# ndmarco/BayesFMMM

Measured on AMD Instinct MI355X. Metric: Gibbs iterations/sec (whole node) at n_funct=4096, K=3, P=30, higher is better.
Workload: dtype f64; 1 GPU; BFMMM_warm_start sweep, n_funct=4096, n_i=100, K=3, P=30, M=6, fp64, one independent chain per GPU (1 chain(s): a chain does not shard, replicas only); chains=1, chains_per_gpu=1

## Files before the change

bayesfmmm_amd/_lib.py:

```python
import ctypes as C
import os

_HERE = os.path.dirname(os.path.abspath(__file__))
LIB_PATH = os.environ.get("BFMMM_LIB_PATH", os.path.join(_HERE, "libbfmmm_hip.so"))

c_double_p = C.POINTER(C.c_double)
c_int64_p = C.POINTER(C.c_int64)


class BfmmmConfig(C.Structure):
    _fields_ = [("model", C.c_int32), ("n_funct", C.c_int32), ("K", C.c_int32), ("n_eigen", C.c_int32),
                ("basis_degree", C.c_int32), ("n_internal_knots", C.c_int32), ("P", C.c_int32),
                ("tot_mcmc_iters", C.c_int32), ("c", C.c_double * 8), ("b", C.c_double), ("nu_1", C.c_double),
                ("alpha1l", C.c_double), ("alpha2l", C.c_double), ("beta1l", C.c_double), ("beta2l", C.c_double),
                ("a_Z_PM", C.c_double), ("a_pi_PM", C.c_double), ("var_alpha3", C.c_double),
                ("var_epsilon1", C.c_double), ("var_epsilon2", C.c_double), ("alpha_nu", C.c_double),
                ("beta_nu", C.c_double), ("alpha_eta", C.c_double), ("beta_eta", C.c_double),
                ("alpha_0", C.c_double), ("beta_0", C.c_double)]


SYMBOLS = {
    "bfmmm_config_defaults": (None, [C.POINTER(BfmmmConfig)]),
    "bfmmm_create": (C.c_int, [C.POINTER(BfmmmConfig), C.c_int, c_double_p, c_double_p, c_int64_p, c_double_p,
                               c_double_p, C.POINTER(C.c_void_p)]),
    "bfmmm_destroy": (None, [C.c_void_p]),
    "bfmmm_create_batch": (C.c_int, [C.POINTER(BfmmmConfig), C.c_int, c_double_p, c_double_p, c_int64_p, c_double_p,
                                     c_double_p, C.c_int, C.POINTER(C.c_void_p)]),
    "bfmmm_create_from_basis_batch": (C.c_int, [C.POINTER(BfmmmConfig), C.c_int, c_double_p, c_double_p, c_int64_p, C.c_int,
                                                C.c_int, c_double_p, C.c_int, C.c_int, C.POINTER(C.c_void_p)]),
    "bfmmm_select_chain": (C.c_int, [C.c_void_p, C.c_int]),
    "bfmmm_n_chains": (C.c_int, [C.c_void_p]),
    "bfmmm_selected_chain": (C.c_int, [C.c_void_p]),
    "bfmmm_set_chain_id_stride": (C.c_int, [C.c_void_p, C.c_uint32]),
    "bfmmm_gather_best": (C.c_int, [C.POINTER(C.c_void_p), C.c_int, c_double_p, C.POINTER(C.c_int32), C.POINTER(C.c_int)]),
    "bfmmm_set_covariates": (C.c_int, [C.c_void_p, c_double_p, C.c_int, C.c_int]),
    "bfmmm_get_basis": (C.c_int, [C.c_void_p, c_double_p, C.c_int64]),
    "bfmmm_set_state": (C.c_int, [C.c_void_p, C.c_char_p, c_double_p, C.c_int64]),
    "bfmmm_get_state": (C.c_int, [C.c_void_p, C.c_char_p, c_double_p, C.c_int64]),
    "bfmmm_init_state": (C.c_int, [C.c_void_p, C.c_int, C.c_uint64, C.c_uint32]),
    "bfmmm_run": (C.c_int, [C.c_void_p, C.c_uint32, C.c_int, C.c_int, C.c_uint64, C.c_uint32, C.c_int, C.c_double]),
    "bfmmm_prepare_run": (C.c_int, [C.c_void_p, C.c_uint32, C.c_int, C.c_int, C.c_uint64, C.c_uint32, C.c_int]),
    "bfmmm_set_slot_base": (C.c_int, [C.c_void_p, C.c_int]),
    "bfmmm_create_from_basis": (C.c_int, [C.POINTER(BfmmmConfig), C.c_int, c_double_p, c_double_p, c_int64_p, C.c_int, C.c_int,
                                          c_double_p, C.c_int, C.POINTER(C.c_void_p)]),
    "bfmmm_tempered_transition": (C.c_int, [C.c_void_p, C.c_uint32, C.c_int, C.c_int, C.c_double, C.c_uint64, C.c_uint32,
                                            c_double_p, C.POINTER(C.c_int)]),
    "bfmmm_get_chain": (C.c_int, [C.c_void_p, C.c_char_p, C.c_int, c_double_p, C.c_int64]),
    "bfmmm_chain_diagnostics": (C.c_int, [C.c_void_p, C.c_char_p, C.c_int, C.c_int, C.c_int64, c_double_p, c_double_p, c_double_p,
                                          c_double_p, c_double_p, c_double_p, c_double_p, C.c_int64]),
    "bfmmm_chain_curve_loglik": (C.c_int, [C.c_void_p, C.c_int, C.c_int, c_double_p, C.c_int64]),
    "bfmmm_chain_curve_diagnostics": (C.c_int, [C.c_void_p, C.c_int, C.c_int, C.c_int64, c_double_p, c_double_p, c_double_p,
                                                c_double_p, c_double_p, c_double_p, c_double_p, C.c_int64]),
    "bfmmm_chain_loo": (C.c_int, [C.c_void_p, C.c_int, C.c_int, C.c_int64, c_double_p, c_double_p, c_double_p, c_double_p,
                                  c_double_p, c_double_p, C.c_int64]),
    "bfmmm_chain_curve_fit": (C.c_int, [C.c_void_p, C.c_int, c_double_p, C.c_int, C.POINTER(C.c_int32), C.c_int, C.c_int, C.c_int,
                                        c_double_p, C.c_int64]),
    "bfmmm_chain_curve_bands": (C.c_int, [C.c_void_p, C.c_int, c_double_p, C.c_int, C.POINTER(C.c_int32), C.c_int, C.c_int, C.c_int,
                                          c_double_p, C.c_int, C.c_int64, c_double_p, c_double_p, c_double_p, C.c_int64]),
    "bfmmm_chain_curve_bands_sim": (C.c_int, [C.c_void_p, C.c_int, c_double_p, C.c_int, C.POINTER(C.c_int32), C.c_int, C.c_int, C.c_int,
                                              C.c_double, C.c_int64, c_double_p, c_double_p, c_double_p, c_double_p, c_double_p, C.c_int64]),
    "bfmmm_set_curve_fit_route": (None, [C.c_int]),
    "bfmmm_chain_similarity": (C.c_int, [C.c_void_p, C.POINTER(C.c_int32), C.c_int, C.c_int, C.c_int, C.c_int64, c_double_p, c_double_p,
                                         c_double_p, C.c_int64]),
    "bfmmm_set_similarity_block": (None, [C.c_int]),
    "bfmmm_chain_similarity_loss": (C.c_int, [C.c_void_p, C.c_int, C.c_int, C.c_int64, c_double_p, C.c_int64, C.POINTER(C.c_int32),
                                              C.POINTER(C.c_int32), c_double_p]),
    "bfmmm_get_slot": (C.c_int, [C.c_void_p, C.c_char_p, C.c_int, c_double_p, C.c_int64]),
    "bfmmm_set_chain": (C.c_int, [C.c_void_p, C.c_char_p, C.c_int, C.c_int, c_double_p, C.c_int64]),
    "bfmmm_chain_slot_loglik": (C.c_int, [C.c_void_p, C.c_int, C.c_int, C.c_int, C.c_int64, c_double_p, c_double_p, C.c_int64]),
    "bfmmm_chain_curve_cov": (C.c_int, [C.c_void_p, c_double_p, C.c_int, c_double_p, C.c_int, C.c_int, C.POINTER(C.c_int32), C.c_int, C.c_int,
                                        C.c_int, C.c_int64, c_double_p, c_double_p, c_double_p, C.c_int64]),
    "bfmmm_chain_align": (C.c_int, [C.c_void_p, c_double_p, C.c_int, C.c_int, C.POINTER(C.c_int32), c_double_p, C.c_int64]),
    "bfmmm_chain_aligned_summary": (C.c_int, [C.c_void_p, C.c_char_p, C.POINTER(C.c_int32), C.c_int, C.c_int, c_double_p, C.c_int,
                                              C.c_int64, c_double_p, c_double_p, c_double_p, c_double_p, c_double_p, c_double_p,
                                              c_double_p, c_double_p, C.c_int64]),
    "bfmmm_chain_cluster_mean_bands": (C.c_int, [C.c_void_p, C.POINTER(C.c_int32), c_double_p, C.c_int, C.c_int, C.c_int, c_double_p,
                                                 C.c_int, C.c_int64, c_double_p, c_double_p, c_double_p, C.c_int64]),
    "bfmmm_chain_cluster_cov_bands": (C.c_int, [C.c_void_p, C.POINTER(C.c_int32), c_double_p, C.c_int, c_double_p, C.c_int, C.c_int,
                                                C.POINTER(C.c_int32), C.c_int, c_double_p, C.c_int, C.c_int, c_double_p, C.c_int, C.c_double,
                                                C.c_int64, c_double_p, c_double_p, c_double_p, c_double_p, c_double_p, c_double_p,
                                                c_double_p, C.c_int64]),
    "bfmmm_chain_rescale": (C.c_int, [C.c_void_p, C.POINTER(C.c_int32), c_double_p, C.c_int, C.c_int, c_double_p, c_double_p,
                                      C.POINTER(C.c_int32), c_double_p, c_double_p, c_int64_p, C.c_int64]),
    "bfmmm_chain_rescaled_summary": (C.c_int, [C.c_void_p, C.c_char_p, c_double_p, c_double_p, C.c_int, C.c_int, c_double_p, C.c_int,
                                               C.c_int64] + [c_double_p] * 8 + [C.c_int64]),
    "bfmmm_chain_cluster_mean_bands_rescaled": (C.c_int, [C.c_void_p, c_double_p, c_double_p, C.c_int, c_double_p, C.c_int, C.c_int,
                                                          c_double_p, C.c_int, C.c_int64, c_double_p, c_double_p, c_double_p, C.c_int64]),
    "bfmmm_chain_cluster_cov_bands_rescaled": (C.c_int, [C.c_void_p, c_double_p, c_double_p, C.c_int, c_double_p, C.c_int, C.c_int,
                                                         C.POINTER(C.c_int32), C.c_int, c_double_p, C.c_int, C.c_int, c_double_p, C.c_int,
                                                         C.c_double, C.c_int64] + [c_double_p] * 7 + [C.c_int64]),
    "bfmmm_chain_cluster_contrast_bands": (C.c_int, [C.c_void_p, c_double_p, c_double_p, C.c_int, c_double_p, c_double_p, C.c_int,
                                                     c_double_p, C.c_int, C.c_int, c_double_p, C.c_int, C.c_double, C.c_int64,
                                                     c_double_p, c_double_p, c_double_p, C.POINTER(C.c_int32), c_double_p, c_double_p,
                                                     c_double_p, C.POINTER(C.c_int32), c_double_p, c_double_p, c_double_p, c_double_p,
                                                     C.c_int64]),
    "bfmmm_chain_cluster_eigen": (C.c_int, [C.c_void_p, C.POINTER(C.c_int32), c_double_p, C.c_int, c_double_p, c_double_p, C.c_int,
                                            c_double_p, C.c_int, C.c_int, c_double_p, C.c_int, C.c_int64] + [c_double_p] * 13 +
                                  [C.POINTER(C.c_int32), C.c_int64]),
    "bfmmm_set_cluster_eig_form": (None, [C.c_int]),
    "bfmmm_chain_predict": (C.c_int, [C.c_void_p, c_double_p, c_double_p, c_double_p, c_int64_p, C.c_int, c_double_p,
                                      C.POINTER(C.c_int32), C.c_int, C.c_int, C.c_int, C.c_int, C.c_uint64, c_double_p, C.c_int64] +
                            [c_double_p] * 10 + [C.c_int64]),
    "bfmmm_chain_predict_fit": (C.c_int, [C.c_void_p, c_double_p, c_double_p, c_double_p, c_int64_p, C.c_int, c_double_p,
                                          C.POINTER(C.c_int32), C.c_int, C.c_int, C.c_int, C.c_int, C.c_uint64, c_double_p,
                                          c_double_p, C.c_int, C.c_int, c_double_p, C.c_int, C.c_int64] +
                                [c_double_p] * 16 + [C.POINTER(C.c_int32), c_double_p, c_double_p, C.c_int64]),
    "bfmmm_chain_loo_marginal": (C.c_int, [C.c_void_p, C.c_int, C.c_int, C.c_int, C.c_int, C.c_uint64, C.c_int, C.c_double, C.c_int,
                                           C.c_int, C.c_int64] + [c_double_p] * 8 + [C.POINTER(C.c_int32)] * 2 + [c_double_p] * 3 +
                                 [C.POINTER(C.c_int32), c_double_p, c_double_p, c_int64_p, C.c_int64, C.c_int64]),
    "bfmmm_chain_predict_laplace": (C.c_int, [C.c_void_p, c_double_p, c_double_p, c_double_p, c_int64_p, C.c_int, c_double_p,
                                              C.POINTER(C.c_int32), C.c_int, C.c_int, C.c_int, C.c_uint64, C.c_int64] +
                                    [c_double_p] * 8 + [C.POINTER(C.c_int32), c_double_p, c_double_p, C.c_int64]),
    "bfmmm_chain_loo_marginal_laplace": (C.c_int, [C.c_void_p, C.c_int, C.c_int, C.c_int, C.c_uint64, C.c_double, C.c_int64] +
                                         [c_double_p] * 8 + [C.POINTER(C.c_int32), c_double_p, c_double_p, C.POINTER(C.c_int32),
                                                             c_double_p, c_double_p, C.c_int64]),
    "bfmmm_chain_loo_pointwise": (C.c_int, [C.c_void_p, C.POINTER(C.c_int32), C.c_int, C.c_int, C.c_int, C.c_int64] +
                                  [c_double_p] * 13 + [C.c_int64]),
    "bfmmm_chain_loo_blocks": (C.c_int, [C.c_void_p, C.POINTER(C.c_int32), c_int64_p, C.POINTER(C.c_int32), C.c_int64, C.c_int, C.c_int,
                                         C.c_int64] + [c_double_p] * 13 + [C.c_int64, C.c_int64]),
    "bfmmm_chain_loo_by_chain": (C.c_int, [C.c_void_p, C.c_int, C.POINTER(C.c_int32), C.c_int, C.c_int, C.c_int, C.c_int64] +
                                 [c_double_p] * 6 + [C.c_int64]),
    "bfmmm_debug_get": (C.c_int, [C.c_void_p, C.c_char_p, c_double_p, C.c_int64, c_int64_p]),
    "bfmmm_set_profile": (C.c_int, [C.c_void_p, C.c_int]),
    "bfmmm_get_timing": (C.c_int, [C.c_void_p, C.c_char_p, C.POINTER(C.c_double), c_int64_p]),
    "bfmmm_set_exact_instances": (None, [C.c_int]),
    "bfmmm_set_curve_record": (None, [C.c_int]),
    "bfmmm_set_solo_pair_gram": (None, [C.c_int]),
    "bfmmm_set_solo_pair_gram_tail": (None, [C.c_int]),
    "bfmmm_last_error": (C.c_char_p, []),
}

_LIB = None


def load():
    global _LIB
    if _LIB is None:
        if not os.path.exists(LIB_PATH):
            raise RuntimeError(
                f"{LIB_PATH} is missing: build it with `python -c 'import __graft_entry__ as g; g.build()'` "
                "(hipcc --offload-arch=gfx950). bayesfmmm_amd has no CPU fallback.")
        lib = C.CDLL(LIB_PATH)
        for name, (res, args) in SYMBOLS.items():
            fn = getattr(lib, name)
            fn.restype = res
            fn.argtypes = args
        _LIB = lib
    return _LIB


class BfmmmError(RuntimeError):
    pass


def check(rc):
    if rc != 0:
        raise BfmmmError(load().bfmmm_last_error().decode())
```

bayesfmmm_amd/csrc/bfmmm_capi.hip:

```cpp
#include "handle.hpp"
#include "rng.hpp"
#include "launchers.hpp"

#include <algorithm>
#include <cmath>
#include <cstring>
#include <map>
#include <chrono>
#include <mutex>

using namespace bfmmm;

static thread_local std::string g_err;
static constexpr int GRAPH_UNROLL = 10;
static std::mutex g_capture_mutex;
int bfmmm::fail(const std::string& msg) { g_err = msg; return 1; }

static const char* kFamNames[FAM_COUNT] = {"total", "curve_z", "pair_gram", "factor", "sweep", "curve_chi", "loglik", "pg_reduce"};

hipError_t bfmmm::copy_sync(bfmmm_handle* h, void* dst, const void* src, size_t bytes, hipMemcpyKind kind) {
  hipError_t e = hipMemcpyAsync(dst, src, bytes, kind, h->st);
  if (e != hipSuccess) return e;
  return hipStreamSynchronize(h->st);
}
// ... 45 lines not shown
extern "C" const char* bfmmm_last_error(void) { return g_err.c_str(); }

static void set_md(Dims& d, int MD) {
  d.MD = MD;
  d.A = d.K * MD;
  d.NZZ = d.K * (d.K + 1) / 2;
  d.NCC = MD * (MD + 1) / 2;
  d.R = d.NZZ * d.NCC;
  d.RT = (d.R + 15) / 16;
  d.AT = (d.A + 15) / 16;
  d.CTG = d.mv ? 1 : (d.LG + 15) / 16;
  d.CTS = (d.P + 15) / 16;
  d.NT = d.RT * d.CTG + d.AT * d.CTS;
}

struct BasisSpec {
  int P, band, pen_band;
  const double* B;
  const double* Pmat;
};

static int create_impl(const bfmmm_config* cfg, int device, const double* y, const double* t, const int64_t* offsets,
                       const double* internal_knots, const double* boundary_knots, const BasisSpec* bs, int n_chains,
                       bfmmm_handle** out);

extern "C" int bfmmm_create(const bfmmm_config* cfg, int device, const double* y, const double* t, const int64_t* offsets,
                            const double* internal_knots, const double* boundary_knots, bfmmm_handle** out) {
  return create_impl(cfg, device, y, t, offsets, internal_knots, boundary_knots, nullptr, 1, out);
}

extern "C" int bfmmm_create_batch(const bfmmm_config* cfg, int device, const double* y, const double* t, const int64_t* offsets,
                                  const double* internal_knots, const double* boundary_knots, int n_chains, bfmmm_handle** out) {
  return create_impl(cfg, device, y, t, offsets, internal_knots, boundary_knots, nullptr, n_chains, out);
}

extern "C" int bfmmm_create_from_basis(const bfmmm_config* cfg, int device, const double* y, const double* B, const int64_t* offsets,
                                       int P, int band, const double* Pmat, int pen_band, bfmmm_handle** out) {
  return bfmmm_create_from_basis_batch(cfg, device, y, B, offsets, P, band, Pmat, pen_band, 1, out);
}

extern "C" int bfmmm_create_from_basis_batch(const bfmmm_config* cfg, int device, const double* y, const double* B, const int64_t* offsets,
                                             int P, int band, const double* Pmat, int pen_band, int n_chains, bfmmm_handle** out) {
  if (!cfg || !y || !B || !offsets || !Pmat || !out) return fail("bfmmm_create_from_basis: null argument");
  if (cfg->model != BFMMM_MODEL_FUNCTIONAL) return fail("bfmmm_create_from_basis: functional model only");
  if (P < 1 || band < 0 || pen_band < 0) return fail("bfmmm_create_from_basis: bad dimensions");
  if (band > BWWIDE) return fail("bfmmm_create_from_basis: the band half-width of B'B must not exceed 31 in this build");
  BasisSpec bs = {P, band, pen_band, B, Pmat};
  return create_impl(cfg, device, y, nullptr, offsets, nullptr, nullptr, &bs, n_chains, out);
}

struct HandleGuard {
  bfmmm_handle* h;
  ~HandleGuard() { if (h) bfmmm_destroy(h); }
};

static int create_impl(const bfmmm_config* cfg, int device, const double* y, const double* t, const int64_t* offsets,
                       const double* internal_knots, const double* boundary_knots, const BasisSpec* bs, int n_chains,
                       bfmmm_handle** out) {
  if (!cfg || !out || !y) return fail("bfmmm_create: null argument");
  if (n_chains < 1 || n_chains > 4096) return fail("bfmmm_create_batch: n_chains must be between 1 and 4096");
  int ndev = 0;
  if (hipGetDeviceCount(&ndev) != hipSuccess || ndev <= 0)
    return fail("bfmmm_create: no HIP device available (the sampler has no CPU fallback)");
  if (device < 0 || device >= ndev) return fail("bfmmm_create: invalid device index");
  const bool mv = cfg->model == BFMMM_MODEL_MULTIVARIATE;
  const int n = cfg->n_funct, K = cfg->K, M = cfg->n_eigen;
  if (n < 1) return fail("'n_funct' must be an integer greater than or equal to 1");
  if (K < 2) return fail("'K' must be an integer greater than or equal to 2");
  if (K > KMAX) return fail("K larger than 8 is not supported by this build");
  if (M < 1) return fail("'n_eigen' must be an integer greater than or equal to 1");
  if (cfg->tot_mcmc_iters < 1) return fail("'tot_mcmc_iters' must be positive");
  int P, BW;
  if (mv) {
    P = cfg->P; BW = 0;
    if (P < 1) return fail("multivariate model: P must be positive");
  } else if (bs) {
    P = bs->P;
    BW = (bs->band <= BWMAX) ? std::min(bs->band, std::max(P - 1, 0)) : (bs->band <= BWMID) ? BWMID : BWWIDE;
  } else {
    if (!t || !offsets || !boundary_knots || (cfg->n_internal_knots > 0 && !internal_knots))
      return fail("bfmmm_create: null argument");
    if (cfg->basis_degree < 1) return fail("'basis_degree' must be an integer greater than or equal to 1");
    if (cfg->basis_degree > BWMAX) return fail("basis_degree larger than 5 is not supported by this build");
    for (int i = 0; i < cfg->n_internal_knots; ++i) {
      if (boundary_knots[0] >= internal_knots[i])
        return fail("at least one element in 'internal_knots' is less than or equal to first boundary knot");
      if (boundary_knots[1] <= internal_knots[i])
        return fail("at least one element in 'internal_knots' is more than or equal to second boundary knot");
    }
    P = cfg->n_internal_knots + cfg->basis_degree + 1;
    BW = std::min(cfg->basis_degree, P - 1);
  }
  if (P > PMAX) return fail("P larger than 64 is not supported by this build");
  if (M > 16) return fail("n_eigen larger than 16 is not supported by this build");

  HIPCHK(hipSetDevice(device));
  prepare_curve_kernels();
  prepare_pair_gram_kernels();
  prepare_factor_kernels();
  prepare_sweep_kernels();
  prepare_cov_kernels();
  { hipError_t e0 = hipGetLastError(); if (e0 != hipSuccess) fprintf(stderr, "[bfmmm] note: kernel attribute setup reported %s\n", hipGetErrorString(e0)); }
  bfmmm_handle* h = new bfmmm_handle();
  HandleGuard guard{h};
  h->cfg = *cfg;
  h->device = device;
  h->T = cfg->tot_mcmc_iters;
  h->nch = n_chains;
  HIPCHK(hipStreamCreateWithFlags(&h->st, hipStreamNonBlocking));
  HIPCHK(hipEventCreate(&h->evA));
  HIPCHK(hipEventCreate(&h->ev0));
  HIPCHK(hipEventCreate(&h->ev1));
  HIPCHK(hipHostMalloc((void**)&h->status_host, sizeof(uint32_t) * (size_t)n_chains, hipHostMallocMapped));
  if (hipHostGetDevicePointer((void**)&h->status_dev, h->status_host, 0) != hipSuccess) { (void)hipGetLastError(); h->status_dev = nullptr; }
  Ctx& c = h->c;
  memset(&c, 0, sizeof c);
  Dims& d = c.d;
  d.n = n; d.K = K; d.P = P; d.M = M; d.D = 0; d.BW = BW; d.LG = (BW + 1) * P;
  d.LREC = (d.LG + P + 1 + 1) / 2 * 2;
  d.mv = mv ? 1 : 0;
  d.BWP = mv ? 0 : std::max(BW, 1);
  if (bs) d.BWP = std::min(std::max(BW, bs->pen_band), (BW > BWMAX) ? BWWIDE : BWMAX);
  if (bs && BW == BWMID && bs->pen_band > BWMID) { BW = BWWIDE; d.BW = BW; d.LG = (BW + 1) * P; d.LREC = (d.LG + P + 1 + 1) / 2 * 2; d.BWP = std::min(std::max(BW, bs->pen_band), BWWIDE); }
  if (bs && BW <= BWMAX && bs->pen_band > BWMAX) return fail("bfmmm_create_from_basis: a penalty band wider than 5 needs a basis band wider than 5 in this build");
  set_md(d, M + 1);
  for (int k = 0; k < KMAX; ++k) c.h.c[k] = (k < 8) ? cfg->c[k] : 10.0;
  c.h.b = cfg->b; c.h.nu_1 = cfg->nu_1;
  c.h.alpha1l = cfg->alpha1l; c.h.alpha2l = cfg->alpha2l; c.h.beta1l = cfg->beta1l; c.h.beta2l = cfg->beta2l;
  c.h.a_Z_PM = cfg->a_Z_PM; c.h.a_pi_PM = cfg->a_pi_PM; c.h.var_alpha3 = cfg->var_alpha3;
  c.h.var_epsilon1 = cfg->var_epsilon1; c.h.var_epsilon2 = cfg->var_epsilon2;
  c.h.alpha_nu = cfg->alpha_nu; c.h.beta_nu = cfg->beta_nu; c.h.alpha_eta = cfg->alpha_eta; c.h.beta_eta = cfg->beta_eta;
  c.h.alpha_0 = cfg->alpha_0; c.h.beta_0 = cfg->beta_0;
  c.T = h->T;
  c.nblk_curve = curve_blocks(n, P);

  const int64_t n_obs = mv ? (int64_t)n * P : offsets[n];
  h->n_obs = n_obs;
  double* rec; int* ni;
  if (dalloc(h, &rec, (size_t)n * d.LREC) || dalloc(h, &ni, n)) return 1;
  c.rec = rec; c.ni = ni;
  int* stab;
  if (dalloc(h, &stab, sweep_tab_ints(K * (M + 1)))) return 1;
  c.sweep_tab = stab;
  std::vector<ArenaReq> ar;
  areq(ar, &c.dyn, 1);
  areq(ar, &c.Z, (size_t)n * K); areq(ar, &c.chi, (size_t)n * M); areq(ar, &c.theta, (size_t)K * (M + 1) * P);
  areq(ar, &c.delta, (size_t)K * M); areq(ar, &c.Aa, (size_t)K * 2); areq(ar, &c.gamma, (size_t)K * P * M);
  int NKS, KS;
  pg_geometry(d, NKS, KS);
  h->pg_part_doubles = (size_t)NKS * d.NT * 256;
  areq(ar, &c.logz_part, (size_t)c.nblk_curve * K); areq(ar, &c.rss_part, c.nblk_curve);
  areq(ar, &c.pg_part, h->pg_part_doubles); areq(ar, &c.H, (size_t)d.R * d.LG + 2); areq(ar, &c.H2, (size_t)d.R * P * (2 * d.BW + 2));
  areq(ar, &c.tvec, (size_t)d.A * P); areq(ar, &c.rvec, (size_t)d.A * P); areq(ar, &c.hq, (size_t)d.A * P);
  areq(ar, &c.gstd, gstd_doubles(K, P, M)); areq(ar, &c.zprep, (size_t)(3 * K + 5) * n);
  areq(ar, &c.chi_norm, (size_t)n * M); areq(ar, &c.zrec, zrec_stride(n, K)); areq(ar, &c.piprep, 9 * KMAX + 16); areq(ar, &c.Lz, (size_t)d.A * P);
  areq(ar, &c.Cmat, (size_t)d.A * P * P + 2);
  {
    const size_t T = (size_t)h->T;
    areq(ar, &c.c_nu, T * K * P); areq(ar, &c.c_chi, T * n * M); areq(ar, &c.c_Z, T * n * K); areq(ar, &c.c_pi, T * K);
    areq(ar, &c.c_alpha3, T); areq(ar, &c.c_delta, T * K * M); areq(ar, &c.c_A, T * K * 2); areq(ar, &c.c_sigma, T);
    areq(ar, &c.c_tau, T * K); areq(ar, &c.c_gamma, T * K * P * M); areq(ar, &c.c_Phi, T * K * P * M); areq(ar, &c.c_loglik, T);
  }
  if (arena_commit(h, ar, n_chains, &c.chain_bytes, &h->arena)) return 1;
  c.chain_bytes_cov = 0; c.chain_id_stride = 1; c.nch = n_chains;
  double* pm;
  if (dalloc(h, &pm, (size_t)P * P)) return 1;
  c.Pmat = pm;
  if (bs) {
    HIPCHK(copy_sync(h, pm, bs->Pmat, sizeof(double) * (size_t)P * P, hipMemcpyHostToDevice));
  } else {
    std::vector<double> Pm((size_t)P * P, 0.0);
    for (int j = 0; j < P; ++j) {
      Pm[0] = 1;
      if (j > 0) { Pm[j + (size_t)P * j] = 2; Pm[(j - 1) + (size_t)P * j] = -1; Pm[j + (size_t)P * (j - 1)] = -1; }
      Pm[(P - 1) + (size_t)P * (P - 1)] = 1;
    }
    HIPCHK(copy_sync(h, pm, Pm.data(), sizeof(double) * Pm.size(), hipMemcpyHostToDevice));
  }

  if (dalloc(h, &h->d_y, (size_t)n_obs)) return 1;
  HIPCHK(copy_sync(h, h->d_y, y, sizeof(double) * (size_t)n_obs, hipMemcpyHostToDevice));
  int* d_err;
  if (dalloc(h, &d_err, 1)) return 1;
  if (mv) {
    launch_stats_multivariate(n, P, d.LREC, h->d_y, rec, ni, h->st);
  } else if (bs) {
    std::vector<double> hrec((size_t)n * d.LREC, 0.0);
    std::vector<int> hni((size_t)n);
    for (int i = 0; i < n; ++i) {
      double* r = hrec.data() + (size_t)i * d.LREC;
      hni[i] = (int)(offsets[i + 1] - offsets[i]);
      for (int64_t l = offsets[i]; l < offsets[i + 1]; ++l) {
        const double* b = bs->B + (size_t)l * P;
        for (int lo = 0; lo < P; ++lo) {
          if (b[lo] == 0.0) continue;
          for (int dd = 0; dd <= BW && lo + dd < P; ++dd) r[dd * P + lo] += b[lo] * b[lo + dd];
          r[d.LG + lo] += b[lo] * y[l];
        }
        r[d.LG + P] += y[l] * y[l];
      }
    }
    HIPCHK(copy_sync(h, rec, hrec.data(), sizeof(double) * hrec.size(), hipMemcpyHostToDevice));
    HIPCHK(copy_sync(h, ni, hni.data(), sizeof(int) * hni.size(), hipMemcpyHostToDevice));
    h->B_host.assign(bs->B, bs->B + (size_t)n_obs * P);
  } else {
    const int deg = cfg->basis_degree, nint = cfg->n_internal_knots;
    h->n_knots = nint + 2 * (deg + 1);
    std::vector<double> knots(h->n_knots);
    for (int i = 0; i <= deg; ++i) knots[i] = boundary_knots[0];
    for (int i = 0; i < nint; ++i) knots[deg + 1 + i] = internal_knots[i];
    for (int i = 0; i <= deg; ++i) knots[deg + 1 + nint + i] = boundary_knots[1];
    if (dalloc(h, &h->d_t, (size_t)n_obs) || dalloc(h, &h->d_off, (size_t)n + 1) || dalloc(h, &h->d_knots, h->n_knots))
      return 1;
    HIPCHK(copy_sync(h, h->d_t, t, sizeof(double) * (size_t)n_obs, hipMemcpyHostToDevice));
    HIPCHK(copy_sync(h, h->d_off, offsets, sizeof(int64_t) * ((size_t)n + 1), hipMemcpyHostToDevice));
    HIPCHK(copy_sync(h, h->d_knots, knots.data(), sizeof(double) * knots.size(), hipMemcpyHostToDevice));
    if (launch_stats_functional(deg, n, P, d.LREC, h->d_off, h->d_t, h->d_y, h->d_knots, h->n_knots, rec, ni, nullptr,
                                d_err, h->st))
      return fail("unsupported basis_degree");
  }
  double* d_yy; long long* d_cnt;
  if (dalloc(h, &d_yy, 1) || dalloc(h, &d_cnt, 2)) return 1;
  launch_stats_totals(n, d.LREC, d.LG + P, rec, ni, d_yy, d_cnt, h->st);
  HIPCHK(hipStreamSynchronize(h->st));
  HIPCHK(hipGetLastError());
  int herr = 0; long long cnt[2];
  HIPCHK(copy_sync(h, &herr, d_err, sizeof(int), hipMemcpyDeviceToHost));
  HIPCHK(copy_sync(h, &c.YY, d_yy, sizeof(double), hipMemcpyDeviceToHost));
  HIPCHK(copy_sync(h, cnt, d_cnt, sizeof cnt, hipMemcpyDeviceToHost));
  if (herr) return fail("at least one time point lies outside 'boundary_knots'");
  d.n_obs_total = cnt[0];
  d.half_sum = cnt[1];
  Dyn dyn0;
  memset(&dyn0, 0, sizeof dyn0);
  dyn0.beta = 1; dyn0.sigma2 = 1; dyn0.alpha3 = 1;
  for (int k = 0; k < KMAX; ++k) { dyn0.pi[k] = 1.0 / K; dyn0.tau[k] = 1; }
  for (int q = 0; q < n_chains; ++q)
    HIPCHK(copy_sync(h, chain_ctx(c, (unsigned)q).dyn, &dyn0, sizeof dyn0, hipMemcpyHostToDevice));
  guard.h = nullptr;
  *out = h;
  return 0;
}

extern "C" int bfmmm_set_covariates(bfmmm_handle* h, const double* X, int D, int covariance_adj) {
  if (!h || !X) return fail("bfmmm_set_covariates: null argument");
  if (D < 1 || D > 8) return fail("bfmmm_set_covariates: the number of covariates must be between 1 and 8 in this build");
  if (h->c.d.D != 0) return fail("bfmmm_set_covariates: covariates are already set");
  HIPCHK(hipSetDevice(h->device));
  Ctx& c = h->c;
  Dims& d = c.d;
  const size_t n = d.n, K = d.K, P = d.P, M = d.M, T = (size_t)h->T;
  d.D = D;
  c.covariance_adj = covariance_adj ? 1 : 0;
  c.A2 = (int)(K * D + (covariance_adj ? K * M * D : 0));
  c.NB2 = cov_w2_chunks((int)n);
  c.NBS = cov_step_blocks(c.nblk_curve);
  c.NPG = D * (D + 1) / 2;
  c.NPAIR = (c.A2 / D) * c.NPG;
  if (!cov_block_fits(c)) {
    d.D = 0;
    return fail("bfmmm_set_covariates: this many covariates with this basis exceed the covariate kernels' on-chip staging (fewer covariates or a narrower band)");
  }
  double* Xd;
  if (dalloc(h, &Xd, n * D)) return 1;
  HIPCHK(copy_sync(h, Xd, X, sizeof(double) * n * D, hipMemcpyHostToDevice));
  c.X = Xd;
  std::vector<ArenaReq> ar;
  areq(ar, &c.thetaX, K * (M + 1) * D * P); areq(ar, &c.tau_eta, K * D); areq(ar, &c.gamma_xi, K * P * D * M);
  areq(ar, &c.delta_xi, K * M * D); areq(ar, &c.A_xi, K * 2 * D); areq(ar, &c.stil, n * P);
  areq(ar, &c.yyp_part, (size_t)c.nblk_curve); areq(ar, &c.cfull, n * P); areq(ar, &c.gfull, n * P);
  areq(ar, &c.w2_part, (size_t)c.NPAIR * c.NB2 * d.LG); areq(ar, &c.H2aa, (size_t)c.NPAIR * d.LG);
  areq(ar, &c.Wdir, n * (size_t)c.A2); areq(ar, &c.gstd2, K * D + K * M * D + K * D * P * M);
  areq(ar, &c.C2, (size_t)c.A2 * P * P + 2); areq(ar, &c.Lz2, (size_t)c.A2 * P);
  areq(ar, &c.step_part, 2 * (size_t)c.NBS * (D * P + 1)); areq(ar, &c.thetaN, K * (M + 1) * D * P); areq(ar, &c.delta_cur, P + 2);
  areq(ar, &c.c_eta, T * P * D * K); areq(ar, &c.c_xi, T * K * P * D * M); areq(ar, &c.c_tau_eta, T * K * D);
  areq(ar, &c.c_gamma_xi, T * K * P * D * M); areq(ar, &c.c_delta_xi, T * K * M * D); areq(ar, &c.c_A_xi, T * K * 2 * D);
  if (arena_commit(h, ar, h->nch, &c.chain_bytes_cov, &h->arena_cov)) { d.D = 0; return 1; }
  std::vector<double> ones(std::max({K * D, K * P * D * M, K * M * D, K * 2 * D}), 1.0);
  for (int q = 0; q < h->nch; ++q) {
    const Ctx cq = chain_ctx(c, (unsigned)q);
    HIPCHK(copy_sync(h, cq.tau_eta, ones.data(), sizeof(double) * K * D, hipMemcpyHostToDevice));
    HIPCHK(copy_sync(h, cq.gamma_xi, ones.data(), sizeof(double) * K * P * D * M, hipMemcpyHostToDevice));
    HIPCHK(copy_sync(h, cq.delta_xi, ones.data(), sizeof(double) * K * M * D, hipMemcpyHostToDevice));
    HIPCHK(copy_sync(h, cq.A_xi, ones.data(), sizeof(double) * K * 2 * D, hipMemcpyHostToDevice));
  }
  drop_graphs(h);
  return 0;
}

extern "C" void bfmmm_destroy(bfmmm_handle* h) {
  if (!h) return;
  (void)hipSetDevice(h->device);
  if (h->st) (void)hipStreamSynchronize(h->st);
  drop_graphs(h);
  for (int q = 1; q < bfmmm_handle::MAX_SUB; ++q) { if (h->sub_st[q]) (void)hipStreamDestroy(h->sub_st[q]); if (h->sub_ev[q]) (void)hipEventDestroy(h->sub_ev[q]); }
  for (void* p : h->allocs) (void)hipFree(p);
  if (h->status_host) (void)hipHostFree(h->status_host);
  if (h->ev0) (void)hipEventDestroy(h->ev0);
  if (h->ev1) (void)hipEventDestroy(h->ev1);
  if (h->evA) (void)hipEventDestroy(h->evA);
  if (h->st) (void)hipStreamDestroy(h->st);
  delete h;
}

extern "C" int bfmmm_get_basis(bfmmm_handle* h, double* out, int64_t capacity) {
  if (!h || !out) return fail("bfmmm_get_basis: null argument");
  const Dims& d = h->c.d;
// ... 270 lines not shown
    launch_loglik_flush(c, sb.st, h->status_dev);
    return;
  }
  for (int r = 0; r < reps; ++r)
    launch_iteration(h, sb.c, plan, sb.r, sb.st, nullptr, kind != GK_FULL, kind == GK_FUSED, kind == GK_DEFERRED);
}

template <typename F>
static int cached_graph(bfmmm_handle* h, int sub, int kind, int reps, hipStream_t st, std::vector<FreshGraph>& fresh, F body,
                        hipGraphExec_t* out) {
  int n_whole = 0;
  for (const auto& e : h->graphs) {
    if (e.sub == sub && e.kind == kind && e.reps == reps) { *out = e.g; return 0; }
    n_whole += e.kind == GK_WHOLE;
  }
  if (kind == GK_WHOLE && n_whole >= WHOLE_KEEP) {
    auto it = std::find_if(h->graphs.begin(), h->graphs.end(), [](const bfmmm_handle::CachedGraph& e) { return e.kind == GK_WHOLE; });
    (void)hipGraphExecDestroy(it->g);
    h->graphs.erase(it);
  }
  std::lock_guard<std::mutex> lock(g_capture_mutex);
  hipGraph_t graph = nullptr;
  HIPCHK(hipStreamBeginCapture(st, hipStreamCaptureModeRelaxed));
  body();
  const hipError_t ec = hipStreamEndCapture(st, &graph);
  if (ec != hipSuccess) { if (graph) (void)hipGraphDestroy(graph); HIPCHK(ec); }
  hipGraphExec_t g = nullptr;
  const hipError_t ei = hipGraphInstantiate(&g, graph, nullptr, nullptr, 0);
  (void)hipGraphDestroy(graph);
  HIPCHK(ei);
  (void)hipGraphUpload(g, st);
  h->graphs.push_back({sub, kind, reps, g});
  fresh.push_back({g, st});
  *out = g;
  return 0;
}

static int dry_launch(bfmmm_handle* h, const Ctx& c, uint32_t mask, const Sub* subs, int nsub, const std::vector<FreshGraph>& fresh,
                      int first_iter, uint32_t tt_step, double beta) {
  if (fresh.empty()) return 0;
  const size_t wb1 = (size_t)((char*)h->c.c_nu - (char*)h->c.dyn);
  const size_t wb2 = (c.d.D > 0 && h->arena_cov) ? (size_t)((char*)h->c.c_eta - (char*)h->c.thetaX) : 0;
  const size_t need = (size_t)h->nch * (wb1 + wb2);
  if (h->dry_snap_bytes < need) {
    char* nb = nullptr;
    if (hipMalloc((void**)&nb, need) != hipSuccess) { (void)hipGetLastError(); return 0; }
    h->allocs.push_back(nb);
    h->dry_snap = nb; h->dry_snap_bytes = need;
  }
  const size_t cb1 = h->nch > 1 ? h->c.chain_bytes : wb1, cb2 = h->nch > 1 ? h->c.chain_bytes_cov : wb2;
  char* snap2 = h->dry_snap + (size_t)h->nch * wb1;
  for (int q = 0; q < nsub; ++q) HIPCHK(hipStreamSynchronize(subs[q].st));
  HIPCHK(hipMemcpy2DAsync(h->dry_snap, wb1, h->c.dyn, cb1, wb1, (size_t)h->nch, hipMemcpyDeviceToDevice, h->st));
  if (wb2) HIPCHK(hipMemcpy2DAsync(snap2, wb2, h->c.thetaX, cb2, wb2, (size_t)h->nch, hipMemcpyDeviceToDevice, h->st));
  ensure_sweep_tables(h, c, mask);
  const auto t_dry = std::chrono::steady_clock::now();
  for (int round = 0; round < 64; ++round) {
    for (const FreshGraph& fg : fresh) {
      hipLaunchKernelGGL(k_run_begin, dim3(h->nch), dim3(64), 0, h->st, h->c, (uint32_t)first_iter, (uint32_t)h->slot_base, tt_step, beta, 0);
      HIPCHK(hipStreamSynchronize(h->st));
      HIPCHK(hipGraphLaunch(fg.g, fg.st));
      HIPCHK(hipStreamSynchronize(fg.st));
    }
    if (std::chrono::duration<double, std::milli>(std::chrono::steady_clock::now() - t_dry).count() >= 10.0) break;
  }
  HIPCHK(hipMemcpy2DAsync(h->c.dyn, cb1, h->dry_snap, wb1, wb1, (size_t)h->nch, hipMemcpyDeviceToDevice, h->st));
  if (wb2) HIPCHK(hipMemcpy2DAsync(h->c.thetaX, cb2, snap2, wb2, wb2, (size_t)h->nch, hipMemcpyDeviceToDevice, h->st));
  HIPCHK(hipStreamSynchronize(h->st));
  HIPCHK(hipGetLastError());
  return 0;
}

static int run_profiled(bfmmm_handle* h, const Ctx& c, const Plan& plan, const PgRoute& r, int n_iters, uint32_t tt_step) {
  const bool fuse = plan.z && plan.z_update && plan.chi && c.d.D == 0 && n_iters >= 2 && tt_step == 0;
  for (int it = 0; it < n_iters; ++it) {
    std::vector<hipEvent_t> evs;
    const bool skip_z = fuse && it > 0, fuse_z = fuse && it + 1 < n_iters;
    launch_iteration(h, c, plan, r, h->st, &evs, skip_z, fuse_z, false);
    HIPCHK(hipStreamSynchronize(h->st));
    const int fams[7] = {FAM_Z, FAM_PG, FAM_REDUCE, FAM_FACTOR, FAM_SWEEP, FAM_CHI, FAM_LOGLIK};
    const bool ran[7] = {plan.z && !skip_z, true, plan.pg, plan.factor, true, true, c.defer_loglik == 0};
    for (int q = 0; q < 7; ++q) {
      float ms = 0;
      (void)hipEventElapsedTime(&ms, evs[q], evs[q + 1]);
      if (ran[q]) { h->fam_ms[fams[q]] += ms; h->fam_launches[fams[q]] += 1; }
    }
    for (hipEvent_t e : evs) (void)hipEventDestroy(e);
  }
  return 0;
}

static int finish_run(bfmmm_handle* h, const Ctx& c, const Plan& plan, uint32_t mask, int first_iter, int n_iters, bool whole) {
  const bool status_by_kernel = c.defer_loglik && n_iters > 0 && h->status_dev != nullptr;
  if (c.defer_loglik && n_iters > 0 && !whole) launch_loglik_flush(c, h->st, status_by_kernel ? h->status_dev : nullptr);
  const int s0 = first_iter - h->slot_base, s1 = s0 + n_iters;
  if (!(mask & U_Z)) launch_fill_slots(c, c.c_Z, c.Z, (size_t)c.d.n * c.d.K, s0, s1, h->st);
  if (!plan.chi_update) launch_fill_slots(c, c.c_chi, c.chi, (size_t)c.d.n * c.d.M, s0, s1, h->st);
  HIPCHK(hipEventRecord(h->ev1, h->st));
  if (!status_by_kernel)
    HIPCHK(hipMemcpy2DAsync(h->status_host, sizeof(uint32_t), &h->c.dyn->status, h->nch > 1 ? h->c.chain_bytes : sizeof(uint32_t), sizeof(uint32_t),
                            (size_t)h->nch, hipMemcpyDeviceToHost, h->st));
  HIPCHK(hipStreamSynchronize(h->st));
  if (h->launch_error == 2) { h->launch_error = 0; drop_graphs(h); return fail("bfmmm_run: internal error (no per-curve kernel instance is built for the route the launcher chose)"); }
  if (h->launch_error) { h->launch_error = 0; return fail("bfmmm_run: problem size exceeds the sweep kernel's LDS (5 A P doubles + A^2 ints must fit 160 KB)"); }
  HIPCHK(hipGetLastError());
  float ms = 0;
  HIPCHK(hipEventElapsedTime(&ms, h->ev0, h->ev1));
  h->fam_ms[FAM_TOTAL] = ms;
  h->fam_launches[FAM_TOTAL] = n_iters;
  for (int q = 0; q < h->nch; ++q) {
    const uint32_t status = h->status_host[q];
    if (status & 8u) return fail("bfmmm_run: internal error (the pi / alpha_3 job of k_factor did not signal)");
    if (status & 4u) return fail("bfmmm_run: internal error (a hand-off inside the sweep kernel timed out)");
    if (status & 2u) return fail("bfmmm_run: internal error (fused Z update without prepared proposals)");
    if (status & 1u)
      return fail("bfmmm_run: a conditional precision matrix was not positive definite");
  }
  return 0;
}

static void record_curve_route(bfmmm_handle* h, const Ctx& c, const Plan& plan, bool fuse, bool defer) {
  double v[14] = {0, -1, 0, 0, 0, 0, -1, 0, 0, 0, 0, 0, 0, 0};
  const int mode = chi_launch_arg(plan, false);
  const CurveRoute rc = curve_route_decide(c.d, 1, mode);
  const double w[8] = {(double)rc.BW, (double)rc.LPC, rc.COV ? 1.0 : 0.0, rc.SMALL ? 1.0 : 0.0, (double)rc.KX, (double)rc.MX, (double)mode,
                       fuse ? 1.0 : 0.0};
  memcpy(v + 6, w, sizeof w);
  if (fuse) {
    const CurveRoute rf = curve_route_decide(c.d, 1, chi_launch_arg(plan, true));
    const double z[6] = {3, (double)rf.BW, (double)rf.LPC, 0, (double)(rf.KX ? rf.KX : (rf.SMALL ? 4 : KMAX)), rf.KX ? 1.0 : 0.0};
    memcpy(v, z, sizeof z);
  } else if (plan.z) {
    const CurveRoute rz = curve_route_decide(c.d, 0, z_launch_arg(plan, defer));
    const double z[6] = {rz.LEAN ? 2.0 : 1.0, (double)rz.BW, (double)rz.LPC, rz.COV ? 1.0 : 0.0, (double)rz.KT, rz.KEX ? 1.0 : 0.0};
    memcpy(v, z, sizeof z);
  }
  memcpy(h->last_curve, v, sizeof v);
}

static int run_impl(bfmmm_handle* h, uint32_t mask, int first_iter, int n_iters, uint64_t seed, uint32_t chain,
                    int phi_chi_zero, double beta, uint32_t tt_step, bool prepare_only = false) {
  if (!h) return fail("bfmmm_run: null handle");
  if (n_iters < 0 || first_iter < h->slot_base || first_iter - h->slot_base + n_iters > h->T)
    return fail("bfmmm_run: iterations exceed the allocated chain");
  HIPCHK(hipSetDevice(h->device));
  Ctx c = h->c;
  const int MD = phi_chi_zero ? 1 : (c.d.M + 1);
  set_md(c.d, MD);
  c.seed = seed; c.chain = chain; c.mask = mask;
  Plan plan = make_plan(mask, MD);
  if (c.d.D > 0) { plan.z = true; plan.chi = true; plan.use_rss_part = 1; }
  c.defer_loglik = (c.d.D == 0) ? 1 : 0;
  c.ll_use_part = plan.use_rss_part;
  h->last_md = MD;
  int nsub = 1;
  if (!h->profile && h->nch >= 4) nsub = 2;
  if (const char* env_split = h->profile ? nullptr : getenv("BFMMM_BATCH_SPLIT"))
    nsub = std::max(1, std::min({atoi(env_split), (int)bfmmm_handle::MAX_SUB, h->nch / 2}));
  Sub subs[bfmmm_handle::MAX_SUB];
  h->sub_st[0] = h->st;
  for (int q = 0, q0 = 0; q < nsub; ++q) {
    const int cnt = h->nch / nsub + (q < h->nch % nsub ? 1 : 0);
    if (pg_route(h, c, plan.pg, cnt, h->profile ? bfmmm_handle::MAX_SUB : q, subs[q].r)) return 1;
    if (!h->sub_st[q]) HIPCHK(hipStreamCreateWithFlags(&h->sub_st[q], hipStreamNonBlocking));
    if (!h->sub_ev[q]) HIPCHK(hipEventCreateWithFlags(&h->sub_ev[q], hipEventDisableTiming));
    subs[q].c = chain_ctx(c, (unsigned)q0);
    subs[q].c.nch = cnt;
    subs[q].st = h->sub_st[q];
    q0 += cnt;
  }
  {
    const PgRoute& r0 = subs[0].r;
    const double v[6] = {r0.packed ? 1.0 : 0.0, (double)r0.KS, (double)r0.NKS, (double)r0.body, (double)r0.G, (double)r0.tail};
    memcpy(h->last_route, v, sizeof v);
    const SweepRoute sr = sweep_route_decide(c.d);
    const double w[5] = {(double)sr.kernel, (double)sr.targ, c.d.mv ? 1.0 : 0.0, (double)sr.direct, (double)sr.threads};
    memcpy(h->last_sweep, w, sizeof w);
    if (c.d.D > 0) {
      const CovRoute cr = cov_route_decide(c);
      const double x[11] = {(double)cr.BW, (double)cr.LPC, (double)cr.DX, (double)cr.W2D, (double)cr.PP, (double)cr.NB2, (double)cr.NBS,
                            (double)cr.NPG, (double)cr.launches, cr.do_eta ? 1.0 : 0.0, cr.do_xi ? 1.0 : 0.0};
      memcpy(h->last_cov, x, sizeof x);
    }
  }
  const int rec_on = bfmmm::g_curve_record;
  if (!rec_on) {
    c.zrec = nullptr;
    for (int q = 0; q < nsub; ++q) subs[q].c.zrec = nullptr;
  }
  c.defer_hyper = (c.defer_loglik && plan.pg && plan.chi && h->nch == 1 && !subs[0].r.packed && subs[0].r.NKS >= 2) ? 1 : 0;
  subs[0].c.defer_hyper = c.defer_hyper;
  if (!prepare_only) {
    ensure_sweep_tables(h, c, mask);
    hipLaunchKernelGGL(k_run_begin, dim3(h->nch), dim3(64), 0, h->st, h->c, (uint32_t)first_iter, (uint32_t)h->slot_base, tt_step, beta,
                       h->state_dirty ? 1 : 0);
    h->state_dirty = false;
    for (int f = 0; f < FAM_COUNT; ++f) { h->fam_ms[f] = 0; h->fam_launches[f] = 0; }
  }
  const bool fuse = plan.z && plan.z_update && plan.chi && c.d.D == 0 && n_iters >= 2 && tt_step == 0;
  const bool defer = !h->profile && !fuse && plan.z && plan.z_update && plan.factor && (mask & U_Z) && c.d.D == 0 && c.d.K <= 4 &&
                     c.d.BW <= 5 && n_iters >= 2 && tt_step == 0;
  if (n_iters > 0) record_curve_route(h, c, plan, fuse, defer);
  {
    const bool lean_host = defer && !plan.chi;
    const double v[3] = {c.defer_hyper ? 2.0 : (lean_host ? 1.0 : 0.0), subs[0].r.packed ? 2.0 : (pg_route_solo_ll(subs[0].r) ? 1.0 : 0.0),
                         (plan.factor && (mask & (U_PI | U_ALPHA3))) ? 1.0 : 0.0};
    memcpy(h->last_hyper, v, sizeof v);
  }
  if (!prepare_only && n_iters > 0) h->zrec_form = (rec_on && plan.z && plan.z_update) ? (fuse ? 2 : 1) : 0;
  if (!prepare_only && n_iters > 0) h->pi_flag_stored = rec_on && (mask & (U_PI | U_ALPHA3)) != 0;
  if (h->profile) {
    if (prepare_only) return 0;
    HIPCHK(hipEventRecord(h->ev0, h->st));
    if (run_profiled(h, c, plan, subs[0].r, n_iters, tt_step)) return 1;
    return finish_run(h, c, plan, mask, first_iter, n_iters, false);
  }
  const bool bodies = fuse || defer;
  const int body_kind = fuse ? GK_FUSED : GK_DEFERRED;
  const int nrep = bodies ? n_iters - 1 : n_iters;
  const bool whole = bodies && nsub == 1 && n_iters <= WHOLE_MAX && c.defer_loglik && h->status_dev != nullptr;
  std::vector<std::pair<int, int>> segs;
  const int kind = bodies ? body_kind : GK_FULL;
  if (whole) {
    segs.push_back({GK_WHOLE, n_iters});
  } else {
    for (int q = 0; q < nrep / GRAPH_UNROLL; ++q) segs.push_back({kind, GRAPH_UNROLL});
    if (nrep % GRAPH_UNROLL) segs.push_back({kind, nrep % GRAPH_UNROLL});
    if (bodies) segs.push_back({GK_CLOSING, 1});
  }
  const bfmmm_handle::GraphKey key{mask, MD, seed, chain, nsub, (bfmmm::g_exact_instances ? 1 : 0) | (bfmmm::g_solo_pair_gram ? 2 : 0) |
                                                                        (bfmmm::g_solo_pair_gram_tail ? 4 : 0) | (rec_on ? 8 : 0)};
  if (n_iters > 0 && !(h->g_valid && h->g_key == key)) { drop_graphs(h); h->g_key = key; h->g_valid = true; }
  std::vector<FreshGraph> fresh;
  std::vector<hipGraphExec_t> seq[bfmmm_handle::MAX_SUB];
  for (int s = 0; s < nsub; ++s)
    for (const auto& sg : segs) {
      hipGraphExec_t g = nullptr;
      if (cached_graph(h, s, sg.first, sg.second, subs[s].st, fresh, [&]() { queue_graph(h, c, subs[s], plan, sg.first, sg.second, body_kind); }, &g))
        return 1;
      seq[s].push_back(g);
    }
  if (prepare_only) return dry_launch(h, c, mask, subs, nsub, fresh, first_iter, tt_step, beta);
  HIPCHK(hipEventRecord(h->ev0, h->st));
  if (nsub > 1) HIPCHK(hipEventRecord(h->evA, h->st));
  for (int q = 1; q < nsub; ++q) HIPCHK(hipStreamWaitEvent(subs[q].st, h->evA, 0));
  for (int s = 0; s < nsub && n_iters > 0; ++s) {
    if (bodies && !whole) launch_curve_checked(h, subs[s].c, 0, z_launch_arg(plan, false), subs[s].st);
    for (hipGraphExec_t g : seq[s]) HIPCHK(hipGraphLaunch(g, subs[s].st));
  }
  for (int q = 1; q < nsub; ++q) { HIPCHK(hipEventRecord(h->sub_ev[q], subs[q].st)); HIPCHK(hipStreamWaitEvent(h->st, h->sub_ev[q], 0)); }
  return finish_run(h, c, plan, mask, first_iter, n_iters, whole);
}

extern "C" int bfmmm_set_slot_base(bfmmm_handle* h, int base) {
  if (!h || base < 0) return fail("bfmmm_set_slot_base: bad arguments");
  h->slot_base = base;
  return 0;
}

extern "C" int bfmmm_run(bfmmm_handle* h, uint32_t mask, int first_iter, int n_iters, uint64_t seed, uint32_t chain,
                         int phi_chi_zero, double beta) {
  return run_impl(h, mask, first_iter, n_iters, seed, chain, phi_chi_zero, beta, 0);
}

extern "C" int bfmmm_prepare_run(bfmmm_handle* h, uint32_t mask, int first_iter, int n_iters, uint64_t seed, uint32_t chain,
                                 int phi_chi_zero) {
  return run_impl(h, mask, first_iter, n_iters, seed, chain, phi_chi_zero, 1.0, 0, true);
}

extern "C" int bfmmm_tempered_transition(bfmmm_handle* h, uint32_t mask, int iter, int N_t, double beta_N_t,
                                         uint64_t seed, uint32_t chain, double* logA_out, int* accepted_out) {
  if (!h) return fail("bfmmm_tempered_transition: null handle");
  if (N_t < 1 || iter < h->slot_base || iter - h->slot_base >= h->T) return fail("bfmmm_tempered_transition: bad arguments");
  if (h->nch != 1) return fail("bfmmm_tempered_transition: a tempered transition accepts or rejects one chain: not available on a chain batch");
  HIPCHK(hipSetDevice(h->device));
  const Ctx& c = h->c;
  const Dims& d = c.d;
  const size_t n_th = (size_t)d.K * (d.M + 1) * d.P, n_chi = (size_t)d.n * d.M, n_Z = (size_t)d.n * d.K,
               n_dl = (size_t)d.K * d.M, n_A = (size_t)d.K * 2, n_g = (size_t)d.K * d.P * d.M;
  const size_t Dc = (size_t)d.D;
  const size_t n_tx = (size_t)d.K * (d.M + 1) * Dc * d.P, n_te = (size_t)d.K * Dc, n_gx = (size_t)d.K * d.P * Dc * d.M,
               n_dx = (size_t)d.K * d.M * Dc, n_ax = (size_t)d.K * 2 * Dc;
  if (!h->tt_save) { if (dalloc(h, &h->tt_save, n_th + n_chi + n_Z + n_dl + n_A + n_g + n_tx + n_te + n_gx + n_dx + n_ax + 8)) return 1; }
  double* sv = h->tt_save;
  double* sv_th = sv; double* sv_chi = sv_th + n_th; double* sv_Z = sv_chi + n_chi; double* sv_dl = sv_Z + n_Z;
  double* sv_A = sv_dl + n_dl; double* sv_g = sv_A + n_A;
  double* sv_tx = sv_g + n_g; double* sv_te = sv_tx + n_tx; double* sv_gx = sv_te + n_te; double* sv_dx = sv_gx + n_gx;
  double* sv_ax = sv_dx + n_dx;
  auto d2d = [&](double* dst, const double* src, size_t cnt) {
    return cnt ? hipMemcpyAsync(dst, src, sizeof(double) * cnt, hipMemcpyDeviceToDevice, h->st) : hipSuccess;
  };
  HIPCHK(d2d(sv_th, c.theta, n_th)); HIPCHK(d2d(sv_chi, c.chi, n_chi)); HIPCHK(d2d(sv_Z, c.Z, n_Z));
  HIPCHK(d2d(sv_dl, c.delta, n_dl)); HIPCHK(d2d(sv_A, c.Aa, n_A)); HIPCHK(d2d(sv_g, c.gamma, n_g));
  if (Dc > 0) {
    HIPCHK(d2d(sv_tx, c.thetaX, n_tx)); HIPCHK(d2d(sv_te, c.tau_eta, n_te)); HIPCHK(d2d(sv_gx, c.gamma_xi, n_gx));
    HIPCHK(d2d(sv_dx, c.delta_xi, n_dx)); HIPCHK(d2d(sv_ax, c.A_xi, n_ax));
  }
  Dyn dyn0;
  if (dyn_get(h, dyn0)) return 1;
  std::vector<double> ladder((size_t)N_t, 1.0);
  ladder[N_t - 1] = beta_N_t;
  const double geom_mult = std::pow(beta_N_t, 1.0 / N_t);
  for (int i = 1; i < N_t; ++i) ladder[i] = ladder[i - 1] * geom_mult;
  const int L = 2 * N_t + 1;
  std::vector<double> sig((size_t)L), rss((size_t)L);
  sig[0] = dyn0.sigma2; rss[0] = dyn0.rss;
  int temp_ind = 0;
  for (int l = 1; l < L; ++l) {
    if (run_impl(h, mask | U_LOGLIK, iter, 1, seed, chain, 0, ladder[temp_ind], (uint32_t)l)) return 1;
    Dyn dl;
    if (dyn_get(h, dl)) return 1;
    sig[l] = dl.sigma2; rss[l] = dl.rss;
    if (l < N_t) temp_ind = temp_ind + 1;
    if (l > N_t) temp_ind = temp_ind - 1;
  }
  const double N = (double)d.n_obs_total;
  auto PZ = [&](double b, int l) { return (-(b / 2) * std::log(sig[l])) * N - (b / (2 * sig[l])) * rss[l]; };
  double logA = 0;
  const int m = L - 1;
  for (int i = 0; i < N_t - 1; ++i) {
    logA = logA + PZ(ladder[i + 1], i);
    logA = logA - PZ(ladder[i], i);
    logA = logA - PZ(ladder[i + 1], m - i);
    logA = logA + PZ(ladder[i], m - i);
  }
  const double logu = std::log(runif(make_key(seed, chain, (uint32_t)iter, 0), UPD_TT_ACC, 0));
  const int accepted = (logu < logA) ? 1 : 0;
  if (accepted) {
    HIPCHK(d2d(c.gamma, sv_g, n_g));
    HIPCHK(hipStreamSynchronize(h->st));
  } else {
    HIPCHK(d2d(c.theta, sv_th, n_th)); HIPCHK(d2d(c.chi, sv_chi, n_chi)); HIPCHK(d2d(c.Z, sv_Z, n_Z));
    HIPCHK(d2d(c.delta, sv_dl, n_dl)); HIPCHK(d2d(c.Aa, sv_A, n_A)); HIPCHK(d2d(c.gamma, sv_g, n_g));
    if (Dc > 0) {
      HIPCHK(d2d(c.thetaX, sv_tx, n_tx)); HIPCHK(d2d(c.tau_eta, sv_te, n_te)); HIPCHK(d2d(c.gamma_xi, sv_gx, n_gx));
      HIPCHK(d2d(c.delta_xi, sv_dx, n_dx)); HIPCHK(d2d(c.A_xi, sv_ax, n_ax));
    }
    dyn0.zprep_valid = 0;
    dyn0.piprep_valid = 0;
    if (dyn_put(h, dyn0)) return 1;
    if (run_impl(h, U_LOGLIK, iter, 1, seed, chain, 0, 1.0, 0)) return 1;
  }
  Dyn dn;
  if (dyn_get(h, dn)) return 1;
  dn.iter = (uint32_t)(iter + 1); dn.slot = (uint32_t)(iter + 1 - h->slot_base); dn.tt_step = 0; dn.beta = 1.0;
  if (dyn_put(h, dn)) return 1;
  if (logA_out) *logA_out = logA;
  if (accepted_out) *accepted_out = accepted;
  return 0;
}

extern "C" int bfmmm_debug_get(bfmmm_handle* h, const char* name, double* out, int64_t capacity, int64_t* count) {
  if (!h || !name || !out || !count) return fail("bfmmm_debug_get: null argument");
  HIPCHK(hipSetDevice(h->device));
  const Ctx c = selc(h);
  Dims d = c.d;
  if (h->last_md > 0) set_md(d, h->last_md);
  const std::string s(name);
  HIPCHK(hipStreamSynchronize(h->st));
  if (s == "dims") {
    const double v[] = {(double)d.n, (double)d.K, (double)d.P, (double)d.M, (double)d.BW, (double)d.LG, (double)d.LREC,
                        (double)d.MD, (double)d.A, (double)d.R, (double)d.NT, (double)d.n_obs_total, (double)d.half_sum, c.YY,
                        (double)d.BWP};
    const int64_t cnt = sizeof v / sizeof v[0];
    if (capacity < cnt) return fail("bfmmm_debug_get: buffer too small");
    memcpy(out, v, sizeof v);
    *count = cnt;
    return 0;
  }
  if (s == "pg_route") {
    const int64_t cnt = sizeof h->last_route / sizeof h->last_route[0];
    if (capacity < cnt) return fail("bfmmm_debug_get: buffer too small");
    memcpy(out, h->last_route, sizeof h->last_route);
    *count = cnt;
    return 0;
  }
  if (s == "sweep_route") {
    const int64_t cnt = sizeof h->last_sweep / sizeof h->last_sweep[0];
    if (capacity < cnt) return fail("bfmmm_debug_get: buffer too small");
    memcpy(out, h->last_sweep, sizeof h->last_sweep);
    *count = cnt;
    return 0;
  }
  if (s == "curve_route") {
    const int64_t cnt = sizeof h->last_curve / sizeof h->last_curve[0];
    if (capacity < cnt) return fail("bfmmm_debug_get: buffer too small");
    memcpy(out, h->last_curve, sizeof h->last_curve);
    *count = cnt;
    return 0;
  }
  if (s == "cov_route") {
    if (d.D == 0) return fail("bfmmm_debug_get(" + s + "): the record exists once covariates are set");
    const int64_t cnt = sizeof h->last_cov / sizeof h->last_cov[0];
    if (capacity < cnt) return fail("bfmmm_debug_get: buffer too small");
    memcpy(out, h->last_cov, sizeof h->last_cov);
    *count = cnt;
    return 0;
  }
  if (s == "hyper_route") {
    const int64_t cnt = sizeof h->last_hyper / sizeof h->last_hyper[0];
    if (capacity < cnt) return fail("bfmmm_debug_get: buffer too small");
    memcpy(out, h->last_hyper, sizeof h->last_hyper);
    *count = cnt;
    return 0;
  }
  if (s == "pi_prepared") {
    if (!bfmmm::g_curve_record) return fail("bfmmm_debug_get(" + s + "): recording is off (bfmmm_set_curve_record)");
    if (!h->pi_flag_stored) return fail("bfmmm_debug_get(" + s + "): the last run stored no flag (neither U_PI nor U_ALPHA3 in its mask, or recording was off)");
    if (capacity < 1) return fail("bfmmm_debug_get(" + s + "): buffer too small");
    HIPCHK(copy_sync(h, out, c.zrec + zrec_stride(d.n, d.K) - 1, sizeof(double), hipMemcpyDeviceToHost));
    *count = 1;
    return 0;
  }
  if (s == "z_record" || s == "z_prepared") {
    if (!bfmmm::g_curve_record) return fail("bfmmm_debug_get(" + s + "): recording is off (bfmmm_set_curve_record)");
    if (!h->zrec_form) return fail("bfmmm_debug_get(" + s + "): the last run stored no record (no Z update in its mask, or recording was off)");
    const int64_t len = (int64_t)(ZREC_SCALARS + d.K) * d.n, cnt = s == "z_record" ? len : 1;
    if (capacity < cnt) return fail("bfmmm_debug_get(" + s + "): buffer too small");
    if (s == "z_prepared" && h->zrec_form == 2) out[0] = 1.0;
    else HIPCHK(copy_sync(h, out, c.zrec + (s == "z_record" ? 0 : len), sizeof(double) * (size_t)cnt, hipMemcpyDeviceToHost));
    *count = cnt;
    return 0;
  }
  if (s == "rss") {
    if (capacity < 1) return fail("bfmmm_debug_get: buffer too small");
    Dyn dn;
    if (dyn_get(h, dn)) return 1;
    out[0] = dn.rss;
    *count = 1;
    return 0;
  }
  if (s == kPostNames[PT_CURVE_LL]) {
    if (capacity < 1) return fail("bfmmm_debug_get: buffer too small");
    out[0] = h->post_ms[PT_CURVE_LL];
    *count = 1;
    return 0;
  }
  struct Arr { const char* nm; const double* p; int64_t len; };
  const Arr arrs[] = {{"rec", c.rec, (int64_t)d.n * d.LREC}, {"H", c.H, (int64_t)d.R * d.LG}, {"tvec", c.tvec, (int64_t)d.A * d.P},
                      {"H2", c.H2, (int64_t)d.R * d.P * (2 * d.BW + 2)},
                      {"Cmat", c.Cmat, (int64_t)d.A * d.P * d.P}, {"Lz", c.Lz, (int64_t)d.A * d.P},
                      {"rvec", c.rvec, (int64_t)d.A * d.P}, {"hq", c.hq, (int64_t)d.A * d.P},
                      {"theta", c.theta, (int64_t)d.K * (d.M + 1) * d.P},
                      {"chi_norm", c.chi_norm, (int64_t)d.n * d.M}, {"zprep", c.zprep, (int64_t)(3 * d.K + 5) * d.n},
                      {"gstd", c.gstd, (int64_t)gstd_doubles(d.K, d.P, d.M)}, {"piprep", c.piprep, (int64_t)9 * KMAX + 16},
                      {"rss_part", c.rss_part, (int64_t)c.nblk_curve}, {"logz_part", c.logz_part, (int64_t)c.nblk_curve * d.K},
                      {"stil", c.stil, (int64_t)d.n * d.P}, {"yyp_part", c.yyp_part, (int64_t)c.nblk_curve},
                      {"cfull", c.cfull, (int64_t)d.n * d.P}, {"gfull", c.gfull, (int64_t)d.n * d.P},
                      {"Wdir", c.Wdir, (int64_t)d.n * c.A2}, {"H2aa", c.H2aa, (int64_t)c.NPAIR * d.LG},
                      {"C2", c.C2, (int64_t)c.A2 * d.P * d.P}, {"Lz2", c.Lz2, (int64_t)c.A2 * d.P},
                      {"gstd2", c.gstd2, (int64_t)d.K * d.D + (int64_t)d.K * d.M * d.D + (int64_t)d.K * d.D * d.P * d.M},
                      {"thetaX", c.thetaX, (int64_t)d.K * (d.M + 1) * d.D * d.P}};
  for (const Arr& a : arrs)
    if (s == a.nm) {
      if (!a.p) return fail("bfmmm_debug_get(" + s + "): the array exists once covariates are set");
      if (capacity < a.len) return fail("bfmmm_debug_get(" + s + "): buffer too small");
      HIPCHK(copy_sync(h, out, a.p, sizeof(double) * (size_t)a.len, hipMemcpyDeviceToHost));
      *count = a.len;
      return 0;
    }
  return fail("bfmmm_debug_get: unknown name '" + s + "'");
}

namespace bfmmm { int g_exact_instances = 1; int g_solo_pair_gram = 1; int g_solo_pair_gram_tail = 1; int g_curve_record = 0; }
extern "C" void bfmmm_set_curve_record(int enable) { bfmmm::g_curve_record = enable ? 1 : 0; }
extern "C" void bfmmm_set_exact_instances(int enable) { bfmmm::g_exact_instances = enable ? 1 : 0; }
extern "C" void bfmmm_set_solo_pair_gram(int enable) { bfmmm::g_solo_pair_gram = enable ? 1 : 0; }
extern "C" void bfmmm_set_solo_pair_gram_tail(int enable) { bfmmm::g_solo_pair_gram_tail = enable ? 1 : 0; }

extern "C" int bfmmm_set_profile(bfmmm_handle* h, int enable) {
  if (!h) return fail("bfmmm_set_profile: null handle");
  h->profile = enable ? 1 : 0;
  return 0;
}

extern "C" int bfmmm_get_timing(bfmmm_handle* h, const char* name, double* ms, int64_t* launches) {
  if (!h || !name || !ms || !launches) return fail("bfmmm_get_timing: null argument");
  for (int f = 0; f < FAM_COUNT; ++f)
    if (!strcmp(name, kFamNames[f])) { *ms = h->fam_ms[f]; *launches = h->fam_launches[f]; return 0; }
  for (int f = PT_CURVE_LL + 1; f < PT_COUNT; ++f)
    if (!strcmp(name, kPostNames[f])) { *ms = h->post_ms[f]; *launches = h->post_launches[f]; return 0; }
  if (!strcmp(name, "curve_fit")) {
    *ms = 0; *launches = 0;
    for (int f = PT_FIT_PROJECT; f <= PT_FIT_REDUCE; ++f) { *ms += h->post_ms[f]; *launches += h->post_launches[f]; }
    return 0;
  }
  return fail("bfmmm_get_timing: unknown name");
}

#include <rccl/rccl.h>

#define NCCLCHK(x)                                                                                   \
  do {                                                                                              \
    ncclResult_t r_ = (x);                                                                          \
    if (r_ != ncclSuccess) {                                                                        \
      char buf_[512];                                                                               \
      snprintf(buf_, sizeof buf_, "RCCL error %s at %s:%d (%s)", ncclGetErrorString(r_), __FILE__, __LINE__, #x); \
      return fail(buf_);                                                                            \
    }                                                                                               \
  } while (0)

struct GatherGuard {
  std::vector<ncclComm_t> comms;
  std::vector<int> devs;
  std::vector<double*> bufs;
  ~GatherGuard() {
    for (ncclComm_t cm : comms) if (cm) (void)ncclCommDestroy(cm);
    for (size_t i = 0; i < bufs.size(); ++i)
      if (bufs[i]) { (void)hipSetDevice(devs[i / 2]); (void)hipFree(bufs[i]); }
  }
};

extern "C" int bfmmm_gather_best(bfmmm_handle* const* handles, int n_handles, const double* scores, const int32_t* chain_ids,
                                 int* winner_out) {
  if (!handles || !scores || !chain_ids || n_handles < 1) return fail("bfmmm_gather_best: bad arguments");
  const int G = n_handles;
  std::vector<int> devs(G);
  for (int g = 0; g < G; ++g) {
    if (!handles[g]) return fail("bfmmm_gather_best: null handle");
    devs[g] = handles[g]->device;
    if (handles[g]->c.chain_bytes != handles[0]->c.chain_bytes || handles[g]->c.chain_bytes_cov != handles[0]->c.chain_bytes_cov)
      return fail("bfmmm_gather_best: the handles were not created with the same configuration");
    for (int g2 = 0; g2 < g; ++g2)
      if (devs[g2] == devs[g]) return fail("bfmmm_gather_best: one handle per device");
  }
  GatherGuard gg;
  gg.devs = devs;
  gg.comms.assign(G, nullptr);
  gg.bufs.assign(2 * (size_t)G, nullptr);
  std::vector<ncclComm_t>& comms = gg.comms;
  NCCLCHK(ncclCommInitAll(comms.data(), G, devs.data()));
  std::vector<double*> sbuf(G, nullptr), rbuf(G, nullptr);
  for (int g = 0; g < G; ++g) {
    HIPCHK(hipSetDevice(devs[g]));
    HIPCHK(hipMalloc((void**)&gg.bufs[2 * g], sizeof(double) * 2));
    HIPCHK(hipMalloc((void**)&gg.bufs[2 * g + 1], sizeof(double) * 2 * (size_t)G));
    sbuf[g] = gg.bufs[2 * g];
    rbuf[g] = gg.bufs[2 * g + 1];
    const double pair[2] = {scores[g], (double)chain_ids[g]};
    HIPCHK(copy_sync(handles[g], sbuf[g], pair, sizeof pair, hipMemcpyHostToDevice));
  }
  NCCLCHK(ncclGroupStart());
  for (int g = 0; g < G; ++g) NCCLCHK(ncclAllGather(sbuf[g], rbuf[g], 2, ncclDouble, comms[g], handles[g]->st));
  NCCLCHK(ncclGroupEnd());
  std::vector<double> all(2 * (size_t)G);
  int winner = -1;
  for (int g = 0; g < G; ++g) {
    HIPCHK(hipSetDevice(devs[g]));
    HIPCHK(hipStreamSynchronize(handles[g]->st));
    HIPCHK(copy_sync(handles[g], all.data(), rbuf[g], sizeof(double) * all.size(), hipMemcpyDeviceToHost));
    int w = -1;
    for (int r = 0; r < G; ++r) {
      if (!(all[2 * r] == all[2 * r])) continue;
      if (w < 0 || all[2 * r] > all[2 * w] || (all[2 * r] == all[2 * w] && all[2 * r + 1] < all[2 * w + 1])) w = r;
    }
    if (g == 0) winner = w;
    else if (w != winner) return fail("bfmmm_gather_best: ranks disagree on the winner");
  }
  if (winner < 0) return fail("bfmmm_gather_best: no rank holds a valid chain");
  if (winner != 0) {
    bfmmm_handle* hs = handles[winner], *hd = handles[0];
    const size_t cb = hd->c.chain_bytes, cbc = hd->c.chain_bytes_cov;
    if (!hs->arena || !hd->arena || (cbc && (!hs->arena_cov || !hd->arena_cov))) return fail("bfmmm_gather_best: a handle has no chain arena");
    NCCLCHK(ncclGroupStart());
    NCCLCHK(ncclSend(hs->arena + (size_t)hs->sel * cb, cb, ncclChar, 0, comms[winner], hs->st));
    NCCLCHK(ncclRecv(hd->arena + (size_t)hd->sel * cb, cb, ncclChar, winner, comms[0], hd->st));
    if (cbc) {
      NCCLCHK(ncclSend(hs->arena_cov + (size_t)hs->sel * cbc, cbc, ncclChar, 0, comms[winner], hs->st));
      NCCLCHK(ncclRecv(hd->arena_cov + (size_t)hd->sel * cbc, cbc, ncclChar, winner, comms[0], hd->st));
    }
    NCCLCHK(ncclGroupEnd());
    HIPCHK(hipSetDevice(devs[winner]));
    HIPCHK(hipStreamSynchronize(handles[winner]->st));
    HIPCHK(hipSetDevice(devs[0]));
    HIPCHK(hipStreamSynchronize(handles[0]->st));
    handles[0]->state_dirty = true;
  }
  if (winner_out) *winner_out = winner;
  return 0;
}
```

bayesfmmm_amd/csrc/handle.hpp:

```cpp
#pragma once
#include "../../include/bfmmm.h"
#include "model.hpp"

#include <cstdio>
#include <string>
#include <tuple>
#include <vector>

#define HIPCHK(x)                                                                                   \
  do {                                                                                              \
    hipError_t e_ = (x);                                                                            \
    if (e_ != hipSuccess) {                                                                         \
      (void)hipGetLastError();  \
      char buf_[512];                                                                               \
      snprintf(buf_, sizeof buf_, "HIP error %s at %s:%d (%s)", hipGetErrorString(e_), __FILE__, __LINE__, #x); \
      return bfmmm::fail(buf_);                                                                     \
    }                                                                                               \
  } while (0)

enum { FAM_TOTAL = 0, FAM_Z, FAM_PG, FAM_FACTOR, FAM_SWEEP, FAM_CHI, FAM_LOGLIK, FAM_REDUCE, FAM_COUNT };

enum { PT_CURVE_LL = 0, PT_FIT_PROJECT, PT_FIT_ROWS, PT_FIT_VALUES, PT_FIT_REDUCE, PT_SIM, PT_SIM_REDUCE, PT_SIMILARITY,
       PT_COV_PROJECT, PT_COV, PT_SIM_LOSS, PT_SIM_LOSS_REDUCE, PT_ALIGN_GRAM, PT_ALIGN_GATHER, PT_ALIGN_PROJECT,
       PT_CCOV_PROJECT, PT_CCOV, PT_CCOV_MAXDEV, PT_CEIG_GRAM, PT_CEIG, PT_CEIG_VALUES, PT_PREDICT_STATS, PT_PREDICT, PT_PREDICT_FIT,
       PT_LOO_MARGINAL, PT_LOO_MARGINAL_PSIS, PT_PREDICT_LAPLACE, PT_LOO_MARGINAL_LAPLACE, PT_LOO_POINTWISE, PT_LOO_POINTWISE_PSIS,
       PT_RESCALE_TRANSFORM, PT_RESCALE_GATHER, PT_RESCALE_PROJECT, PT_LOO_BLOCKS, PT_LOO_BLOCKS_PSIS, PT_CONTRAST_COEF,
       PT_CONTRAST_VALUES, PT_CONTRAST_NORM, PT_SLOT_LL, PT_SLOT_LL_REDUCE, PT_COUNT };
inline constexpr const char* kPostNames[PT_COUNT] = {"curve_ll_ms", "curve_fit_project", "curve_fit_rows", "curve_fit_values",
                                                     "curve_fit_reduce", "curve_sim", "curve_sim_reduce", "similarity",
                                                     "curve_cov_project", "curve_cov", "similarity_loss", "similarity_loss_reduce",
                                                     "align_gram", "align_gather", "align_project",
                                                     "cluster_cov_project", "cluster_cov", "cluster_cov_maxdev",
                                                     "cluster_eig_gram", "cluster_eig", "cluster_eig_values",
                                                     "predict_stats", "predict", "predict_fit",
                                                     "loo_marginal", "loo_marginal_psis", "predict_laplace",
                                                     "loo_marginal_laplace", "loo_pointwise", "loo_pointwise_psis",
                                                     "rescale_transform", "rescale_gather", "rescale_project",
                                                     "loo_blocks", "loo_blocks_psis",
                                                     "contrast_coef", "contrast_values", "contrast_norm",
                                                     "slot_loglik", "slot_loglik_reduce"};

struct bfmmm_handle {
  bfmmm_config cfg;
  int device = 0;
  hipStream_t st = nullptr;
  hipEvent_t evA = nullptr;
  bfmmm::Ctx c;
  int nch = 1;
  int sel = 0;
  int T = 0;
  int64_t n_obs = 0;
  double* d_t = nullptr; double* d_y = nullptr; int64_t* d_off = nullptr; double* d_knots = nullptr; int n_knots = 0;
  std::vector<void*> allocs;
  char* arena = nullptr;
  char* arena_cov = nullptr;
  uint32_t* status_host = nullptr;
  uint32_t* status_dev = nullptr;
  size_t pg_part_doubles = 0;
  static constexpr int MAX_SUB = 4;
  char* dry_snap = nullptr;
  size_t dry_snap_bytes = 0;
  double* pg_pack[MAX_SUB + 1] = {};
  size_t pg_pack_doubles[MAX_SUB + 1] = {};
  hipStream_t sub_st[MAX_SUB] = {nullptr, nullptr, nullptr, nullptr};
  hipEvent_t sub_ev[MAX_SUB] = {nullptr, nullptr, nullptr, nullptr};
  struct CachedGraph { int sub, kind, reps; hipGraphExec_t g; };
  std::vector<CachedGraph> graphs;
  using GraphKey = std::tuple<uint32_t, int, uint64_t, uint32_t, int, int>;
  GraphKey g_key;
  bool g_valid = false;
  int last_md = -1;
  double last_route[6] = {0, 0, 0, -1, 0, 0};
  double last_sweep[5] = {-1, 0, 0, 0, 0};
  double last_curve[14] = {0, -1, 0, 0, 0, 0, -1, 0, 0, 0, 0, 0, 0, 0};
  double last_cov[11] = {-1, 0, 0, 0, 0, 0, 0, 0, 0, 0, 0};
  double last_hyper[3] = {-1, -1, 0};
  bool pi_flag_stored = false;
  int64_t tab_key = -1;
  int launch_error = 0;
  int zrec_form = 0;
  int slot_base = 0;
  double* tt_save = nullptr;
  std::vector<double> B_host;
  bool state_dirty = true;
  int profile = 0;
  double fam_ms[FAM_COUNT] = {0};
  int64_t fam_launches[FAM_COUNT] = {0};
  hipEvent_t ev0 = nullptr, ev1 = nullptr;
  double post_ms[PT_COUNT] = {0};
  int64_t post_launches[PT_COUNT] = {0};
};

namespace bfmmm {
int fail(const std::string& msg);
hipError_t copy_sync(bfmmm_handle* h, void* dst, const void* src, size_t bytes, hipMemcpyKind kind);
Ctx selc(const bfmmm_handle* h);
}
```

bayesfmmm_amd/csrc/kernels_factor.hip:

```cpp
#include "model.hpp"
#include "rng.hpp"
#include "scalar_jobs.hpp"
#include "factor_core.hpp"
#include "z_proposal.hpp"
#include "sweep_helpers.hpp"
#include "launchers.hpp"

namespace bfmmm {

#ifdef BFMMM_TIMELINE
void fetch_fct(unsigned long long* out) { (void)hipMemcpyFromSymbol(out, HIP_SYMBOL(g_fct), sizeof(unsigned long long) * 8); }
#endif

template <int PP, int BW>
__global__ __launch_bounds__(256, (BW <= 5) ? 3 : 1) void k_factor(Ctx c0) {
  const int nch_ = c0.nch;
  const Ctx c = chain_ctx(c0, blockIdx.x % nch_);
  const int bx = blockIdx.x / nch_;
  TIMELINE(c, 3);
  extern __shared__ __attribute__((aligned(16))) double smem[];
  const Dims& d = c.d;
  const int P = d.P, MD = d.MD, K = d.K, A = d.A, M = d.M;
  constexpr int W = 2 * BW + 2;
  const int tid = threadIdx.x;
  const bool split = !((BW == 0) && d.BWP == 0);
  const int nF0 = split ? 2 * A : A;
  if (c.pi_in_factor && bx == nF0) {
    job_pi_alpha(c, true, c0.zrec != nullptr);
    __syncthreads();
    if (tid == 0) {
      __threadfence();
      __hip_atomic_store(&c.dyn->pi_done, c.dyn->iter + 1u, __ATOMIC_RELEASE, __HIP_MEMORY_SCOPE_AGENT);
    }
    return;
  }
  const int nF = nF0 + (c.pi_in_factor ? 1 : 0);
  auto wait_pi = [&]() {
    if (!c.pi_in_factor) return;
    if (tid == 0) {
      const uint32_t want = c.dyn->iter + 1u;
      int spins = 0;
      while (__hip_atomic_load(&c.dyn->pi_done, __ATOMIC_RELAXED, __HIP_MEMORY_SCOPE_AGENT) != want) {
        __builtin_amdgcn_s_sleep(64);
        if (++spins > (1 << 20)) { atomicOr(&c.dyn->status, 8u); break; }
      }
      __builtin_amdgcn_fence(__ATOMIC_ACQUIRE, "agent");
    }
    __syncthreads();
  };
  if (bx >= nF) {
    const int ndraw = (hyper_gstd_count(d) + 1 + 8 * d.K + 255) / 256;
    const int zcw = zprep_curves_per_wg(d.K);
    const int nzp = (c.mask & U_Z) ? (d.n + zcw - 1) / zcw : 0;
    const int npi = (c.mask & (U_PI | U_ALPHA3)) ? 1 : 0;
    const int sb = bx - nF;
#ifdef BFMMM_TIMELINE
    const int kind_ = sb < ndraw ? 0 : sb < ndraw + npi ? 2 : sb < ndraw + npi + nzp ? 1 : 3;
    const bool first_ = (sb == 0) || kind_ == 2 || (sb == ndraw + npi && nzp > 0) || (kind_ == 3 && sb == ndraw + npi + nzp);
    if (first_ && threadIdx.x == 0) c.dyn->stamps[56 + 2 * kind_] = wall_clock64();
#endif
    if (sb < ndraw) job_hyper_draws(c, sb * 256);
    else if (sb < ndraw + npi) { wait_pi(); job_pi_prepare(c); }
    else if (sb < ndraw + npi + nzp) job_z_prepare(c, sb - ndraw - npi);
    else job_chi_normals(c, sb - ndraw - npi - nzp);
#ifdef BFMMM_TIMELINE
    if (first_ && threadIdx.x == 0) c.dyn->stamps[57 + 2 * kind_] = wall_clock64();
#endif
    return;
  }
  const bool role_r = split && bx >= A;
  const bool role_f = !role_r;
  const bool do_r = role_r || !split;
  const int a = role_r ? bx - A : bx;
  const int j = a / MD, mt = a - j * MD;
#ifdef BFMMM_TIMELINE
#define FST(i) do { if (bx == 1 && threadIdx.x == 0) c.dyn->stamps[48 + (i)] = wall_clock64(); } while (0)
#else
#define FST(i) do { } while (0)
#endif
  FST(0);
  const int AP = A * P, PS = P + 2 * BW + 1;
  const bool diag = (BW == 0) && d.BWP == 0;
  double* S = smem;
  double* X = S + PP * PP;
  double* thp = diag ? smem : X + PP * PP;
  double* part = thp + A * PS;
  double* zv = part + AP;
  double* hb2 = zv + PP;
  double* dsc = hb2 + P * W;
  const bool upd_nu = (mt == 0) && (c.mask & U_NU);
  const bool upd_phi = (mt > 0) && (c.mask & U_PHI);
  const bool upd = upd_nu || upd_phi;
  const Dyn* dyn = c.dyn;
  constexpr int MAXI = (BW > 5) ? 1 : 4;
  v2d hreg[MAXI][BW + 1];
  double tval[MAXI];
  const bool upd_nu0 = (mt == 0) && (c.mask & U_NU), upd_phi0 = (mt > 0) && (c.mask & U_PHI);
  if (split && role_f && !(upd_nu0 || upd_phi0)) return;
  if (do_r) {
#pragma unroll
    for (int it = 0; it < MAXI; ++it) {
      const int e = min(tid + 256 * it, AP - 1);
      const int b = e / P, p = e - b * P;
      tval[it] = c.theta[(size_t)full_dir(d, b) * P + p];
      const v2d* blk = (const v2d*)(c.H2 + (size_t)hrow(d, a, b) * P * W);
#pragma unroll
      for (int k = 0; k <= BW; ++k) hreg[it][k] = blk[k * P + p];
    }
  } else {
    const v2d* blk = (const v2d*)(c.H2 + (size_t)hrow(d, a, a) * P * W);
    const int p = min(tid, P - 1);
#pragma unroll
    for (int k = 0; k <= BW; ++k) hreg[0][k] = blk[k * P + p];
  }
  const double tv0 = do_r ? c.tvec[a * P + min(tid >> 3, P - 1)] : 0.0;
  constexpr int NPRI = (BW > 5) ? ((BWWIDE + 1) * PP + 255) / 256 : 2;
  double pri[NPRI];
#pragma unroll
  for (int u = 0; u < NPRI; ++u) {
    const int e = tid + 256 * u, t = e / PP, p = e - t * PP, q = p + t;
    const bool in = t <= d.BWP && q < P;
    const int pc = min(p, P - 1), qc = min(q, P - 1);
    double v = 0.0;
    if (mt == 0) v = d.mv ? 0.0 : c.Pmat[pc + (size_t)P * qc];
    else v = c.gamma[j + (size_t)K * (pc + (size_t)P * (mt - 1))];
    pri[u] = (in && (mt == 0 || t == 0)) ? v : 0.0;
  }
  const double dlt = (mt > 0 && tid < M) ? c.delta[j + (size_t)K * tid] : 1.0;
  const double f = dyn->beta / dyn->sigma2;
  const double tau_j = dyn->tau[j];
  if (do_r) for (int x = tid; x < A * PS; x += 256) thp[x] = 0.0;
  if (role_f && upd && tid >= 64 && tid < 64 + P) {
    const RngKey key = make_key(c.seed, c.chain, dyn->iter, dyn->tt_step);
    const uint32_t idx0 = (mt == 0) ? (uint32_t)(j * P) : (uint32_t)((j * M + (mt - 1)) * P);
    zv[tid - 64] = rnorm(key, (mt == 0) ? UPD_NU : UPD_PHI, idx0 + (uint32_t)(tid - 64));
  }
  FST(1);
  __syncthreads();
  FST(2);
  if (!do_r) {
    if (tid < P) {
#pragma unroll
      for (int k = 0; k <= BW; ++k) { hb2[tid * W + 2 * k] = hreg[0][k].x; hb2[tid * W + 2 * k + 1] = hreg[0][k].y; }
    }
    if (tid < 16) dsc[tid] = dlt;
    __syncthreads();
  }
  if (do_r) {
#pragma unroll
  for (int it = 0; it < MAXI; ++it) {
    const int e = tid + 256 * it;
    if (e < AP) { const int b = e / P, p = e - b * P; thp[b * PS + BW + p] = tval[it]; }
  }
  for (int e = tid + 256 * MAXI; e < AP; e += 256) {
    const int b = e / P, p = e - b * P;
    thp[b * PS + BW + p] = c.theta[(size_t)full_dir(d, b) * P + p];
  }
  if (tid < 16) dsc[tid] = dlt;
  __syncthreads();
  for (int base = 0; base < AP; base += 256 * MAXI) {
    if (base > 0) {
#pragma unroll
      for (int it = 0; it < MAXI; ++it) {
        const int e = min(base + tid + 256 * it, AP - 1);
        const int b = e / P, p = e - b * P;
        const v2d* blk = (const v2d*)(c.H2 + (size_t)hrow(d, a, b) * P * W);
#pragma unroll
        for (int k = 0; k <= BW; ++k) hreg[it][k] = blk[k * P + p];
      }
    }
#pragma unroll
    for (int it = 0; it < MAXI; ++it) {
      const int e = base + tid + 256 * it;
      if (e < AP) {
        const int b = e / P, p = e - b * P;
        const double* tb = thp + b * PS + p;
        double v = 0.0;
#pragma unroll
        for (int k = 0; k <= BW; ++k) v += hreg[it][k].x * tb[2 * k] + hreg[it][k].y * tb[2 * k + 1];
        part[e] = v;
        if (b == a) {
#pragma unroll
          for (int k = 0; k <= BW; ++k) { hb2[p * W + 2 * k] = hreg[it][k].x; hb2[p * W + 2 * k + 1] = hreg[it][k].y; }
        }
      }
    }
  }
  __syncthreads();
  FST(3);
  for (int p0 = 0; p0 < P; p0 += 32) {
    const int p = p0 + (tid >> 3), g = tid & 7;
    double acc = 0.0;
    if (p < P)
      for (int b = g; b < A; b += 8) acc += part[b * P + p];
    acc = dpp_add<0xB1>(acc);
    acc = dpp_add<0x4E>(acc);
    acc = dpp_add<0x141>(acc);
    const double tvp = (p0 == 0) ? tv0 : c.tvec[a * P + min(p, P - 1)];
    if (p < P && g == 0) {
      c.rvec[a * P + p] = tvp - acc;
      c.hq[a * P + p] = part[a * P + p];
    }
  }
  FST(4);
  }
  if (role_r || !upd) return;
  double tt = 1.0;
  for (int m2 = 0; m2 < mt; ++m2) tt *= dsc[m2];
  if (diag) {
    double* Cg = c.Cmat + (size_t)a * P * P;
    for (int e = tid; e < P * P; e += 256) {
      const int p = e % P, q = e / P;
      double cv = 0.0;
      if (p == q) {
        double dk = f * hb2[p * W + BW];
        if (mt == 0) dk += d.mv ? 1.0 / tau_j : tau_j * c.Pmat[p + (size_t)P * p];
        else dk += tt * c.gamma[j + (size_t)K * (p + (size_t)P * (mt - 1))];
        double rk = __builtin_amdgcn_rsq(dk);
        rk = rk * (1.5 - (0.5 * dk) * (rk * rk));
        rk = rk * (1.5 - (0.5 * dk) * (rk * rk));
        if (!(dk > 0.0)) atomicOr(&c.dyn->status, 1u);
        cv = rk * rk;
        c.Lz[(size_t)a * P + p] = rk * zv[p];
      }
      Cg[q + (size_t)P * p] = cv;
    }
    FST(6);
    return;
  }
  auto build_prec = [&](bool full) {
    for (int e = tid; e < PP * PP; e += 256) X[e] = 0.0;
    if (BW > 5 || full) {
      for (int e = tid; e < PP * PP; e += 256) S[e] = (!full && e % PP == e / PP) ? 1.0 : 0.0;
      __syncthreads();
    }
#pragma unroll
    for (int u = 0; u < NPRI; ++u) {
      const int e = tid + 256 * u, t = e / PP, p = e - t * PP, q = p + t;
      if (t <= d.BWP && q < P) {
        double v = (t <= BW) ? f * hb2[p * W + BW + t] : 0.0;
        if (mt == 0) v += d.mv ? ((t == 0) ? 1.0 / tau_j : 0.0) : tau_j * pri[u];
        else v += tt * pri[u];
        S[p + PP * q] = v;
        if (BW > 5 || full) S[q + PP * p] = v;
      }
    }
    __syncthreads();
  };
  build_prec(false);
  FST(5);
  double* wkp = dsc + 16;
  if (factor_core<PP>(S, X, zv, P, d.BWP, c.Cmat + (size_t)a * P * P, nullptr, c.Lz + (size_t)a * P, tid, nullptr)) {
    build_prec(true);
    factor_pinv<PP>(S, X, zv, P, c.Cmat + (size_t)a * P * P, nullptr, c.Lz + (size_t)a * P, tid, wkp);
  }
  FST(6);
}

template <int PP>
static void launch_factor_pp(const Ctx& c, int grid, size_t lds, hipStream_t st) {
  switch (c.d.BW) {
    case 0: hipLaunchKernelGGL((k_factor<PP, 0>), dim3(c.nch * grid), dim3(256), lds, st, c); break;
    case 1: hipLaunchKernelGGL((k_factor<PP, 1>), dim3(c.nch * grid), dim3(256), lds, st, c); break;
    case 2: hipLaunchKernelGGL((k_factor<PP, 2>), dim3(c.nch * grid), dim3(256), lds, st, c); break;
    case 3: hipLaunchKernelGGL((k_factor<PP, 3>), dim3(c.nch * grid), dim3(256), lds, st, c); break;
    case 4: hipLaunchKernelGGL((k_factor<PP, 4>), dim3(c.nch * grid), dim3(256), lds, st, c); break;
    case 5: hipLaunchKernelGGL((k_factor<PP, 5>), dim3(c.nch * grid), dim3(256), lds, st, c); break;
    case BWMID: hipLaunchKernelGGL((k_factor<PP, BWMID>), dim3(c.nch * grid), dim3(256), lds, st, c); break;
    default: hipLaunchKernelGGL((k_factor<PP, BWWIDE>), dim3(c.nch * grid), dim3(256), lds, st, c); break;
  }
}

void launch_factor(const Ctx& c, hipStream_t st) {
  const int PP = (c.d.P <= 32) ? 32 : 64;
  const int W = 2 * c.d.BW + 2, PS = c.d.P + 2 * c.d.BW + 1;
  const bool diag = c.d.BW == 0 && c.d.BWP == 0;
  const size_t lds = ((diag ? 0 : 2 * (size_t)PP * PP) + (size_t)c.d.A * PS + (size_t)c.d.A * c.d.P + PP + (size_t)c.d.P * W + 16 + 4 * PP + 2) * sizeof(double);
  const int n_draw = c.d.K * c.d.P * c.d.M + c.d.K * c.d.M + c.d.K + 4 * c.d.K + 1 + 8 * c.d.K;
  const int zcw = zprep_curves_per_wg(c.d.K);
  const int n_zprep = (c.mask & U_Z) ? (c.d.n + zcw - 1) / zcw : 0;
  const int n_znorm = ((c.mask & U_CHI) && c.d.MD > 1) ? (c.d.n * c.d.M + 255) / 256 : 0;
  const int n_pi = (c.mask & (U_PI | U_ALPHA3)) ? 1 : 0;
  const int grid = (diag ? 1 : 2) * c.d.A + (c.pi_in_factor ? 1 : 0) + (n_draw + 255) / 256 + n_zprep + n_znorm + n_pi;
  if (PP == 32) launch_factor_pp<32>(c, grid, lds, st);
  else launch_factor_pp<64>(c, grid, lds, st);
}

void prepare_factor_kernels() {
  set_max_lds((const void*)k_factor<32, 0>); set_max_lds((const void*)k_factor<64, 0>);
  set_max_lds((const void*)k_factor<32, 1>); set_max_lds((const void*)k_factor<64, 1>);
  set_max_lds((const void*)k_factor<32, 2>); set_max_lds((const void*)k_factor<64, 2>);
  set_max_lds((const void*)k_factor<32, 3>); set_max_lds((const void*)k_factor<64, 3>);
  set_max_lds((const void*)k_factor<32, 4>); set_max_lds((const void*)k_factor<64, 4>);
  set_max_lds((const void*)k_factor<32, 5>); set_max_lds((const void*)k_factor<64, 5>);
  set_max_lds((const void*)k_factor<32, BWMID>); set_max_lds((const void*)k_factor<64, BWMID>);
  set_max_lds((const void*)k_factor<32, BWWIDE>); set_max_lds((const void*)k_factor<64, BWWIDE>);
}

}
```

bayesfmmm_amd/csrc/kernels_pair_gram.hip:

```cpp
#include "model.hpp"
#include "scalar_jobs.hpp"
#include "sweep_helpers.hpp"
#include "launchers.hpp"

#include <algorithm>

namespace bfmmm {

#ifdef BFMMM_TIMELINE
__device__ unsigned long long g_wgtrace[3 * 1024];
void fetch_wgtrace(unsigned long long* out) { (void)hipMemcpyFromSymbol(out, HIP_SYMBOL(g_wgtrace), sizeof(unsigned long long) * 3 * 1024); }
#endif

constexpr int PG_THREADS = 512;

constexpr int PG_SOLO = 2;
constexpr int PGS_TMAX = 4;
constexpr int PGS_KS = 256;

inline bool pg_solo_fits(const Dims& d, int KS) {
  return !d.mv && d.D == 0 && d.K <= 4 && d.MD - 1 <= 8 && d.P <= 32 && d.LG <= 128 && KS <= PGS_KS &&
         d.RT <= PGS_TMAX * (PG_THREADS / 64);
}

// ... 58 lines not shown
  const int nlive = min(KS, n - i0);
  const int nchunk = (nlive + 15) >> 4;
  const int nst = nchunk * 16;
  const int KSP = KS + 2, KQ = KS >> 2;
  const int NZZ = d.NZZ, NP = NZZ + d.NCC;
  double* sB = smem;
  double* sP = sB + 16 * KSP;
  const bool wl = tid < nlive;
  const int iw = i0 + tid;
  double z[4], x[8];
  pg_solo_load_zx(c0, wl, iw, z, x);
  const int ccg = tid & 15, ilg = tid >> 4;
  const bool colok = ct * 16 + ccg < d.LG;
  const double* srcg = c0.rec + (size_t)i0 * d.LREC + min(ct * 16 + ccg, d.LREC - 1);
  double vb[PGS_KS / 32];
#pragma unroll
  for (int u = 0; u < PGS_KS / 32; ++u) {
    const int il = ilg + 32 * u;
    vb[u] = (il < nlive && colok) ? srcg[(size_t)il * d.LREC] : 0.0;
  }
  TSTAMP0(c, 47);
  if (tid < nst) {
    double* dst = sP + (tid & 3) * KQ + (tid >> 2);
    int e = 0;
#pragma unroll
    for (int a = 0; a < 4; ++a)
#pragma unroll
      for (int b = a; b < 4; ++b)
        if (b < K) { dst[e * KSP] = z[a] * z[b]; ++e; }
    const double xt[9] = {1.0, x[0], x[1], x[2], x[3], x[4], x[5], x[6], x[7]};
#pragma unroll
    for (int a = 0; a < 9; ++a)
#pragma unroll
      for (int b = a; b < 9; ++b)
        if (b < MD) { dst[e * KSP] = xt[a] * xt[b]; ++e; }
    dst[NP * KSP] = 0.0;
  }
#pragma unroll
  for (int u = 0; u < PGS_KS / 32; ++u) {
    const int il = ilg + 32 * u;
    if (il < nst) sB[ccg * KSP + (il & 3) * KQ + (il >> 2)] = vb[u];
  }
  TSTAMP0(c, 41);
  lds_barrier();
  TSTAMP0(c, 42);
  constexpr int NW = PG_THREADS / 64;
  const int wave = tid >> 6, lane = tid & 63, lr = lane & 15, kq = lane >> 4;
  const int ntl = __builtin_amdgcn_readfirstlane(max(0, min(PGS_TMAX, (d.RT - wave + NW - 1) / NW)));
  int o1[PGS_TMAX], o2[PGS_TMAX];
#pragma unroll
  for (int q = 0; q < PGS_TMAX; ++q) {
    const int row = (wave + NW * q) * 16 + lr;
    o1[q] = o2[q] = NP;
    if (q < ntl && row < d.R) { const int zz = row / d.NCC; o1[q] = zz; o2[q] = NZZ + (row - zz * d.NCC); }
  }
  double4_t acc[PGS_TMAX];
#pragma unroll
  for (int q = 0; q < PGS_TMAX; ++q) acc[q] = double4_t{0.0, 0.0, 0.0, 0.0};
  switch (ntl) {
    case 1: pg_solo_tiles<1>(sP, sB, KSP, KQ, nchunk, o1, o2, lr, kq, acc); break;
    case 2: pg_solo_tiles<2>(sP, sB, KSP, KQ, nchunk, o1, o2, lr, kq, acc); break;
    case 3: pg_solo_tiles<3>(sP, sB, KSP, KQ, nchunk, o1, o2, lr, kq, acc); break;
    case 4: pg_solo_tiles<4>(sP, sB, KSP, KQ, nchunk, o1, o2, lr, kq, acc); break;
    default: break;
  }
#pragma unroll
  for (int q = 0; q < PGS_TMAX; ++q)
    if (q < ntl) {
      double* out = c0.pg_part + ((size_t)ks * d.NT + (size_t)(wave + NW * q) * d.CTG + ct) * 256 + lane;
      __builtin_nontemporal_store(acc[q][0], out); __builtin_nontemporal_store(acc[q][1], out + 64);
      __builtin_nontemporal_store(acc[q][2], out + 128); __builtin_nontemporal_store(acc[q][3], out + 192);
    }
  TSTAMP0(c, 44);
}

constexpr int PG_SOLO_S = 4;
constexpr int PG_SOLO_LL = 8;
constexpr int PGS_SU = PGS_KS / (PG_THREADS / 32);

__device__ inline void pg_solo_s(const Ctx& c0, int KS, int ks, double* smem) {
  const Dims& d = c0.d;
  const int n = d.n, K = d.K, MD = d.MD, tid = threadIdx.x;
  const int i0 = ks * KS;
  const int nlive = min(KS, n - i0);
  const int nchunk = (nlive + 15) >> 4;
  const int nst = nchunk * 16;
  const int KSP = KS + 2, KQ = KS >> 2;
  const int ncol = d.CTS * 16;
  double* sB = smem;
  double* sS = sB + ncol * KSP;
  const bool wl = tid < nlive;
  const int iw = i0 + tid;
  double z[4], x[8];
  pg_solo_load_zx(c0, wl, iw, z, x);
  const int sh = (d.CTS == 1) ? 4 : 5;
  const int cc = tid & (ncol - 1), ilg = tid >> sh, ilstep = PG_THREADS >> sh;
  const bool colok = cc < d.P;
  const double* src = c0.rec + (size_t)i0 * d.LREC + min(d.LG + cc, d.LREC - 1);
  double vb[PGS_SU];
#pragma unroll
  for (int u = 0; u < PGS_SU; ++u) {
    const int il = ilg + ilstep * u;
    vb[u] = (il < nlive && colok) ? src[(size_t)il * d.LREC] : 0.0;
  }
  if (tid < nst) {
    double* dst = sS + (tid & 3) * KQ + (tid >> 2);
    const double xt[9] = {1.0, x[0], x[1], x[2], x[3], x[4], x[5], x[6], x[7]};
#pragma unroll
    for (int a = 0; a < 4; ++a)
#pragma unroll
      for (int m = 0; m < 9; ++m)
        if (a < K && m < MD) dst[(a * MD + m) * KSP] = z[a] * xt[m];
    dst[d.A * KSP] = 0.0;
  }
#pragma unroll
  for (int u = 0; u < PGS_SU; ++u) {
    const int il = ilg + ilstep * u;
    if (il < nst) sB[cc * KSP + (il & 3) * KQ + (il >> 2)] = vb[u];
  }
  lds_barrier();
  const int wave = __builtin_amdgcn_readfirstlane(tid >> 6), lane = tid & 63, lr = lane & 15, kq = lane >> 4;
  if (wave >= d.AT * d.CTS) return;
  const int at = wave / d.CTS, cs = wave - at * d.CTS;
  const int row = at * 16 + lr;
  const v2d* pa = (const v2d*)(sS + (row < d.A ? row : d.A) * KSP + kq * KQ);
  const v2d* pc = (const v2d*)(sB + (cs * 16 + lr) * KSP + kq * KQ);
  struct Ops { v2d a[2], c[2]; };
  auto load = [&](Ops& o, int t) { o.a[0] = pa[2 * t]; o.c[0] = pc[2 * t]; o.a[1] = pa[2 * t + 1]; o.c[1] = pc[2 * t + 1]; };
  double4_t acc = double4_t{0.0, 0.0, 0.0, 0.0};
  auto mfma = [&](const Ops& o) {
#pragma unroll
    for (int u = 0; u < 2; ++u) {
      acc = __builtin_amdgcn_mfma_f64_16x16x4f64(o.a[u].x, o.c[u].x, acc, 0, 0, 0);
      acc = __builtin_amdgcn_mfma_f64_16x16x4f64(o.a[u].y, o.c[u].y, acc, 0, 0, 0);
    }
  };
  Ops s0, s1;
  load(s0, 0);
  for (int t = 0; t < nchunk; t += 2) {
    if (t + 1 < nchunk) load(s1, t + 1);
    __builtin_amdgcn_sched_barrier(0);
    mfma(s0);
    __builtin_amdgcn_sched_barrier(0);
    if (t + 2 < nchunk) load(s0, t + 2);
    __builtin_amdgcn_sched_barrier(0);
    if (t + 1 < nchunk) mfma(s1);
    __builtin_amdgcn_sched_barrier(0);
  }
  double* out = c0.pg_part + ((size_t)ks * d.NT + (size_t)d.RT * d.CTG + wave) * 256 + lane;
  __builtin_nontemporal_store(acc[0], out); __builtin_nontemporal_store(acc[1], out + 64);
  __builtin_nontemporal_store(acc[2], out + 128); __builtin_nontemporal_store(acc[3], out + 192);
}

template <bool BATCH, bool GROUPS>
__global__ __launch_bounds__(PG_THREADS) void k_pair_gram(Ctx c0, int KS, int nks, int do_pg, int G) {
  const int nch = BATCH ? c0.nch : 1;
  TIMELINE(c0, 1);
#ifdef BFMMM_TIMELINE
  const int wgid = blockIdx.x + gridDim.x * blockIdx.y;
  if (threadIdx.x == 0 && wgid < 1024) {
    unsigned id, hw;
    asm volatile("s_getreg_b32 %0, hwreg(HW_REG_XCC_ID)" : "=s"(id));
    asm volatile("s_getreg_b32 %0, hwreg(HW_REG_HW_ID)" : "=s"(hw));
    g_wgtrace[3 * wgid] = wall_clock64();
    g_wgtrace[3 * wgid + 1] = ((unsigned long long)(id & 0xf) << 32) | hw;
  }
  struct EndTrace { int w; __device__ ~EndTrace() { if (threadIdx.x == 0 && w < 1024) g_wgtrace[3 * w + 2] = wall_clock64(); } } et_{wgid};
#endif
  extern __shared__ __attribute__((aligned(16))) double smem[];
  const Dims& d = c0.d;
  const int n = d.n, K = d.K, MD = d.MD;
  const int ks = blockIdx.y, ct = blockIdx.x;
  if (ct == d.CTG + 1) {
    if (ks < nch && threadIdx.x < 256) {
      const Ctx c = chain_ctx(c0, (unsigned)ks);
      job_pi_alpha(c, BATCH || !(do_pg & PG_SOLO_LL), c0.zrec != nullptr);
      TSTAMP(c, 46);
    } else if (ks >= nch && ks < 2 * nch && threadIdx.x < 256) {
      const Ctx c = chain_ctx(c0, (unsigned)(ks - nch));
      if (c.dyn->hyper_pending) {
        job_hyper(c, false);
        __syncthreads();
        if (threadIdx.x == 0) c.dyn->hyper_pending = 0u;
      }
    } else if (!BATCH && (do_pg & PG_SOLO_LL) && ks == 2 * nch && threadIdx.x < 256) {
      if (c0.dyn->ll_pending) deferred_loglik(c0, smem);
    }
    return;
  }
  if (ks >= nks) return;
  if (!do_pg) return;
  const bool single = ct == d.CTG;
  if constexpr (!BATCH) {
    if ((do_pg & PG_SOLO) && !single) { pg_solo_g(c0, KS, ks, ct, smem); return; }
    if ((do_pg & PG_SOLO_S) && single) { pg_solo_s(c0, KS, ks, smem); return; }
  }
  const int ncol = single ? d.CTS * 16 : 16;
  const int col0 = single ? d.LG : ct * 16;
  const int colend = single ? d.LG + d.P : d.LG;
  const int i0 = ks * KS;
  const int RS = K + MD + 1, ONE = K;
  const int NP = d.NZZ + d.NCC, RP = NP + 1;
  const int KSP = KS + 2;
  const int KQ4 = KS >> 2;
  auto pos = [&](int il) { return (il & 3) * KQ4 + (il >> 2); };
  const int GG = GROUPS ? G : 1;
  const int TB = RS + (single ? 0 : RP);
  double* sB = smem;
  double* sW = sB + (size_t)ncol * KSP;
  double* sP = sW + (size_t)RS * KSP;
  const int tid = threadIdx.x;
  constexpr int UW = 12, UB = 6;
  const int ncw = K + MD - 1;
  const int nB = KS * ncol;
  auto loadW = [&](const double* Zq, const double* chiq, int il0, int cb, double (&v)[UW]) {
    const int i = min(i0 + il0 + tid, n - 1);
#pragma unroll
    for (int u = 0; u < UW; ++u) {
      const int col = min(cb + u, ncw - 1);
      v[u] = (col < K) ? Zq[i + (size_t)n * col] : chiq[i + (size_t)n * (col - K)];
    }
  };
  auto storeW = [&](int il0, int cb, const double (&v)[UW]) {
    const int il = il0 + tid;
    if (il >= KS) return;
    const bool live = i0 + il < n;
#pragma unroll
    for (int u = 0; u < UW; ++u) {
      const int col = cb + u;
      if (col < ncw) sW[((col < K) ? col : col + 1) * KSP + pos(il)] = live ? v[u] : 0.0;
    }
    if (cb == 0) { sW[ONE * KSP + il] = 1.0; sW[(K + MD) * KSP + il] = 0.0; }
  };
  auto loadB = [&](const double* stilq, int base, double (&v)[UB]) {
#pragma unroll
    for (int u = 0; u < UB; ++u) {
      const int q = min(base + tid + PG_THREADS * u, nB - 1);
      const int il = q / ncol, cc = q - il * ncol;
      const int i = min(i0 + il, n - 1), col = min(col0 + cc, d.LREC - 1);
      v[u] = (d.D > 0) ? stilq[(size_t)i * d.P + min(cc, d.P - 1)] : c0.rec[(size_t)i * d.LREC + col];
    }
  };
  auto storeB = [&](int base, const double (&v)[UB]) {
#pragma unroll
    for (int u = 0; u < UB; ++u) {
      const int q = base + tid + PG_THREADS * u;
      if (q < nB) {
        const int il = q / ncol, cc = q - il * ncol;
        sB[cc * KSP + pos(il)] = (i0 + il < n && col0 + cc < colend) ? v[u] : 0.0;
      }
    }
  };
  const int ccg = tid & 15, ilg = tid >> 4;
  const double* srcg = c0.rec + min(col0 + ccg, d.LREC - 1);
  const bool colok = col0 + ccg < colend;
  auto loadG = [&](int ub0, double (&v)[UB]) {
#pragma unroll
    for (int u = 0; u < UB; ++u) v[u] = srcg[(size_t)min(i0 + ilg + (PG_THREADS / 16) * (ub0 + u), n - 1) * d.LREC];
  };
  auto storeG = [&](int ub0, const double (&v)[UB]) {
#pragma unroll
    for (int u = 0; u < UB; ++u) {
      const int il = ilg + (PG_THREADS / 16) * (ub0 + u);
      if (il < KS) sB[ccg * KSP + pos(il)] = (i0 + il < n && colok) ? v[u] : 0.0;
    }
  };
  int* ptab = (int*)(sW + (size_t)GG * TB * KSP);
  if (!single && tid < NP) {
    int e = tid, off = 0, dim = K;
    if (e >= d.NZZ) { e -= d.NZZ; off = K; dim = MD; }
    int a = 0;
    while (e >= dim - a) { e -= dim - a; ++a; }
    ptab[tid] = (off + a) | ((off + a + e) << 16);
  }
  const bool shared_cols = !(single && d.D > 0);
  for (int q = 0; q < nch; q += GG) {
    const int gc = GROUPS ? min(GG, nch - q) : 1;
    const size_t off1 = (size_t)q * c0.chain_bytes;
    const double* Zq = ptr_shift(c0.Z, off1);
    const double* chiq = ptr_shift(c0.chi, off1);
    const double* stilq = ptr_shift(c0.stil, (size_t)q * c0.chain_bytes_cov);
#ifdef BFMMM_TIMELINE
    struct { Dyn* dyn; } c = {ptr_shift(c0.dyn, off1)};
#endif
    {
      TSTAMP0(c, 40);
      double vw[UW], vb[UB];
      const bool stage_cols = (q == 0) || !shared_cols;
      const int nitem = gc * ncw * KS;
      constexpr bool grp = GROUPS;
      if (grp) {
#pragma unroll
        for (int u = 0; u < UW; ++u) {
          const int e = min(tid + PG_THREADS * u, nitem - 1);
          const int ci = e / KS, il = e - ci * KS;
          const int g = ci / ncw, col = ci - g * ncw;
          const int i = min(i0 + il, n - 1);
          const size_t offg = (size_t)g * c0.chain_bytes;
          vw[u] = (col < K) ? ptr_shift(Zq, offg)[i + (size_t)n * col] : ptr_shift(chiq, offg)[i + (size_t)n * (col - K)];
        }
      } else {
        loadW(Zq, chiq, 0, 0, vw);
      }
      if (stage_cols) { if (single) loadB(stilq, 0, vb); else loadG(0, vb); }
      TSTAMP0(c, 47);
      if (grp) {
#pragma unroll
        for (int u = 0; u < UW; ++u) {
          const int e = tid + PG_THREADS * u;
          if (e < nitem) {
            const int ci = e / KS, il = e - ci * KS;
            const int g = ci / ncw, col = ci - g * ncw;
            sW[((size_t)g * TB + ((col < K) ? col : col + 1)) * KSP + pos(il)] = (i0 + il < n) ? vw[u] : 0.0;
          }
        }
        for (int x = tid; x < gc * KS; x += PG_THREADS) {
          const int g = x / KS, il = x - g * KS;
          sW[((size_t)g * TB + ONE) * KSP + il] = 1.0; sW[((size_t)g * TB + K + MD) * KSP + il] = 0.0;
        }
      } else {
        storeW(0, 0, vw);
      }
      TSTAMP0(c, 48);
      if (stage_cols) { if (single) storeB(0, vb); else storeG(0, vb); }
      if (!grp)
// ... 306 lines not shown
        b[u][1] = *(const v2d*)(sB + il * PGP_RB + 32);
      }
#pragma unroll
      for (int u = 0; u < 2; ++u) {
        acc[0] = __builtin_amdgcn_mfma_f64_16x16x4f64(a[u], b[u][0].x, acc[0], 0, 0, 0);
        acc[1] = __builtin_amdgcn_mfma_f64_16x16x4f64(a[u], b[u][0].y, acc[1], 0, 0, 0);
        acc[2] = __builtin_amdgcn_mfma_f64_16x16x4f64(a[u], b[u][1].x, acc[2], 0, 0, 0);
        acc[3] = __builtin_amdgcn_mfma_f64_16x16x4f64(a[u], b[u][1].y, acc[3], 0, 0, 0);
      }
    }
  };
  load_chunk(0);
  store_chunk(0, 0);
  __syncthreads();
  for (int t = 0; t < nchunk; ++t) {
    if (t + 1 < nchunk) load_chunk(t + 1);
    mfma_chunk(t & 1);
    if (t + 1 < nchunk) store_chunk(t + 1, (t + 1) & 1);
    __syncthreads();
  }
  if (!has_tile) return;
  double* out0 = pack + (size_t)ks * g.NTP * 256 + lane;
#pragma unroll
  for (int x = 0; x < 4; ++x) {
    const int tp = 2 * cg + (x >> 1);
    const bool keep = single ? (x < 2) : (tp < g.NP2);
    if (keep) {
      const int idx = single ? g.TG * 2 * g.NP2 + tile * 2 + x : (tile * g.NP2 + tp) * 2 + (x & 1);
      double* out = out0 + (size_t)idx * 256;
      out[0] = acc[x][0]; out[64] = acc[x][1]; out[128] = acc[x][2]; out[192] = acc[x][3];
    }
  }
}

__global__ __launch_bounds__(256) void k_pg_reduce_pack(Ctx c0, PgPack g, const double* __restrict__ pack) {
  const Dims& d = c0.d;
  const int bx = blockIdx.x;
  const int gid4 = bx * 256 + threadIdx.x;
  const int gid = gid4 >> 2, gl = gid4 & 3;
  const bool live = gid < g.NTP * 256;
  const int gc = live ? gid : 0;
  const int t = gc >> 8, q = gc & 255;
  const int r = q >> 6, lane = q & 63;
  const int rit = (lane >> 4) + 4 * r, cit = lane & 15;
  const double* src = pack + (size_t)t * 256 + q;
  const size_t stride = (size_t)g.NTP * 256;
  const int NKS = g.NKS;
  double sg = 0.0;
  const int nfull = NKS & ~3;
  for (int k0 = gl; k0 < nfull; k0 += 32) {
    double v8[8];
#pragma unroll
    for (int u = 0; u < 8; ++u) v8[u] = src[(size_t)min(k0 + 4 * u, NKS - 1) * stride];
#pragma unroll
    for (int u = 0; u < 8; ++u) if (k0 + 4 * u < nfull) sg += v8[u];
  }
  {
    double vt[3];
#pragma unroll
    for (int u = 0; u < 3; ++u) vt[u] = src[(size_t)min(nfull + u, NKS - 1) * stride];
#pragma unroll
    for (int u = 0; u < 3; ++u) if (gl == 0 && nfull + u < NKS) sg += vt[u];
  }
  const double s01 = sg + __shfl_xor(sg, 1, 4);
  const double s = s01 + __shfl_xor(s01, 2, 4);
  if (!live || gl != 0) return;
  const int NACC = 2 * g.NP2;
  if (t < g.TG * NACC) {
    const int tile = t / NACC, x = t - tile * NACC;
    const int grow = tile * 16 + rit;
    const int qc = grow / d.R, row = grow - qc * d.R;
    const int col = 32 * (x >> 1) + 2 * cit + (x & 1);
    if (qc < c0.nch && col < d.LG) {
      const size_t off = (size_t)qc * c0.chain_bytes;
      ptr_shift(c0.H, off)[(size_t)row * d.LG + col] = s;
      const int dd = col / d.P, p0 = col - dd * d.P, W = 2 * d.BW + 2;
      double* h2 = ptr_shift(c0.H2, off) + (size_t)row * d.P * W;
      h2[h2_index(d.P, p0, d.BW + dd)] = s;
      if (dd > 0 && p0 + dd < d.P) h2[h2_index(d.P, p0 + dd, d.BW - dd)] = s;
    }
  } else {
    const int t2 = t - g.TG * NACC;
    const int tile = t2 >> 1, par = t2 & 1;
    const int grow = tile * 16 + rit;
    const int qc = grow / d.A, a = grow - qc * d.A;
    const int p = 2 * cit + par;
    if (qc < c0.nch && p < d.P) ptr_shift(c0.tvec, (size_t)qc * c0.chain_bytes)[(size_t)a * d.P + p] = s;
  }
}

void pg_geometry(const Dims& d, int& NKS, int& KS) {
  const int row_g = (d.K + d.MD + 1) + 16 + (d.NZZ + d.NCC + 1);
  const int row_s = (d.K + d.MD + 1) + d.CTS * 16;
  const int ks_cap = std::max(16, (int)((96 * 1024) / (sizeof(double) * (size_t)std::max(row_g, row_s)) - 2) / 16 * 16);
  NKS = std::max(1, std::min(256 / (d.CTG + 2), d.n / 16));
  KS = (d.n + NKS - 1) / NKS;
  KS = (KS + 15) / 16 * 16;
  KS = std::min(KS, ks_cap);
  NKS = (d.n + KS - 1) / KS;
}

static size_t pair_gram_lds_bytes(const Dims& d, int KS, int G) {
  const int RS = d.K + d.MD + 1, RP = d.NZZ + d.NCC + 1;
  const size_t tables = (size_t)(KS + 2) * std::max(16 + G * (RS + RP), d.CTS * 16 + G * RS) + 128;
  return std::max(tables, (size_t)std::max(PI_ALPHA_LDS_DOUBLES, HYPER_LDS_DOUBLES)) * sizeof(double);
}

static size_t pgp_lds_bytes(const PgPack& g) {
  const size_t lg = 2 * (16 * (size_t)PGP_RB + (size_t)g.NQG * 16 * g.SLS), ls = 2 * (16 * (size_t)PGP_RB + (size_t)g.NQS * 16 * g.SLS);
  return std::max(lg, ls) * sizeof(double);
}
static bool pgp_geometry(const Dims& d, int nch, int KS, int NKS, PgPack& g) {
  if (d.mv || d.D > 0 || d.K > 4 || d.MD - 1 > 8 || d.P > 32 || (d.LREC & 1) || (KS & 15)) return false;
  g.KS = KS; g.NKS = NKS;
  g.NP2 = (d.LG + 31) / 32;
  g.TG = (nch * d.R + 15) / 16; g.TS = (nch * d.A + 15) / 16;
  g.WPG = PGP_WPG;
  g.NRG = (g.TG + PGP_WPG - 1) / PGP_WPG; g.NCG = (g.NP2 + 1) / 2; g.NWG_S = (g.TS + PGP_WPG - 1) / PGP_WPG;
  g.SLG = (d.NZZ + d.NCC + 1 + 1) & ~1; g.SLS = (d.K + d.MD + 1 + 1) & ~1;
  g.NQG = std::min(nch, (PGP_WPG * 16 + d.R - 2) / d.R + 1); g.NQS = std::min(nch, (PGP_WPG * 16 + d.A - 2) / d.A + 1);
  g.NTP = g.TG * 2 * g.NP2 + g.TS * 2;
  const int NV = d.K + d.MD - 1;
  if (std::max(g.NQG, g.NQS) * NV * 16 > PGP_NWV * 64 * PGP_WPG) return false;
  return pgp_lds_bytes(g) <= 64 * 1024;
}
size_t pgp_pack_doubles(const PgPack& g) { return (size_t)g.NKS * g.NTP * 256; }

PgRoute pg_route_decide(const Dims& d, int nch_handle, int nch, bool pg, bool defer_loglik, size_t pg_part_doubles, bool may_pack) {
  PgRoute r;
  pg_geometry(d, r.NKS, r.KS);
  const int KSl = ((d.n + 127) / 128 + 15) / 16 * 16, NKSl = (d.n + KSl - 1) / KSl;
  const bool long_set = d.n > 16384 && pgp_geometry(d, 1, KSl, NKSl, r.pk);
  if (long_set) { r.KS = KSl; r.NKS = NKSl; }
  if (may_pack && pg && (long_set || nch_handle >= 4) && pgp_geometry(d, nch, r.KS, r.NKS, r.pk)) {
    r.packed = true;
    r.lds = pgp_lds_bytes(r.pk);
    return r;
  }
  if (long_set && (pair_gram_lds_bytes(d, r.KS, 1) > 160 * 1024 || (size_t)r.NKS * d.NT * 256 > pg_part_doubles))
    pg_geometry(d, r.NKS, r.KS);
  const int ncw = d.K + d.MD - 1;
  r.G = 1;
  if (nch > 1 && d.D == 0 && d.RT < 8)
    while (r.G < nch && pair_gram_lds_bytes(d, r.KS, r.G + 1) <= 144 * 1024 && (size_t)(r.G + 1) * ncw * r.KS <= 12 * 512) ++r.G;
  r.body = nch > 1 ? (r.G > 1 ? 3 : 2) : (g_solo_pair_gram && pg_solo_fits(d, r.KS)) ? 1 : 0;
  r.lds = pair_gram_lds_bytes(d, r.KS, r.G);
  if (pg && r.body == 1) {
    if (g_solo_pair_gram_tail) {
      if (d.AT * d.CTS <= PG_THREADS / 64 && d.CTS <= 2) r.tail |= PG_SOLO_S;
      if (defer_loglik && r.NKS >= 3) r.tail |= PG_SOLO_LL;
    }
    r.do_pg = PG_SOLO | r.tail;
    if (r.tail & PG_SOLO_S) r.lds = std::max(r.lds, (size_t)(r.KS + 2) * (d.CTS * 16 + d.A + 1) * sizeof(double));
  } else {
    r.do_pg = pg ? 1 : 0;
  }
  return r;
}

bool pg_route_solo_ll(const PgRoute& r) { return !r.packed && r.body <= 1 && (r.do_pg & PG_SOLO_LL) != 0; }

void launch_pair_gram(const Ctx& c, const PgRoute& r, hipStream_t st) {
  const Dims& d = c.d;
  if (r.body == 3) hipLaunchKernelGGL((k_pair_gram<true, true>), dim3(d.CTG + 2, r.do_pg ? std::max(r.NKS, c.nch) : c.nch, 1), dim3(PG_THREADS), r.lds, st, c, r.KS, r.NKS, r.do_pg, r.G);
  else if (r.body == 2) hipLaunchKernelGGL((k_pair_gram<true, false>), dim3(d.CTG + 2, r.do_pg ? std::max(r.NKS, c.nch) : c.nch, 1), dim3(PG_THREADS), r.lds, st, c, r.KS, r.NKS, r.do_pg, 1);
  else hipLaunchKernelGGL((k_pair_gram<false, false>), dim3(d.CTG + 2, r.do_pg ? r.NKS : 1, 1), dim3(PG_THREADS), r.lds, st, c, r.KS, r.NKS, r.do_pg, 1);
}

void launch_pair_gram_pack(const Ctx& c, const PgRoute& r, hipStream_t st) {
  const PgPack& g = r.pk;
  const dim3 grid(g.NRG * g.NCG + g.NWG_S, g.NKS, 1);
  hipLaunchKernelGGL(k_pair_gram_pack<PGP_WPG>, grid, dim3(64 * PGP_WPG), r.lds, st, c, g, r.pack);
  const int nblk_red = (g.NTP * 256 * 4 + 255) / 256;
  hipLaunchKernelGGL(k_pg_reduce_pack, dim3(nblk_red), dim3(256), 0, st, c, g, r.pack);
}

void launch_pg_reduce(const Ctx& c, int NKS, hipStream_t st) {
  const int nthreads = c.d.NT * 256 * 4;
  hipLaunchKernelGGL(k_pg_reduce, dim3((nthreads + 255) / 256, 1, c.nch), dim3(256), 0, st, c, NKS);
}

void prepare_pair_gram_kernels() {
  set_max_lds((const void*)k_pair_gram<false, false>); set_max_lds((const void*)k_pair_gram<true, false>); set_max_lds((const void*)k_pair_gram<true, true>);
}

}
```

bayesfmmm_amd/csrc/launchers.hpp:

```cpp
#pragma once
#include "model.hpp"
#include <string>

long long diag_row_max();
size_t diag_row_ws_doubles(int C, int S);
std::string diag_launch(const double* d_x, long long rows, int C, int S, double* d_out, long long ld_out, double* ws, long long ws_rows,
                        hipStream_t st);
std::string diag_gather(const double* base, size_t chain_bytes, long long ss, long long ps, int first, int S, int C, int p0, int P,
                        double* ws, hipStream_t st);

int post_psis_device(const double* d_ll, long long ld, int n, int S, double* const out[6]);
int post_psis_expect_device(const double* d_ll, long long ld, int n, int S, const double* d_aux, int n_aux, long long aux_stride,
                            double* const out[6], double* expect_host);

int post_stacking_device(double* d_L, long long n, int Q, const double* init, int max_iter, int check_every, double tol, double* weights,
                         double* pointwise, double* objective, double* gap, int* n_iter, int* converged);
void post_stacking_geometry(int* threads, int* max_workgroups);

namespace bfmmm {

int launch_stats_functional(int degree, int n, int P, int LREC, const int64_t* off, const double* t, const double* y,
                            const double* knots, int n_knots, double* rec, int* ni, double* B_dense, int* err,
                            hipStream_t st);
void launch_stats_multivariate(int n, int P, int LREC, const double* Y, double* rec, int* ni, hipStream_t st);
void launch_stats_totals(int n, int LREC, int yy_off, const double* rec, const int* ni, double* out_yy,
                         long long* out_counts, hipStream_t st);

struct CurveRoute {
  int which = 0;
  int BW = -1;
  int LPC = 0;
  bool COV = false;
  int KT = 0;
  bool LEAN = false, KEX = false;
  bool SMALL = false;
  int KX = 0, MX = 0;
  int nblk = 0;
  size_t lds = 0;
};
CurveRoute curve_route_decide(const Dims& d, int which, int arg);
int launch_curve(const Ctx& c, int which, int do_update, hipStream_t st);
int curve_blocks(int n, int P);
void prepare_curve_kernels();

struct PgRoute {
  bool packed = false;
  int KS = 0, NKS = 0;
  int body = -1;
  int G = 0;
  int tail = 0;
  int do_pg = 0;
  size_t lds = 0;
  PgPack pk;
  double* pack = nullptr;
};
void pg_geometry(const Dims& d, int& NKS, int& KS);
PgRoute pg_route_decide(const Dims& d, int nch_handle, int nch, bool pg, bool defer_loglik, size_t pg_part_doubles, bool may_pack);
bool pg_route_solo_ll(const PgRoute& r);
size_t pgp_pack_doubles(const PgPack& g);
void launch_pair_gram(const Ctx& c, const PgRoute& r, hipStream_t st);
void launch_pg_reduce(const Ctx& c, int NKS, hipStream_t st);
void launch_pair_gram_pack(const Ctx& c, const PgRoute& r, hipStream_t st);
void prepare_pair_gram_kernels();

void launch_factor(const Ctx& c, hipStream_t st);
void prepare_factor_kernels();

struct SweepRoute {
  int kernel = -1;
  int targ = 0;
  int direct = 0;
  int threads = 0;
  size_t lds = 0;
};
SweepRoute sweep_route_decide(const Dims& d);
int launch_sweep(const Ctx& c, hipStream_t st);
void launch_sweep_tables(const Ctx& c, hipStream_t st);
size_t sweep_tab_ints(int A);
void launch_loglik(const Ctx& c, int use_rss_part, int r_stored, hipStream_t st);
void launch_loglik_flush(const Ctx& c, hipStream_t st, uint32_t* status_out);
void launch_fill_slots(const Ctx& c, double* chain, const double* cur, size_t len, int s0, int s1, hipStream_t st);
void prepare_sweep_kernels();

struct CovRoute {
  int BW = 0;
  int LPC = 0;
  int DX = 0;
  int W2D = 0;
  int PP = 0;
  int NB2 = 0, NBS = 0, NPG = 0;
  int launches = 0;
  bool do_eta = false, do_xi = false;
  size_t lds_group = 0;
};
CovRoute cov_route_decide(const Ctx& c);
void launch_cov_block(const Ctx& c, hipStream_t st);
int cov_step_blocks(int nblk_curve);
int cov_w2_chunks(int n);
void prepare_cov_kernels();
bool cov_block_fits(const Ctx& c);

std::string launch_chain_curve_ll(const Ctx& c, int first_slot, int n_slots, int i0, int rows, double* out, hipStream_t st);

std::string launch_slot_rss(const Ctx& c, int first_slot, int n_slots, int i0, int rows, double* part, hipStream_t st);
std::string launch_slot_ll_reduce(const Ctx& c, int first_slot, int n_slots, int i0, int rows, int per_curve, int store, double* part,
                                  double* acc, hipStream_t st);

constexpr int LP_ROWS = 64;
struct LpTile { int32_t curve, rows; int64_t y0, b0, out_row; };
std::string loo_pointwise_check(const Ctx& c);
std::string launch_loo_pointwise(const Ctx& c, const LpTile* tiles, long long n_tiles, const double* B, const double* y, int first_slot,
                                 int n_slots, double* out, size_t out_stride, hipStream_t st);
std::string launch_loo_pointwise_var(const double* mean, double* second, size_t count, hipStream_t st);

struct LbRow { int64_t b; int32_t obs; int16_t bpos, blen; };
struct LbTile { int32_t curve, rows; int64_t y0, row0; };
std::string loo_blocks_check(const Ctx& c);
std::string launch_loo_blocks(const Ctx& c, const LbTile* tiles, long long n_tiles, const LbRow* rows, const double* B, const double* y,
                              int first_slot, int n_slots, double* out, size_t out_stride, hipStream_t st);

struct FitCall {
  int which = 0, G = 0, first_slot = 0, n_slots = 0;
  const double* E = nullptr;
  const int* curves = nullptr;
  double* tab = nullptr;
};
long long fit_directions(const Dims& d, int which);
int fit_lds_rows();
std::string fit_check(const Ctx& c, const FitCall& f);
std::string launch_fit_project(const Ctx& c, const FitCall& f, hipStream_t st);
std::string launch_fit_rows(const Ctx& c, const FitCall& f, int r0, int rows, const double* probs, int nq, double* mean, double* sd,
                            double* quant, hipStream_t st);
std::string launch_fit_values(const Ctx& c, const FitCall& f, int r0, int rows, double* out, hipStream_t st);
std::string launch_fit_quantiles(const double* W, int NP, int T, long long ncol, const double* probs, int nq, double* quant, hipStream_t st);
int fit_sim_gmax();
std::string launch_fit_sim(const Ctx& c, const FitCall& f, int r0, int rows, double p, double* mean, double* sd, double* crit, double* lower,
                           double* upper, double* cw, hipStream_t st);
std::string launch_fit_sim_band(const double* mean, const double* sd, const double* crit, int G, int rows, double* lower, double* upper,
                                hipStream_t st);

std::string launch_similarity(const Ctx& c, int first_slot, int n_slots, const int* curves, int r0, int rows, double* mean, double* sd,
                              double* chain_mean, hipStream_t st);
extern int g_similarity_block;
long long similarity_loss_blocks(int n);
std::string launch_similarity_loss(const Ctx& c, int first_slot, int n_slots, long long b0, long long nb, double* partial, hipStream_t st);
std::string launch_similarity_loss_reduce(const Ctx& c, int first_slot, int n_slots, long long b0, long long nb, const double* partial,
                                          double* loss, hipStream_t st);

std::string launch_align_gram(const Ctx& c, const double* Zref, int first_slot, int n_slots, int32_t* perm, double* score, hipStream_t st);
std::string launch_align_gather(const double* base, size_t chain_bytes, long long ss, long long ps, int first, int S, int C, int p0, int P,
                                const int32_t* perm, int K, long long inner, double* ws, hipStream_t st);
std::string launch_align_project(const Ctx& c, const double* E, int G, const int32_t* perm, int first_slot, int n_slots, int r0, int rows,
                                 double* V, hipStream_t st);

std::string launch_rescale_transform(const Ctx& c, const int32_t* perm, const double* given, int first_slot, int n_slots, double* mix,
                                     double* mix_inv, int32_t* curve, double* rcond, double* z_min, int32_t* singular_flag, hipStream_t st);
std::string launch_rescale_gather(const double* base, size_t chain_bytes, long long ss, long long ps, int first, int S, int C, int p0, int P,
                                  const double* W, int sk, int sc, int K, long long inner, double* ws, hipStream_t st);
std::string launch_rescale_project(const Ctx& c, const double* E, int G, const double* mix, const double* x, int first_slot, int n_slots,
                                   int r0, int rows, double* V, hipStream_t st);

struct CovCall {
  int G1 = 0, G2 = 0, diagonal = 0, first_slot = 0, n_slots = 0;
  const double *E1 = nullptr, *E2 = nullptr;
  const int* curves = nullptr;
  double *tab1 = nullptr, *tab2 = nullptr;
};
std::string cov_check(const Ctx& c, const CovCall& f);
size_t cov_table_doubles(const Ctx& c, const CovCall& f, int which);
std::string launch_cov_project(const Ctx& c, const CovCall& f, hipStream_t st);
std::string launch_curve_cov(const Ctx& c, const CovCall& f, int r0, int rows, double* mean, double* sd, double* chain_mean, hipStream_t st);

struct CcovCall {
  int G1 = 0, G2 = 0, diagonal = 0, first_slot = 0, n_slots = 0;
  long long n_pairs = 0;
  const double *E1 = nullptr, *E2 = nullptr, *x = nullptr;
  const int32_t *perm = nullptr, *pairs = nullptr;
  const double* mix = nullptr;
  double *tab1 = nullptr, *tab2 = nullptr;
};
std::string ccov_check(const Ctx& c, const CcovCall& f);
size_t ccov_table_doubles(const Ctx& c, const CcovCall& f, int which);
std::string launch_ccov_project(const Ctx& c, const CcovCall& f, hipStream_t st);
std::string launch_ccov_values(const Ctx& c, const CcovCall& f, long long r0, long long rows, double* V, hipStream_t st);
std::string launch_ccov_maxdev(const CcovCall& f, long long N, long long r0, long long rows, const double* V, const double* mean,
                               const double* sd, double* dev, hipStream_t st);
int ccov_sort_rows();
std::string launch_ccov_crit(const double* dev, long long N, long long m, double p, double* crit, hipStream_t st);

struct ContrastCall {
  int G = 0, R = 0, first_slot = 0, n_slots = 0;
  const double *E = nullptr, *mix = nullptr, *w_nu = nullptr, *w_eta = nullptr, *w = nullptr;
  double* tab = nullptr;
};
std::string contrast_check(const Ctx& c, const ContrastCall& f);
std::string launch_contrast_coef(const Ctx& c, const ContrastCall& f, hipStream_t st);
std::string launch_contrast_values(const Ctx& c, const ContrastCall& f, long long r0, long long rows, double* V, hipStream_t st);
std::string launch_contrast_norm(const Ctx& c, const ContrastCall& f, long long r0, long long rows, const double* V, double* acc, hipStream_t st);
std::string launch_rows_count(const double* V, long long N, long long rows, const double* thr, int ge, int32_t* count, hipStream_t st);

struct CeigCall {
  int G = 0, J = 0, first_slot = 0, n_slots = 0;
  const double *E = nullptr, *w = nullptr, *x = nullptr, *ref = nullptr;
  const int32_t* perm = nullptr;
// ... 60 lines not shown
```

bayesfmmm_amd/csrc/model.hpp:

```cpp
#pragma once
#include <hip/hip_runtime.h>
#include <stdint.h>

namespace bfmmm {

constexpr int KMAX = 8;
constexpr int PMAX = 64;
constexpr int BWMAX = 5;
constexpr int BWWIDE = 31;
constexpr int BWMID = 15;

enum : uint32_t {
  U_Z = 1u << 0, U_PI = 1u << 1, U_ALPHA3 = 1u << 2, U_PHI = 1u << 3, U_DELTA = 1u << 4, U_A = 1u << 5,
  U_GAMMA = 1u << 6, U_NU = 1u << 7, U_TAU = 1u << 8, U_SIGMA = 1u << 9, U_CHI = 1u << 10,
  U_ETA = 1u << 11, U_TAU_ETA = 1u << 12, U_XI = 1u << 13, U_DELTA_XI = 1u << 14, U_A_XI = 1u << 15,
  U_GAMMA_XI = 1u << 16, U_LOGLIK = 1u << 17
};

struct Hyper {
  double c[KMAX];
  double b, nu_1;
  double alpha1l, alpha2l, beta1l, beta2l;
  double a_Z_PM, a_pi_PM, var_alpha3, var_epsilon1, var_epsilon2;
  double alpha_nu, beta_nu, alpha_eta, beta_eta, alpha_0, beta_0;
};

struct Dyn {
  uint32_t iter;
  uint32_t slot;
  uint32_t tt_step;
  uint32_t status;
  uint32_t iter_hyper;
  uint32_t slot_hyper;
  int32_t pend_dir;
  uint32_t ll_pending;
  uint32_t ll_slot;
  uint32_t ll_use_part;
  uint32_t zprep_valid, zprep_iter, zprep_tt, zprep_chain;
  uint32_t znorm_valid, znorm_iter, znorm_tt;
  uint32_t piprep_valid, piprep_iter;
  uint32_t slot_base;
  unsigned long long zprep_seed;
  double beta;
  double sigma2;
  double alpha3;
  double rss;
  double loglik;
  double pi[KMAX];
  double tau[KMAX];
  uint32_t pi_done;
  uint32_t hyper_pending;
  unsigned long long stamps[64];
};

struct DynHead {
  uint32_t iter, slot, tt_step, status, iter_hyper, slot_hyper;
  int32_t pend_dir;
  uint32_t ll_pending, ll_slot, ll_use_part;
  uint32_t zprep_valid, zprep_iter, zprep_tt, zprep_chain;
  uint32_t znorm_valid, znorm_iter, znorm_tt;
  uint32_t piprep_valid, piprep_iter;
  uint32_t slot_base;
  unsigned long long zprep_seed;
  double beta, sigma2, alpha3;
};
static_assert(sizeof(DynHead) == 112, "DynHead is seven 16-byte loads");
static_assert(offsetof(Dyn, zprep_seed) == offsetof(DynHead, zprep_seed) && offsetof(Dyn, alpha3) == offsetof(DynHead, alpha3) &&
              offsetof(Dyn, slot_base) == offsetof(DynHead, slot_base), "DynHead mirrors the head of Dyn");

#if defined(__HIPCC__)
__device__ __forceinline__ DynHead dyn_head(const Dyn* dyn) {
  union U { DynHead h; int4 q[7]; __device__ U() {} } u;
  const int4* p = reinterpret_cast<const int4*>(dyn);
#pragma unroll
  for (int j = 0; j < 7; ++j) u.q[j] = p[j];
  return u.h;
}
#endif

constexpr int DYN_LDS_DOUBLES = 24;
static_assert(offsetof(Dyn, pi) == 128 && sizeof(double) * KMAX == 64, "dwords 0 .. 47 of Dyn: head, rss, loglik, pi");
#if defined(__HIPCC__)
__device__ __forceinline__ uint32_t dyn_head_fetch(const Dyn* dyn) {
  return reinterpret_cast<const uint32_t*>(dyn)[min((int)(threadIdx.x & 63), 47)];
}
__device__ __forceinline__ void dyn_head_stage(double* sDyn, uint32_t w) {
  reinterpret_cast<uint32_t*>(sDyn)[min((int)(threadIdx.x & 63), 47)] = w;
}
__device__ __forceinline__ DynHead dyn_head_lds(const double* sDyn) {
  union U { DynHead h; int4 q[7]; __device__ U() {} } u;
  const int4* p = reinterpret_cast<const int4*>(sDyn);
#pragma unroll
  for (int j = 0; j < 7; ++j) u.q[j] = p[j];
  return u.h;
}
__device__ __forceinline__ const double* dyn_pi_lds(const double* sDyn) { return sDyn + 16; }
#endif

struct Dims {
  int n, K, P, M, D;
  int BW;
  int BWP;
  int LG;
  int LREC;
  int MD;
  int A;
  int NZZ, NCC, R;
  int RT, AT;
  int CTG, CTS;
  int NT;
  int NWG;
  int mv;
  int64_t n_obs_total;
  int64_t half_sum;
};

constexpr int ZREC_SCALARS = 6;
__host__ __device__ inline size_t zrec_stride(int n, int K) { return (size_t)(ZREC_SCALARS + K) * n + 2; }
constexpr int GSTD_SPARE = 7, GSTD_REC = 2;
static_assert(GSTD_REC <= GSTD_SPARE, "the recorded acceptance values live in the spare doubles of gstd");
__host__ __device__ inline size_t gstd_used(int K, int P, int M) { return (size_t)K * P * M + (size_t)K * M + 13 * (size_t)K + 1; }
__host__ __device__ inline size_t gstd_doubles(int K, int P, int M) { return gstd_used(K, P, M) + GSTD_SPARE; }

struct Ctx {
  Dims d;
  Hyper h;
  uint64_t seed;
  uint32_t chain;
  uint32_t mask;
  int T;
  Dyn* dyn;
  const double* rec;
  const int* ni;
  double* Z;
  double* chi;
  double* theta;
  double* delta;
  double* Aa;
  double* gamma;
  double* logz_part;
  double* rss_part;
  double* pg_part;
  double* H;
  double* H2;
  double* tvec;
  double* rvec;
  double* hq;
  double* Lz;
  double* gstd;
  double* zprep;
  double* chi_norm;
  double* piprep;
  double* Cmat;
  const double* Pmat;
  const int* sweep_tab;
  const double* X;
  double* thetaX;
  double* tau_eta;
  double* gamma_xi;
  double* delta_xi;
  double* A_xi;
  double* stil;
  double* yyp_part;
  double* cfull;
  double* gfull;
  double* w2_part;
  double* H2aa;
  double* gstd2;
  double* Wdir;
  double* C2;
  double* Lz2;
  double* step_part;
  double* thetaN;
  double* delta_cur;
  int pi_in_factor;
  int defer_loglik;
  int defer_hyper;
  int ll_use_part;
  int covariance_adj;
  int A2;
  int NB2, NBS;
  int NPG, NPAIR;
  double *c_eta, *c_xi, *c_tau_eta, *c_gamma_xi, *c_delta_xi, *c_A_xi;
  double YY;
  size_t chain_bytes, chain_bytes_cov;
  uint32_t chain_id_stride;
  int nch;
  double *c_nu, *c_chi, *c_Z, *c_pi, *c_alpha3, *c_delta, *c_A, *c_sigma, *c_tau, *c_gamma, *c_Phi, *c_loglik;
  int nblk_curve;
  double* zrec;
};

struct PgPack {
  int KS, NKS;
  int TG, TS;
  int NRG, NCG, NWG_S;
  int SLG, SLS;
  int NQG, NQS;
  int WPG;
  int NTP;
  int NP2;
};

#define BFMMM_CHAIN_PTRS(X_)                                                                                         \
  X_(dyn) X_(Z) X_(chi) X_(theta) X_(delta) X_(Aa) X_(gamma) X_(logz_part) X_(rss_part) X_(pg_part) X_(H) X_(H2)       \
  X_(tvec) X_(rvec) X_(hq) X_(Lz) X_(gstd) X_(zprep) X_(chi_norm) X_(zrec) X_(piprep) X_(Cmat)                        \
  X_(c_nu) X_(c_chi) X_(c_Z) X_(c_pi) X_(c_alpha3) X_(c_delta) X_(c_A) X_(c_sigma) X_(c_tau) X_(c_gamma) X_(c_Phi) X_(c_loglik)
#define BFMMM_CHAIN_PTRS_COV(X_)                                                                                     \
  X_(thetaX) X_(tau_eta) X_(gamma_xi) X_(delta_xi) X_(A_xi) X_(stil) X_(yyp_part) X_(cfull) X_(gfull) X_(w2_part)      \
  X_(H2aa) X_(gstd2) X_(Wdir) X_(C2) X_(Lz2) X_(step_part) X_(thetaN) X_(delta_cur)                                   \
  X_(c_eta) X_(c_xi) X_(c_tau_eta) X_(c_gamma_xi) X_(c_delta_xi) X_(c_A_xi)

template <typename T>
__host__ __device__ inline T* ptr_shift(T* p, size_t bytes) { return (T*)((char*)p + bytes); }

__host__ __device__ inline Ctx chain_ctx(const Ctx& c0, unsigned q) {
  Ctx c = c0;
  const size_t o1 = (size_t)q * c0.chain_bytes, o2 = (size_t)q * c0.chain_bytes_cov;
#define X_(f) c.f = ptr_shift(c0.f, o1);
  BFMMM_CHAIN_PTRS(X_)
#undef X_
#define X_(f) c.f = ptr_shift(c0.f, o2);
  BFMMM_CHAIN_PTRS_COV(X_)
#undef X_
  c.chain = c0.chain + q * c0.chain_id_stride;
  return c;
}
#ifdef __HIPCC__
__device__ inline Ctx chain_view(const Ctx& c0) { return chain_ctx(c0, blockIdx.z); }
#endif

extern int g_exact_instances;
extern int g_curve_record;
extern int g_solo_pair_gram;
extern int g_solo_pair_gram_tail;

__host__ __device__ inline int tri_index(int n, int a, int b) {
  return a * n - (a * (a - 1)) / 2 + (b - a);
}

#ifdef BFMMM_TIMELINE
struct Timeline {
  unsigned long long* s; int k;
  __device__ Timeline(const Ctx& c, int k_) : s(c.dyn->stamps), k(k_) {
    if (blockIdx.x == 0 && blockIdx.y == 0 && threadIdx.x == 0) s[2 * k] = wall_clock64();
    if (threadIdx.x == 0) atomicMax(&s[16 + k], (unsigned long long)wall_clock64());
  }
  __device__ ~Timeline() { if (threadIdx.x == 0) atomicMax(&s[2 * k + 1], (unsigned long long)wall_clock64()); }
};
#define TIMELINE(c, k) Timeline tl_((c), (k))
#define TSTAMP(c, i) do { if (threadIdx.x == 0) atomicMax(&(c).dyn->stamps[i], (unsigned long long)wall_clock64()); } while (0)
#define TSTAMP0(c, i) do { if (threadIdx.x == 0 && blockIdx.x == 0 && blockIdx.y == 0) (c).dyn->stamps[i] = wall_clock64(); } while (0)
#else
#define TIMELINE(c, k) do { } while (0)
#define TSTAMP(c, i) do { } while (0)
#define TSTAMP0(c, i) do { } while (0)
#endif

typedef double double4_t __attribute__((ext_vector_type(4)));
typedef double v2d __attribute__((ext_vector_type(2)));

template <int CTRL>
__device__ inline double dpp_add(double v) {
  const int lo = __builtin_amdgcn_update_dpp(0, __double2loint(v), CTRL, 0xf, 0xf, true);
  const int hi = __builtin_amdgcn_update_dpp(0, __double2hiint(v), CTRL, 0xf, 0xf, true);
  return v + __hiloint2double(hi, lo);
}
__device__ inline double row16_sum(double v) {
  v = dpp_add<0xB1>(v);
  v = dpp_add<0x4E>(v);
  v = dpp_add<0x141>(v);
  v = dpp_add<0x140>(v);
  return v;
}

template <int LPC>
__device__ inline double group_sum(double v) {
  v = row16_sum(v);
  v += __shfl_xor(v, 16, 64);
  if (LPC == 64) v += __shfl_xor(v, 32, 64);
  return v;
}

template <int UN>
__device__ inline void copy_to_lds(double* dst, const double* __restrict__ src, int count, int tid, int nthreads) {
  for (int base = 0; base < count; base += nthreads * UN) {
    double v[UN];
#pragma unroll
    for (int u = 0; u < UN; ++u) v[u] = src[min(base + tid + nthreads * u, count - 1)];
#pragma unroll
    for (int u = 0; u < UN; ++u) {
      const int idx = base + tid + nthreads * u;
      if (idx < count) dst[idx] = v[u];
    }
  }
}

inline void set_max_lds(const void* fn) {
  hipFuncAttributes at;
  if (hipFuncGetAttributes(&at, fn) != hipSuccess) { (void)hipGetLastError(); return; }
  const int room = 160 * 1024 - (int)at.sharedSizeBytes;
  if (hipFuncSetAttribute(fn, hipFuncAttributeMaxDynamicSharedMemorySize, room) != hipSuccess) (void)hipGetLastError();
}

}
```

bayesfmmm_amd/csrc/scalar_jobs.hpp:

```cpp
#pragma once
#include "model.hpp"
#include "rng.hpp"

namespace bfmmm {

__device__ inline double block_sum256(double v, double* scratch) {
  __syncthreads();
  scratch[threadIdx.x] = v;
  __syncthreads();
  for (int o = 128; o > 0; o >>= 1) {
    if ((int)threadIdx.x < o) scratch[threadIdx.x] += scratch[threadIdx.x + o];
    __syncthreads();
  }
  const double r = scratch[0];
  __syncthreads();
  return r;
}

__device__ inline double logGamma_ref(double x) { return log(tgamma(x)); }

__device__ inline void deferred_loglik(const Ctx& c, double* red) {
  Dyn* dyn = c.dyn;
  const int tid = threadIdx.x;
  double rss = dyn->rss;
// ... 47 lines not shown
#pragma unroll
  for (int k = 0; k < KMAX; ++k) if (k < K) gsum += t.g[k];
#pragma unroll
  for (int k = 0; k < KMAX; ++k) { pi_old[k] = (k < K) ? dyn->pi[k] : 0.0; pi_new[k] = (k < K) ? t.g[k] / gsum : 0.0; }
  const double a3_ph = t.ph_s[0];
  if (tid < 6 * K + 6) {
    const bool is_sum = tid >= 6 * K;
    const int row = is_sum ? tid - 6 * K : tid / K, k = is_sum ? 0 : tid - row * K;
    const double sc = (row < 2) ? c.h.a_pi_PM : ((row < 4) ? alpha3 : a3_ph);
    double arg = 0.0;
#pragma unroll
    for (int k2 = 0; k2 < KMAX; ++k2)
      if (k2 < K) {
        const double term = sc * ((row & 1) ? pi_new[k2] : pi_old[k2]);
        if (is_sum) arg += term;
        else if (k2 == k) arg = term;
      }
    t.lg[tid] = lgamma_pos(arg);
  } else if (tid >= 64 && tid < 64 + 2 * K) {
    const int e = tid - 64;
    double arg = 1.0;
#pragma unroll
    for (int k = 0; k < KMAX; ++k) { if (k < K && e == k) arg = pi_old[k]; if (k < K && e == K + k) arg = pi_new[k]; }
    t.lp[e] = log(arg);
  } else if (tid == 128 || tid == 129) {
    t.dt[tid - 128] = (tid == 128) ? dtruncnorm_lo_log(a3_ph, a3_ph, sd, 0.0) : dtruncnorm_lo_log(alpha3, alpha3, sd, 0.0);
  }
  __syncthreads();
}

__device__ inline void job_pi_prepare(const Ctx& c) {
  extern __shared__ __attribute__((aligned(16))) double smem[];
  Dyn* dyn = c.dyn;
  const PiAlphaTabs t = pi_alpha_layout(smem);
  pi_alpha_tables(c, make_key(c.seed, c.chain, dyn->iter + 1u, 0u), t);
  for (int e = threadIdx.x; e < PI_TAB_DOUBLES; e += 256) c.piprep[e] = smem[e];
  if (threadIdx.x == 0) { dyn->piprep_iter = dyn->iter + 1u; dyn->zprep_chain = c.chain; dyn->zprep_seed = c.seed; dyn->piprep_valid = 1u; }
}

__device__ inline void job_pi_alpha(const Ctx& c, bool loglik = true, bool rec = false) {
  extern __shared__ __attribute__((aligned(16))) double smem[];
  double (*red)[256] = (double (*)[256])smem;
  double* S = smem + KMAX * 256;
  const PiAlphaTabs t = pi_alpha_layout(S + KMAX);
  double *g = t.g, *lg = t.lg, *ph_s = t.ph_s, *lu = t.lu, *lp = t.lp, *dt = t.dt;
  const Dims& d = c.d;
  const int K = d.K, n = d.n, tid = threadIdx.x;
  Dyn* dyn = c.dyn;
  const uint32_t mask = c.mask;
  if (loglik && dyn->ll_pending) deferred_loglik(c, smem);
  if (!(mask & (U_PI | U_ALPHA3))) {
    if (tid == 0) {
      c.c_alpha3[dyn->slot] = dyn->alpha3;
      for (int k = 0; k < K; ++k) c.c_pi[(size_t)dyn->slot * K + k] = dyn->pi[k];
    }
    return;
  }
  const bool pre = dyn->piprep_valid && dyn->piprep_iter == dyn->iter && dyn->tt_step == 0 &&
                   dyn->zprep_chain == c.chain && dyn->zprep_seed == c.seed;
  if (rec && tid == 0) c.zrec[zrec_stride(n, K) - 1] = pre ? 1.0 : 0.0;
  if (pre) {
    for (int e = tid; e < PI_TAB_DOUBLES; e += 256) t.g[e] = c.piprep[e];
  } else {
    pi_alpha_tables(c, make_key(c.seed, c.chain, dyn->iter, dyn->tt_step), t);
  }
  {
    double acc[KMAX];
#pragma unroll
    for (int k = 0; k < KMAX; ++k) acc[k] = 0.0;
    const int per = (c.nblk_curve + 255) / 256;
    for (int b = tid * per; b < min(c.nblk_curve, (tid + 1) * per); ++b)
#pragma unroll
      for (int k = 0; k < KMAX; ++k)
        if (k < K) acc[k] += c.logz_part[(size_t)b * K + k];
#pragma unroll
    for (int k = 0; k < KMAX; ++k) red[k][tid] = acc[k];
    __syncthreads();
    for (int o = 128; o > 0; o >>= 1) {
      if (tid < o)
#pragma unroll
        for (int k = 0; k < KMAX; ++k)
          if (k < K) red[k][tid] += red[k][tid + o];
      __syncthreads();
    }
    if (tid < K) S[tid] = red[tid][0];
  }
  __syncthreads();
  double alpha3 = dyn->alpha3;
  double pi_old[KMAX], pi_new[KMAX];
  double gsum = 0.0;
#pragma unroll
  for (int k = 0; k < KMAX; ++k) if (k < K) gsum += g[k];
#pragma unroll
  for (int k = 0; k < KMAX; ++k) { pi_old[k] = (k < K) ? dyn->pi[k] : 0.0; pi_new[k] = (k < K) ? g[k] / gsum : 0.0; }
  const double a3_ph = ph_s[0];
  if (tid == 0) {
    auto lB = [&](int row) {
      double s = 0.0;
      for (int k = 0; k < K; ++k) s += lg[row * K + k];
      return s - lg[6 * K + row];
    };
    double pi[KMAX];
#pragma unroll
    for (int k = 0; k < KMAX; ++k) pi[k] = pi_old[k];
    int pi_is_new = 0;
    double* acc_rec = c.gstd + gstd_used(K, d.P, d.M);
    if (mask & U_PI) {
      double lpdf_new = 0.0, lpdf_old = 0.0, pn = 0.0, po = 0.0;
#pragma unroll
      for (int k = 0; k < KMAX; ++k)
        if (k < K) {
          const double lo = lp[k], ln = lp[K + k];
          lpdf_new += (c.h.c[k] - 1) * ln + ((alpha3 * pi_new[k]) - 1) * S[k];
          lpdf_old += (c.h.c[k] - 1) * lo + ((alpha3 * pi_old[k]) - 1) * S[k];
          pn += (c.h.a_pi_PM * pi_old[k] - 1) * ln;
          po += (c.h.a_pi_PM * pi_new[k] - 1) * lo;
        }
      lpdf_new -= n * lB(3);
      lpdf_old -= n * lB(2);
      const double lpn = pn - lB(0);
      const double lpo = po - lB(1);
      const double acc = lpdf_new - lpdf_old + lpo - lpn;
      if (rec) acc_rec[0] = acc;
      if (lu[0] < acc) {
        pi_is_new = 1;
#pragma unroll
        for (int k = 0; k < KMAX; ++k) pi[k] = pi_new[k];
      }
#pragma unroll
      for (int k = 0; k < KMAX; ++k) if (k < K) dyn->pi[k] = pi[k];
    }
    if (mask & U_ALPHA3) {
      double l_old = (-c.h.b) * alpha3, l_new = (-c.h.b) * a3_ph;
#pragma unroll
      for (int k = 0; k < KMAX; ++k)
        if (k < K) {
          l_old += ((alpha3 * pi[k]) - 1) * S[k];
          l_new += ((a3_ph * pi[k]) - 1) * S[k];
        }
      l_old -= n * lB(2 + pi_is_new);
      l_new -= n * lB(4 + pi_is_new);
      l_old += dt[0];
      l_new += dt[1];
      if (rec) acc_rec[1] = l_new - l_old;
      if (lu[1] < l_new - l_old) alpha3 = a3_ph;
      dyn->alpha3 = alpha3;
    }
    c.c_alpha3[dyn->slot] = dyn->alpha3;
    for (int k = 0; k < K; ++k) c.c_pi[(size_t)dyn->slot * K + k] = dyn->pi[k];
  }
}

__device__ inline int hyper_gstd_count(const Dims& d) { return d.K * d.P * d.M + d.K * d.M + d.K + 4 * d.K; }

__device__ inline void job_hyper_draws(const Ctx& c, int first) {
  const Dims& d = c.d;
  const int P = d.P, K = d.K, M = d.M;
  const Dyn* dyn = c.dyn;
  const RngKey key = make_key(c.seed, c.chain, dyn->iter, dyn->tt_step);
  const int nG = K * P * M;
  const int e = first + threadIdx.x;
  if (e > hyper_gstd_count(d) + 8 * K) return;
  double v;
  if (e > hyper_gstd_count(d)) {
    const int x = e - hyper_gstd_count(d) - 1, cell = x >> 2, q = x & 3;
    const int j = cell / 2, i = cell - 2 * j;
    const double sd = (i == 0) ? (c.h.var_epsilon1 / c.h.beta1l) : (c.h.var_epsilon2 / c.h.beta2l);
    const double cur = c.Aa[j + (size_t)K * i];
    const double na = rtruncnorm_lo(key, UPD_A_PROP, (uint32_t)(j * 2 + i), cur, sd, 0.0);
    const double a = (q < 2) ? cur : na;
    v = (q & 1) ? log(a) : logGamma_ref(a);
  } else if (e == hyper_gstd_count(d)) {
    const bool tempered = (dyn->tt_step != 0);
    double shape = tempered ? (dyn->beta * (double)d.n_obs_total) / 2 : (d.mv ? (double)(d.n_obs_total / 2) : (double)d.half_sum);
    shape += c.h.alpha_0;
    v = rgamma(key, UPD_SIGMA, 0, shape, 1.0);
  } else if (e < nG) {
    v = rgamma(key, UPD_GAMMA, (uint32_t)e, (c.h.nu_1 + 1) / 2, 1.0);
  } else if (e < nG + K * M) {
    const int q = e - nG, k = q / M, i = q - k * M;
    const double param1 = (i == 0) ? c.Aa[k] + ((P * M) / 2.0) : c.Aa[k + (size_t)K] + ((P * (M - i)) / 2.0);
    v = rgamma(key, UPD_DELTA, (uint32_t)(k * M + i), param1, 1.0);
  } else if (e < nG + K * M + K) {
    const int k = e - nG - K * M;
    v = rgamma(key, UPD_TAU, (uint32_t)k, c.h.alpha_nu + (P / 2), 1.0);
  } else if (e < nG + K * M + K + 2 * K) {
    const int cell = e - nG - K * M - K, j = cell / 2, i = cell - 2 * j;
    const double sd = (i == 0) ? (c.h.var_epsilon1 / c.h.beta1l) : (c.h.var_epsilon2 / c.h.beta2l);
    v = rtruncnorm_lo(key, UPD_A_PROP, (uint32_t)(j * 2 + i), c.Aa[j + (size_t)K * i], sd, 0.0);
  } else {
    const int cell = e - nG - K * M - K - 2 * K;
    v = runif(key, UPD_A_ACC, (uint32_t)cell);
  }
  c.gstd[e] = v;
}

constexpr int HYPER_LDS_DOUBLES = 5 * KMAX * 16 + KMAX * 2 * 6 + KMAX + 2 + 2 * KMAX * PMAX + (2 * BWMAX + 1) * PMAX;

template <int MT>
__device__ inline void delta_recursion(double* dk, const double* sk, const double* gd, double* tp, int M, bool do_delta) {
  double dv[MT], sv[MT], gv[MT];
#pragma unroll
  for (int m = 0; m < MT; ++m) { const int mc = min(m, M - 1); dv[m] = dk[mc]; sv[m] = sk[mc]; gv[m] = gd[mc]; }
  if (do_delta) {
    double pre = 1.0;
#pragma unroll
    for (int i = 0; i < MT; ++i)
      if (i < M) {
        double tt = pre;
        double param2 = 1.0 + 0.5 * tt * sv[i];
#pragma unroll
        for (int m = i + 1; m < MT; ++m)
          if (m < M) { tt *= dv[m]; param2 += 0.5 * tt * sv[m]; }
        dv[i] = gv[i] * (1.0 / param2);
        pre *= dv[i];
      }
  }
  double tt = 1.0;
#pragma unroll
  for (int m = 0; m < MT; ++m)
    if (m < M) { tt *= dv[m]; tp[m] = tt; dk[m] = dv[m]; }
}

__device__ inline void job_hyper_counters(const Ctx& c) {
  Dyn* dyn = c.dyn;
  if (c.defer_loglik && threadIdx.x == 0) {
    dyn->ll_slot = dyn->slot_hyper;
    dyn->ll_use_part = (uint32_t)c.ll_use_part;
    dyn->ll_pending = 1u;
    dyn->iter = dyn->iter_hyper + 1u;
    dyn->slot = dyn->iter_hyper + 1u - dyn->slot_base;
  }
}

__device__ inline void job_hyper(const Ctx& c, bool counters = true) {
  extern __shared__ __attribute__((aligned(16))) double smem[];
  double* Skm = smem;
  double* dl = Skm + KMAX * 16;
  double* lgd = dl + KMAX * 16;
  double* tpre = lgd + KMAX * 16;
  double* gDs = tpre + KMAX * 16;
  double* aw = gDs + KMAX * 16;
  double* slog = aw + KMAX * 2 * 6;
  double* qrow = slog + KMAX + 2;
  double* snu = qrow + KMAX * PMAX;
  double* sPb = snu + KMAX * PMAX;
  const Dims& d = c.d;
  const int P = d.P, K = d.K, M = d.M, MD = d.MD, tid = threadIdx.x;
  Dyn* dyn = c.dyn;
  const uint32_t mask = c.mask;
  const bool phi_on = MD > 1;
  const bool do_delta = (mask & U_DELTA) && phi_on, do_A = (mask & U_A) && phi_on, do_gamma = (mask & U_GAMMA) && phi_on;
  const bool do_tau = (mask & U_TAU) != 0;
  const int Mc = max(M, 1);
  const int nG = K * P * M, nGc = max(nG, 1);
  const double* gGam = c.gstd;
  const double* gD = c.gstd + nG;
  const double* gT = gD + K * M;
  const double* aProp = gT + K;
  const double* aUnif = aProp + 2 * K;
  const double* aTerm = c.gstd + hyper_gstd_count(d) + 1;
  const uint32_t slot = dyn->slot_hyper;
  double s_ph[8], s_gm[8];
  {
    const int km = min(tid >> 3, max(K * M - 1, 0)), q = tid & 7;
    const int k = km / Mc, m = km - k * Mc;
#pragma unroll
    for (int u = 0; u < 8; ++u) {
      const int p = min(q + 8 * u, P - 1);
      s_ph[u] = c.theta[(size_t)(k * (M + 1) + min(m + 1, M)) * P + p];
      s_gm[u] = c.gamma[min(k + K * (p + P * m), nGc - 1)];
    }
  }
  const int KP = K * P;
  const int e0 = min(tid, KP - 1), k0 = e0 / P, p0 = e0 - k0 * P;
  const double nu0 = c.theta[(size_t)(k0 * (M + 1)) * P + p0];
  const int e1 = min(tid + 256, KP - 1), k1 = e1 / P, p1 = e1 - k1 * P;
  const double nu1 = c.theta[(size_t)(k1 * (M + 1)) * P + p1];
  const int kmc = min(tid, max(K * M - 1, 0)), kd = kmc / Mc, md = kmc - kd * Mc;
  const double dl0 = c.delta[kd + (size_t)K * md];
  const double gd0 = gD[kmc];
  constexpr int NPB = ((2 * BWMAX + 1) * PMAX + 255) / 256;
  double pb[NPB];
#pragma unroll
  for (int r = 0; r < NPB; ++r) {
    const int idx = min(tid + 256 * r, (2 * BWMAX + 1) * P - 1), u = idx / P, p = idx - u * P;
    pb[r] = c.Pmat[p + (size_t)P * min(max(p - d.BWP + u, 0), P - 1)];
  }
  const int cellT = min(tid >> 2, 2 * K - 1), jobT = tid & 3, jT = cellT / 2, iT = cellT - 2 * jT;
  const double curT = c.Aa[jT + (size_t)K * iT], naT = aProp[cellT];
  const double lgaT = aTerm[cellT * 4 + 2 * (jobT & 1)], laT = aTerm[cellT * 4 + 2 * (jobT & 1) + 1];
  const int cellA = min(tid, 2 * K - 1), idxA = (cellA >> 1) + K * (cellA & 1);
  const double curA = c.Aa[idxA], naA = aProp[cellA], unA = aUnif[cellA];
  const int kt = min(max(tid - 32, 0), K - 1);
  const double tau_old = dyn->tau[kt], gTk = gT[kt];
  constexpr int GU = 3;
  double g_std[GU], g_phi[GU];
#pragma unroll
  for (int u = 0; u < GU; ++u) {
    const int e = min(tid + 256 * u, nGc - 1);
    const int jj = e % Mc, il = e / Mc, l = il % P, i = il / P;
    g_std[u] = gGam[e];
    g_phi[u] = c.theta[(size_t)(i * (M + 1) + min(jj + 1, M)) * P + l];
  }
  if (do_delta) {
    {
      const int km = tid >> 3, q = tid & 7;
      const bool on = km < K * M;
      double acc = 0.0;
      double pr[8];
#pragma unroll
      for (int u = 0; u < 8; ++u) pr[u] = (on && q + 8 * u < P) ? s_gm[u] * (s_ph[u] * s_ph[u]) : 0.0;
#pragma unroll
      for (int u = 0; u < 8; ++u) acc += pr[u];
      acc = dpp_add<0xB1>(acc);
      acc = dpp_add<0x4E>(acc);
      acc = dpp_add<0x141>(acc);
      if (on && q == 0) Skm[km] = acc;
    }
    for (int g0 = 32; g0 < K * M; g0 += 32) {
      const int km = g0 + (tid >> 3), q = tid & 7;
      const bool on = km < K * M;
      const int k = on ? km / M : 0, m = on ? km - k * M : 0;
      double pr[8];
#pragma unroll
      for (int u = 0; u < 8; ++u) {
        const int p = min(q + 8 * u, P - 1);
        const double ph = c.theta[(size_t)(k * (M + 1) + m + 1) * P + p];
        const double gm = c.gamma[k + (size_t)K * (p + (size_t)P * m)];
        pr[u] = (on && q + 8 * u < P) ? gm * (ph * ph) : 0.0;
      }
      double acc = 0.0;
#pragma unroll
      for (int u = 0; u < 8; ++u) acc += pr[u];
      acc = dpp_add<0xB1>(acc);
      acc = dpp_add<0x4E>(acc);
      acc = dpp_add<0x141>(acc);
      if (on && q == 0) Skm[km] = acc;
    }
  }
  if (do_tau) {
    if (tid < KP) snu[tid] = nu0;
    if (tid + 256 < KP) snu[tid + 256] = nu1;
  }
  if (tid < K * M && tid < KMAX * 16) { dl[kd * 16 + md] = dl0; gDs[kd * 16 + md] = gd0; }
#pragma unroll
  for (int r = 0; r < NPB; ++r)
    if (tid + 256 * r < (2 * BWMAX + 1) * P) sPb[tid + 256 * r] = pb[r];
  __syncthreads();
  if (do_tau)
    for (int e = tid; e < KP; e += 256) {
      const int k = e / P, p = e - k * P;
      double s = 0.0;
      if (d.mv) s = snu[e];
      else if (d.BWP > BWMAX) {
        for (int q = 0; q < P; ++q) s += c.Pmat[p + (size_t)P * q] * snu[k * P + q];
      } else {
#pragma unroll
        for (int u = 0; u < 2 * BWMAX + 1; ++u) {
          const int q = p - d.BWP + u;
          if (u <= 2 * d.BWP && q >= 0 && q < P) s += sPb[u * P + p] * snu[k * P + q];
        }
      }
      qrow[e] = snu[e] * s;
    }
  if (tid < K && M > 0) {
    if (M <= 8) delta_recursion<8>(dl + tid * 16, Skm + tid * M, gDs + tid * 16, tpre + tid * 16, M, do_delta);
    else {
      double* dk = dl + tid * 16;
      const double* sk = Skm + tid * M;
      if (do_delta) {
        double pre = 1.0;
        for (int i = 0; i < M; ++i) {
          double tt = pre;
          double param2 = 1.0 + 0.5 * tt * sk[i];
          for (int m = i + 1; m < M; ++m) { tt *= dk[m]; param2 += 0.5 * tt * sk[m]; }
          dk[i] = gDs[tid * 16 + i] * (1.0 / param2);
          pre *= dk[i];
        }
      }
      double tt = 1.0;
      for (int m = 0; m < M; ++m) { tt *= dk[m]; tpre[tid * 16 + m] = tt; }
    }
  }
  __syncthreads();
  if (tid >= 32 && tid < 32 + K) {
    const int k = tid - 32;
    double tv = tau_old;
    if (do_tau) {
      double qf = 0.0;
      for (int p = 0; p < P; ++p) qf += qrow[k * P + p];
      const double b = c.h.beta_nu + (0.5 * qf);
      const double gg = gTk * (1.0 / b);
      tv = d.mv ? (1.0 / gg) : gg;
      dyn->tau[k] = tv;
    }
    c.c_tau[slot + (size_t)c.T * k] = tv;
  }
  if (tid < K * M) {
    const double dv = dl[kd * 16 + md];
    if (do_delta) c.delta[kd + (size_t)K * md] = dv;
    c.c_delta[(size_t)slot * K * M + kd + (size_t)K * md] = dv;
    lgd[kd * 16 + md] = log(dv);
  }
  double* s_gam = c.c_gamma + (size_t)slot * K * P * M;
  if (do_gamma) {
#pragma unroll
    for (int u = 0; u < GU; ++u) {
      const int e = tid + 256 * u;
      if (e < nG) {
        const int jj = e % M, il = e / M, l = il % P, i = il / P;
        const double ph = tpre[i * 16 + jj];
        const double phi = g_phi[u];
        const double gnew = g_std[u] * (2 / (c.h.nu_1 + ph * (phi * phi)));
        const size_t at = i + (size_t)K * (l + (size_t)P * jj);
        c.gamma[at] = gnew;
        s_gam[at] = gnew;
      }
    }
    for (int e = tid + 256 * GU; e < nG; e += 256) {
      const int jj = e % M, il = e / M, l = il % P, i = il / P;
      const double ph = tpre[i * 16 + jj];
      const double phi = c.theta[(size_t)(i * (M + 1) + jj + 1) * P + l];
      const double gnew = gGam[e] * (2 / (c.h.nu_1 + ph * (phi * phi)));
      const size_t at = i + (size_t)K * (l + (size_t)P * jj);
      c.gamma[at] = gnew;
      s_gam[at] = gnew;
    }
  } else {
    for (int e = tid; e < nG; e += 256) s_gam[e] = c.gamma[e];
  }
  __syncthreads();
  if (do_A && tid < K * 2 * 4) {
    const int cell = tid >> 2, job = tid & 3;
    const int j = jT;
    const bool first = (iT == 0);
    const double sd = first ? (c.h.var_epsilon1 / c.h.beta1l) : (c.h.var_epsilon2 / c.h.beta2l);
    const double cur = curT, na = naT;
    double v;
    if (job < 2) {
      const double a = (job == 0) ? cur : na;
      const double lga = lgaT, la = laT;
      if (first) v = -lga + (a - 1) * lgd[j * 16] + (c.h.alpha1l - 1) * la - (a * c.h.beta1l);
      else {
        double sl = 0.0;
        for (int q = 1; q < M; ++q) sl += lgd[j * 16 + q];
        const double x = M - 1;
        v = -x * lga + (c.h.alpha2l - 1) * la - (a * c.h.beta2l) + (a - 1) * sl;
      }
    } else {
      v = (job == 2) ? dtruncnorm_lo_log(cur, na, sd, 0.0) : dtruncnorm_lo_log(na, cur, sd, 0.0);
    }
    aw[cell * 6 + 1 + job] = v;
  }
  __syncthreads();
  if (tid < K * 2) {
    double av = curA;
    if (do_A) {
      const double* w = aw + tid * 6;
      const double acc = (w[2] + w[3]) - w[1] - w[4];
      if (log(unA) < acc) { av = naA; c.Aa[idxA] = naA; }
    }
    c.c_A[(size_t)slot * K * 2 + idxA] = av;
  }
  if (counters) job_hyper_counters(c);
}

}
```

include/bfmmm.h:

```cpp
#ifndef BFMMM_H
#define BFMMM_H

#include <stdint.h>

#ifdef __cplusplus
extern "C" {
#endif

typedef struct bfmmm_handle bfmmm_handle;

enum { BFMMM_MODEL_FUNCTIONAL = 0, BFMMM_MODEL_MULTIVARIATE = 1 };

enum {
  BFMMM_U_Z = 1 << 0, BFMMM_U_PI = 1 << 1, BFMMM_U_ALPHA3 = 1 << 2, BFMMM_U_PHI = 1 << 3,
  BFMMM_U_DELTA = 1 << 4, BFMMM_U_A = 1 << 5, BFMMM_U_GAMMA = 1 << 6, BFMMM_U_NU = 1 << 7,
  BFMMM_U_TAU = 1 << 8, BFMMM_U_SIGMA = 1 << 9, BFMMM_U_CHI = 1 << 10,
  BFMMM_U_ETA = 1 << 11, BFMMM_U_TAU_ETA = 1 << 12, BFMMM_U_XI = 1 << 13, BFMMM_U_DELTA_XI = 1 << 14,
  BFMMM_U_A_XI = 1 << 15, BFMMM_U_GAMMA_XI = 1 << 16, BFMMM_U_LOGLIK = 1 << 17
};
#define BFMMM_SWEEP_NU_Z  (BFMMM_U_Z | BFMMM_U_PI | BFMMM_U_ALPHA3 | BFMMM_U_NU | BFMMM_U_TAU | BFMMM_U_SIGMA | BFMMM_U_LOGLIK)
#define BFMMM_SWEEP_THETA (BFMMM_U_PHI | BFMMM_U_DELTA | BFMMM_U_A | BFMMM_U_GAMMA | BFMMM_U_TAU | BFMMM_U_SIGMA | BFMMM_U_CHI | BFMMM_U_LOGLIK)
#define BFMMM_SWEEP_WARM  (BFMMM_SWEEP_NU_Z | BFMMM_SWEEP_THETA)
#define BFMMM_COV_MEAN (BFMMM_U_ETA | BFMMM_U_TAU_ETA)
#define BFMMM_COV_XI   (BFMMM_U_XI | BFMMM_U_DELTA_XI | BFMMM_U_A_XI | BFMMM_U_GAMMA_XI)
// ... 60 lines not shown
                            double* rhat, double* ess_bulk, double* ess_tail, double* ess_mean, double* mcse_mean,
                            double* mean, double* sd, int64_t capacity);

int bfmmm_chain_curve_loglik(bfmmm_handle* h, int first_slot, int n_slots, double* out, int64_t capacity);
int bfmmm_chain_curve_diagnostics(bfmmm_handle* h, int first_slot, int n_slots, int64_t max_workspace_bytes,
                                  double* rhat, double* ess_bulk, double* ess_tail, double* ess_mean, double* mcse_mean,
                                  double* mean, double* sd, int64_t capacity);
int bfmmm_chain_loo(bfmmm_handle* h, int first_slot, int n_slots, int64_t max_workspace_bytes, double* lppd, double* elpd_loo,
                    double* p_loo, double* pareto_k, double* elpd_waic, double* p_waic, int64_t capacity);

int bfmmm_chain_curve_fit(bfmmm_handle* h, int which, const double* E, int G, const int32_t* curves, int n_curves, int first_slot,
                          int n_slots, double* out, int64_t capacity);
int bfmmm_chain_curve_bands(bfmmm_handle* h, int which, const double* E, int G, const int32_t* curves, int n_curves, int first_slot,
                            int n_slots, const double* probs, int nq, int64_t max_workspace_bytes, double* mean, double* sd,
                            double* quantiles, int64_t capacity);
int bfmmm_chain_curve_bands_sim(bfmmm_handle* h, int which, const double* E, int G, const int32_t* curves, int n_curves,
                                int first_slot, int n_slots, double alpha, int64_t max_workspace_bytes,
                                double* mean, double* sd, double* crit, double* lower, double* upper, int64_t capacity);
void bfmmm_set_curve_fit_route(int route);

int bfmmm_chain_similarity(bfmmm_handle* h, const int32_t* curves, int n_curves, int first_slot, int n_slots,
                           int64_t max_workspace_bytes, double* mean, double* sd, double* chain_mean, int64_t capacity);
void bfmmm_set_similarity_block(int block);

int bfmmm_chain_similarity_loss(bfmmm_handle* h, int first_slot, int n_slots, int64_t max_workspace_bytes, double* loss,
                                int64_t capacity, int32_t* best_chain, int32_t* best_slot, double* stats);

int bfmmm_get_slot(bfmmm_handle* h, const char* name, int slot, double* out, int64_t capacity);

int bfmmm_set_chain(bfmmm_handle* h, const char* name, int first_slot, int n_slots, const double* values, int64_t count);

int bfmmm_chain_slot_loglik(bfmmm_handle* h, int first_slot, int n_slots, int store, int64_t max_workspace_bytes, double* loglik,
                            double* curve, int64_t capacity);

int bfmmm_chain_curve_cov(bfmmm_handle* h, const double* E1, int G1, const double* E2, int G2, int diagonal, const int32_t* curves,
                          int n_curves, int first_slot, int n_slots, int64_t max_workspace_bytes, double* mean, double* sd,
                          double* chain_mean, int64_t capacity);

int bfmmm_chain_align(bfmmm_handle* h, const double* Zref, int first_slot, int n_slots, int32_t* perm, double* score, int64_t capacity);

int bfmmm_chain_aligned_summary(bfmmm_handle* h, const char* name, const int32_t* perm, int first_slot, int n_slots, const double* probs,
                                int nq, int64_t max_workspace_bytes, double* rhat, double* ess_bulk, double* ess_tail, double* ess_mean,
                                double* mcse_mean, double* mean, double* sd, double* quant, int64_t capacity);

int bfmmm_chain_cluster_mean_bands(bfmmm_handle* h, const int32_t* perm, const double* E, int G, int first_slot, int n_slots,
                                   const double* probs, int nq, int64_t max_workspace_bytes, double* mean, double* sd, double* quant,
                                   int64_t capacity);

int bfmmm_chain_cluster_cov_bands(bfmmm_handle* h, const int32_t* perm, const double* E1, int G1, const double* E2, int G2,
                                  int diagonal, const int32_t* pairs, int n_pairs, const double* x, int first_slot, int n_slots,
                                  const double* probs, int nq, double alpha, int64_t max_workspace_bytes,
                                  double* mean, double* sd, double* quant, double* crit, double* lower, double* upper,
                                  double* trace, int64_t capacity);

int bfmmm_chain_rescale(bfmmm_handle* h, const int32_t* perm, const double* transform, int first_slot, int n_slots, double* mix,
                        double* mix_inv, int32_t* curve, double* rcond, double* z_min, int64_t* n_singular, int64_t capacity);

int bfmmm_chain_rescaled_summary(bfmmm_handle* h, const char* name, const double* mix, const double* mix_inv, int first_slot, int n_slots,
                                 const double* probs, int nq, int64_t max_workspace_bytes, double* rhat, double* ess_bulk,
                                 double* ess_tail, double* ess_mean, double* mcse_mean, double* mean, double* sd, double* quant,
                                 int64_t capacity);

int bfmmm_chain_cluster_mean_bands_rescaled(bfmmm_handle* h, const double* mix, const double* E, int G, const double* x, int first_slot,
                                            int n_slots, const double* probs, int nq, int64_t max_workspace_bytes, double* mean,
                                            double* sd, double* quant, int64_t capacity);

int bfmmm_chain_cluster_cov_bands_rescaled(bfmmm_handle* h, const double* mix, const double* E1, int G1, const double* E2, int G2,
                                           int diagonal, const int32_t* pairs, int n_pairs, const double* x, int first_slot,
                                           int n_slots, const double* probs, int nq, double alpha, int64_t max_workspace_bytes,
                                           double* mean, double* sd, double* quant, double* crit, double* lower, double* upper,
                                           double* trace, int64_t capacity);

int bfmmm_chain_cluster_contrast_bands(bfmmm_handle* h, const double* mix, const double* E, int G, const double* w_nu,
                                       const double* w_eta, int R, const double* weights, int first_slot, int n_slots,
                                       const double* probs, int nq, double alpha, int64_t max_workspace_bytes, double* mean,
                                       double* sd, double* quant, int32_t* n_positive, double* crit, double* lower, double* upper,
                                       int32_t* n_exceed, double* norm_stats, double* norm_quant, double* trace, double* norm_trace,
                                       int64_t capacity);

int bfmmm_chain_cluster_eigen(bfmmm_handle* h, const int32_t* perm, const double* E, int G, const double* w, const double* x,
                              int n_functions, const double* ref, int first_slot, int n_slots, const double* probs, int nq,
                              int64_t max_workspace_bytes, double* val_diag, double* val_quant, double* pve_mean, double* pve_sd,
                              double* pve_quant, double* tot_mean, double* tot_sd, double* tot_quant, double* fn_mean, double* fn_sd,
                              double* fn_quant, double* val_trace, double* fn_trace, int32_t* max_sweeps, int64_t capacity);

void bfmmm_set_cluster_eig_form(int form);

int bfmmm_chain_predict(bfmmm_handle* h, const double* y, const double* t, const double* B, const int64_t* offsets,
                        int n_new, const double* X, const int32_t* perm, int first_slot, int n_slots, int n_samples,
                        int n_stages, uint64_t seed, const double* zs, int64_t max_workspace_bytes,
                        double* lpd, double* z_mean, double* z_sd, double* ess_mean, double* ess_min,
                        double* lpd_trace, double* z_trace, double* ess_trace, double* prop_trace, double* samples,
                        int64_t capacity);

int bfmmm_chain_loo_marginal(bfmmm_handle* h, int first_slot, int n_slots, int n_samples, int n_stages, uint64_t seed, int refine,
                             double ess_floor, int refine_samples, int refine_stages, int64_t max_workspace_bytes,
                             double* lppd, double* elpd_loo, double* p_loo, double* pareto_k, double* elpd_waic, double* p_waic,
                             double* ess_mean, double* ess_min, int32_t* n_refined, int32_t* n_below,
                             double* lpd_trace, double* ess_trace, double* ess_trace_first,
                             int32_t* refined_index, double* refine_prop, double* refine_samples_out, int64_t* n_ref,
                             int64_t capacity, int64_t ref_capacity);

int bfmmm_chain_predict_laplace(bfmmm_handle* h, const double* y, const double* t, const double* B, const int64_t* offsets,
                                int n_new, const double* X, const int32_t* perm, int first_slot, int n_slots, int n_samples,
                                uint64_t seed, int64_t max_workspace_bytes,
                                double* lpd, double* z_mean, double* z_sd, double* ess_mean, double* ess_min,
                                double* lpd_trace, double* z_trace, double* ess_trace,
                                int32_t* n_modes, double* components, double* eta_samples, int64_t capacity);
int bfmmm_chain_loo_marginal_laplace(bfmmm_handle* h, int first_slot, int n_slots, int n_samples, uint64_t seed, double ess_floor,
                                     int64_t max_workspace_bytes,
                                     double* lppd, double* elpd_loo, double* p_loo, double* pareto_k, double* elpd_waic,
                                     double* p_waic, double* ess_mean, double* ess_min, int32_t* n_below,
                                     double* lpd_trace, double* ess_trace, int32_t* n_modes, double* components,
                                     double* eta_samples, int64_t capacity);

int bfmmm_chain_loo_pointwise(bfmmm_handle* h, const int32_t* curves, int n_curves, int first_slot, int n_slots,
                              int64_t max_workspace_bytes, double* lppd, double* elpd_loo, double* p_loo, double* pareto_k,
                              double* elpd_waic, double* p_waic, double* pit, double* mean, double* sd, double* loglik_trace,
                              double* pit_trace, double* mean_trace, double* var_trace, int64_t capacity);

int bfmmm_chain_loo_by_chain(bfmmm_handle* h, int unit, const int32_t* curves, int n_curves, int first_slot, int n_slots,
                             int64_t max_workspace_bytes, double* lppd, double* elpd_loo, double* p_loo, double* pareto_k,
                             double* elpd_waic, double* p_waic, int64_t capacity);

int bfmmm_chain_loo_blocks(bfmmm_handle* h, const int32_t* block_curve, const int64_t* block_offsets, const int32_t* block_obs,
                           int64_t n_blocks, int first_slot, int n_slots, int64_t max_workspace_bytes,
                           double* lppd, double* elpd_loo, double* p_loo, double* pareto_k, double* elpd_waic, double* p_waic,
                           double* pit, double* mean, double* sd, double* loglik_trace,
                           double* pit_trace, double* mean_trace, double* var_trace, int64_t block_capacity, int64_t row_capacity);

int bfmmm_chain_predict_fit(bfmmm_handle* h, const double* y, const double* t, const double* B, const int64_t* offsets,
                            int n_new, const double* X, const int32_t* perm, int first_slot, int n_slots, int n_samples,
                            int n_stages, uint64_t seed, const double* zs, const double* E, int G, int noise,
                            const double* probs, int nq, int64_t max_workspace_bytes,
                            double* lpd, double* z_mean, double* z_sd, double* ess_mean, double* ess_min,
                            double* fit_mean, double* fit_sd, double* fit_q,
                            double* lpd_trace, double* z_trace, double* ess_trace, double* prop_trace, double* samples,
                            double* mean_trace, double* var_trace, double* path_trace, int32_t* path_index, double* path_u,
                            double* path_xi, int64_t capacity);

int bfmmm_debug_get(bfmmm_handle* h, const char* name, double* out, int64_t capacity, int64_t* count);

int bfmmm_set_profile(bfmmm_handle* h, int enable);
int bfmmm_get_timing(bfmmm_handle* h, const char* name, double* ms, int64_t* launches);

void bfmmm_set_exact_instances(int enable);

void bfmmm_set_curve_record(int enable);

void bfmmm_set_solo_pair_gram(int enable);

void bfmmm_set_solo_pair_gram_tail(int enable);

const char* bfmmm_last_error(void);

#ifdef __cplusplus
}
#endif
#endif
```

Baseline: 18960 Gibbs iterations/sec.

## Map solo pair_gram workgroups to XCDs and precompute A-move transcendentals ahead

Adds an XCD-aware launch for the non-batched pair_gram kernel. It flattens the grid and assigns ks slices and the three tail jobs to specific XCDs by blockIdx modulo 8, balancing items per XCD when they fit within 32 CUs. Separately, it moves the truncated-normal log-densities and log-uniforms for the A Metropolis step into the parallel hyper draw kernel, stored in extra gstd space, so the serial hyper kernel reads them instead of computing them. Both are on by default behind new toggles. The XCD mapping relies on round-robin workgroup dispatch, and the precomputed values must match the in-place path.

```diff
diff --git a/bayesfmmm_amd/_lib.py b/bayesfmmm_amd/_lib.py
--- a/bayesfmmm_amd/_lib.py
+++ b/bayesfmmm_amd/_lib.py
@@ -127,6 +127,8 @@
     "bfmmm_set_curve_record": (None, [C.c_int]),
     "bfmmm_set_solo_pair_gram": (None, [C.c_int]),
     "bfmmm_set_solo_pair_gram_tail": (None, [C.c_int]),
+    "bfmmm_set_pair_gram_xcd": (None, [C.c_int]),
+    "bfmmm_set_hyper_ahead": (None, [C.c_int]),
     "bfmmm_last_error": (C.c_char_p, []),
 }
 
diff --git a/bayesfmmm_amd/csrc/bfmmm_capi.hip b/bayesfmmm_amd/csrc/bfmmm_capi.hip
--- a/bayesfmmm_amd/csrc/bfmmm_capi.hip
+++ b/bayesfmmm_amd/csrc/bfmmm_capi.hip
@@ -221,7 +221,7 @@
   areq(ar, &c.logz_part, (size_t)c.nblk_curve * K); areq(ar, &c.rss_part, c.nblk_curve);
   areq(ar, &c.pg_part, h->pg_part_doubles); areq(ar, &c.H, (size_t)d.R * d.LG + 2); areq(ar, &c.H2, (size_t)d.R * P * (2 * d.BW + 2));
   areq(ar, &c.tvec, (size_t)d.A * P); areq(ar, &c.rvec, (size_t)d.A * P); areq(ar, &c.hq, (size_t)d.A * P);
-  areq(ar, &c.gstd, gstd_doubles(K, P, M)); areq(ar, &c.zprep, (size_t)(3 * K + 5) * n);
+  areq(ar, &c.gstd, gstd_doubles(K, P, M) + hyper_ahead_doubles(K)); areq(ar, &c.zprep, (size_t)(3 * K + 5) * n);
   areq(ar, &c.chi_norm, (size_t)n * M); areq(ar, &c.zrec, zrec_stride(n, K)); areq(ar, &c.piprep, 9 * KMAX + 16); areq(ar, &c.Lz, (size_t)d.A * P);
   areq(ar, &c.Cmat, (size_t)d.A * P * P + 2);
   {
@@ -798,6 +798,7 @@
   if (c.d.D > 0) { plan.z = true; plan.chi = true; plan.use_rss_part = 1; }
   c.defer_loglik = (c.d.D == 0) ? 1 : 0;
   c.ll_use_part = plan.use_rss_part;
+  c.hyper_inplace = bfmmm::g_hyper_ahead ? 0 : 1;
   h->last_md = MD;
   int nsub = 1;
   if (!h->profile && h->nch >= 4) nsub = 2;
@@ -819,6 +820,8 @@
     const PgRoute& r0 = subs[0].r;
     const double v[6] = {r0.packed ? 1.0 : 0.0, (double)r0.KS, (double)r0.NKS, (double)r0.body, (double)r0.G, (double)r0.tail};
     memcpy(h->last_route, v, sizeof v);
+    const double vx[3] = {r0.xcd ? 1.0 : 0.0, (double)r0.xcd_items, r0.xcd ? 8.0 * r0.xcd_items : 0.0};
+    memcpy(h->last_xcd, vx, sizeof vx);
     const SweepRoute sr = sweep_route_decide(c.d);
     const double w[5] = {(double)sr.kernel, (double)sr.targ, c.d.mv ? 1.0 : 0.0, (double)sr.direct, (double)sr.threads};
     memcpy(h->last_sweep, w, sizeof w);
@@ -875,7 +878,7 @@
     if (bodies) segs.push_back({GK_CLOSING, 1});
   }
   const bfmmm_handle::GraphKey key{mask, MD, seed, chain, nsub, (bfmmm::g_exact_instances ? 1 : 0) | (bfmmm::g_solo_pair_gram ? 2 : 0) |
-                                                                        (bfmmm::g_solo_pair_gram_tail ? 4 : 0) | (rec_on ? 8 : 0)};
+                                                                        (bfmmm::g_solo_pair_gram_tail ? 4 : 0) | (rec_on ? 8 : 0) | (bfmmm::g_pair_gram_xcd ? 16 : 0) | (bfmmm::g_hyper_ahead ? 32 : 0)};
   if (n_iters > 0 && !(h->g_valid && h->g_key == key)) { drop_graphs(h); h->g_key = key; h->g_valid = true; }
   std::vector<FreshGraph> fresh;
   std::vector<hipGraphExec_t> seq[bfmmm_handle::MAX_SUB];
@@ -1021,6 +1024,13 @@
     *count = cnt;
     return 0;
   }
+  if (s == "pg_xcd") {
+    const int64_t cnt = sizeof h->last_xcd / sizeof h->last_xcd[0];
+    if (capacity < cnt) return fail("bfmmm_debug_get: buffer too small");
+    memcpy(out, h->last_xcd, sizeof h->last_xcd);
+    *count = cnt;
+    return 0;
+  }
   if (s == "sweep_route") {
     const int64_t cnt = sizeof h->last_sweep / sizeof h->last_sweep[0];
     if (capacity < cnt) return fail("bfmmm_debug_get: buffer too small");
@@ -1089,7 +1099,7 @@
                       {"rvec", c.rvec, (int64_t)d.A * d.P}, {"hq", c.hq, (int64_t)d.A * d.P},
                       {"theta", c.theta, (int64_t)d.K * (d.M + 1) * d.P},
                       {"chi_norm", c.chi_norm, (int64_t)d.n * d.M}, {"zprep", c.zprep, (int64_t)(3 * d.K + 5) * d.n},
-                      {"gstd", c.gstd, (int64_t)gstd_doubles(d.K, d.P, d.M)}, {"piprep", c.piprep, (int64_t)9 * KMAX + 16},
+                      {"gstd", c.gstd, (int64_t)gstd_doubles(d.K, d.P, d.M)}, {"hyper_ahead", hyper_ahead(c), (int64_t)hyper_ahead_doubles(d.K)}, {"piprep", c.piprep, (int64_t)9 * KMAX + 16},
                       {"rss_part", c.rss_part, (int64_t)c.nblk_curve}, {"logz_part", c.logz_part, (int64_t)c.nblk_curve * d.K},
                       {"stil", c.stil, (int64_t)d.n * d.P}, {"yyp_part", c.yyp_part, (int64_t)c.nblk_curve},
                       {"cfull", c.cfull, (int64_t)d.n * d.P}, {"gfull", c.gfull, (int64_t)d.n * d.P},
@@ -1108,11 +1118,13 @@
   return fail("bfmmm_debug_get: unknown name '" + s + "'");
 }
 
-namespace bfmmm { int g_exact_instances = 1; int g_solo_pair_gram = 1; int g_solo_pair_gram_tail = 1; int g_curve_record = 0; }
+namespace bfmmm { int g_exact_instances = 1; int g_solo_pair_gram = 1; int g_solo_pair_gram_tail = 1; int g_pair_gram_xcd = 1; int g_hyper_ahead = 1; int g_curve_record = 0; }
 extern "C" void bfmmm_set_curve_record(int enable) { bfmmm::g_curve_record = enable ? 1 : 0; }
 extern "C" void bfmmm_set_exact_instances(int enable) { bfmmm::g_exact_instances = enable ? 1 : 0; }
 extern "C" void bfmmm_set_solo_pair_gram(int enable) { bfmmm::g_solo_pair_gram = enable ? 1 : 0; }
 extern "C" void bfmmm_set_solo_pair_gram_tail(int enable) { bfmmm::g_solo_pair_gram_tail = enable ? 1 : 0; }
+extern "C" void bfmmm_set_pair_gram_xcd(int enable) { bfmmm::g_pair_gram_xcd = enable ? 1 : 0; }
+extern "C" void bfmmm_set_hyper_ahead(int enable) { bfmmm::g_hyper_ahead = enable ? 1 : 0; }
 
 extern "C" int bfmmm_set_profile(bfmmm_handle* h, int enable) {
   if (!h) return fail("bfmmm_set_profile: null handle");
diff --git a/bayesfmmm_amd/csrc/handle.hpp b/bayesfmmm_amd/csrc/handle.hpp
--- a/bayesfmmm_amd/csrc/handle.hpp
+++ b/bayesfmmm_amd/csrc/handle.hpp
@@ -70,6 +70,7 @@
   GraphKey g_key;
   bool g_valid = false;
   int last_md = -1;
+  double last_xcd[3] = {0, 0, 0};
   double last_route[6] = {0, 0, 0, -1, 0, 0};
   double last_sweep[5] = {-1, 0, 0, 0, 0};
   double last_curve[14] = {0, -1, 0, 0, 0, 0, -1, 0, 0, 0, 0, 0, 0, 0};
diff --git a/bayesfmmm_amd/csrc/kernels_factor.hip b/bayesfmmm_amd/csrc/kernels_factor.hip
--- a/bayesfmmm_amd/csrc/kernels_factor.hip
+++ b/bayesfmmm_amd/csrc/kernels_factor.hip
@@ -49,7 +49,7 @@
     __syncthreads();
   };
   if (bx >= nF) {
-    const int ndraw = (hyper_gstd_count(d) + 1 + 8 * d.K + 255) / 256;
+    const int ndraw = (hyper_draw_elems(d) + 255) / 256;
     const int zcw = zprep_curves_per_wg(d.K);
     const int nzp = (c.mask & U_Z) ? (d.n + zcw - 1) / zcw : 0;
     const int npi = (c.mask & (U_PI | U_ALPHA3)) ? 1 : 0;
@@ -276,7 +276,7 @@
   const int W = 2 * c.d.BW + 2, PS = c.d.P + 2 * c.d.BW + 1;
   const bool diag = c.d.BW == 0 && c.d.BWP == 0;
   const size_t lds = ((diag ? 0 : 2 * (size_t)PP * PP) + (size_t)c.d.A * PS + (size_t)c.d.A * c.d.P + PP + (size_t)c.d.P * W + 16 + 4 * PP + 2) * sizeof(double);
-  const int n_draw = c.d.K * c.d.P * c.d.M + c.d.K * c.d.M + c.d.K + 4 * c.d.K + 1 + 8 * c.d.K;
+  const int n_draw = c.d.K * c.d.P * c.d.M + c.d.K * c.d.M + c.d.K + 4 * c.d.K + 1 + 8 * c.d.K + HYPER_AHEAD * 2 * c.d.K;
   const int zcw = zprep_curves_per_wg(c.d.K);
   const int n_zprep = (c.mask & U_Z) ? (c.d.n + zcw - 1) / zcw : 0;
   const int n_znorm = ((c.mask & U_CHI) && c.d.MD > 1) ? (c.d.n * c.d.M + 255) / 256 : 0;
diff --git a/bayesfmmm_amd/csrc/kernels_pair_gram.hip b/bayesfmmm_amd/csrc/kernels_pair_gram.hip
--- a/bayesfmmm_amd/csrc/kernels_pair_gram.hip
+++ b/bayesfmmm_amd/csrc/kernels_pair_gram.hip
@@ -234,9 +234,31 @@
   __builtin_nontemporal_store(acc[2], out + 128); __builtin_nontemporal_store(acc[3], out + 192);
 }
 
+constexpr int PGX_ON = 1 << 12, PGX_NONE = 15, PGX_XCDS = 8, PGX_CUS = 32;
+
 template <bool BATCH, bool GROUPS>
-__global__ __launch_bounds__(PG_THREADS) void k_pair_gram(Ctx c0, int KS, int nks, int do_pg, int G) {
+__global__ __launch_bounds__(PG_THREADS) void k_pair_gram(Ctx c0, int KS, int nks, int do_pg, int G, int xcd) {
   const int nch = BATCH ? c0.nch : 1;
+  int ks = blockIdx.y, ct = blockIdx.x;
+  if constexpr (!BATCH) {
+    if (xcd) {
+      const int x = blockIdx.x & (PGX_XCDS - 1), W = c0.d.CTG + 1;
+      int q = blockIdx.x >> 3, job = -1;
+#pragma unroll
+      for (int j = 0; j < 3; ++j)
+        if (((xcd >> (4 * j)) & 15) == x) job = j;
+      if (job >= 0 && q == 0) {
+        ct = W; ks = job;
+      } else {
+        if (job >= 0) --q;
+        const int ns = x < nks ? (nks - x + PGX_XCDS - 1) >> 3 : 0;
+        int s = 0;
+        while (s < ns && q >= W) { q -= W; ++s; }
+        if (s >= ns) return;
+        ks = x + PGX_XCDS * s; ct = q;
+      }
+    }
+  }
   TIMELINE(c0, 1);
 #ifdef BFMMM_TIMELINE
   const int wgid = blockIdx.x + gridDim.x * blockIdx.y;
@@ -252,7 +274,6 @@
   extern __shared__ __attribute__((aligned(16))) double smem[];
   const Dims& d = c0.d;
   const int n = d.n, K = d.K, MD = d.MD;
-  const int ks = blockIdx.y, ct = blockIdx.x;
   if (ct == d.CTG + 1) {
     if (ks < nch && threadIdx.x < 256) {
       const Ctx c = chain_ctx(c0, (unsigned)ks);
@@ -865,6 +886,22 @@
     }
     r.do_pg = PG_SOLO | r.tail;
     if (r.tail & PG_SOLO_S) r.lds = std::max(r.lds, (size_t)(r.KS + 2) * (d.CTS * 16 + d.A + 1) * sizeof(double));
+    if (g_pair_gram_xcd) {
+      int items[PGX_XCDS], jx[3] = {PGX_NONE, PGX_NONE, PGX_NONE};
+      for (int x = 0; x < PGX_XCDS; ++x) items[x] = (x < r.NKS ? (r.NKS - x + PGX_XCDS - 1) / PGX_XCDS : 0) * (d.CTG + 1);
+      const bool has[3] = {true, r.NKS >= 2, (r.tail & PG_SOLO_LL) != 0};
+      const int order[3] = {1, 0, 2};
+      bool taken[PGX_XCDS] = {};
+      for (int j : order) {
+        if (!has[j]) continue;
+        int best = -1;
+        for (int x = PGX_XCDS - 1; x >= 0; --x)
+          if (!taken[x] && (best < 0 || items[x] < items[best])) best = x;
+        jx[j] = best; taken[best] = true; ++items[best];
+      }
+      const int most = *std::max_element(items, items + PGX_XCDS);
+      if (most <= PGX_CUS) { r.xcd = PGX_ON | jx[0] | (jx[1] << 4) | (jx[2] << 8); r.xcd_items = most; }
+    }
   } else {
     r.do_pg = pg ? 1 : 0;
   }
@@ -875,9 +912,10 @@
 
 void launch_pair_gram(const Ctx& c, const PgRoute& r, hipStream_t st) {
   const Dims& d = c.d;
-  if (r.body == 3) hipLaunchKernelGGL((k_pair_gram<true, true>), dim3(d.CTG + 2, r.do_pg ? std::max(r.NKS, c.nch) : c.nch, 1), dim3(PG_THREADS), r.lds, st, c, r.KS, r.NKS, r.do_pg, r.G);
-  else if (r.body == 2) hipLaunchKernelGGL((k_pair_gram<true, false>), dim3(d.CTG + 2, r.do_pg ? std::max(r.NKS, c.nch) : c.nch, 1), dim3(PG_THREADS), r.lds, st, c, r.KS, r.NKS, r.do_pg, 1);
-  else hipLaunchKernelGGL((k_pair_gram<false, false>), dim3(d.CTG + 2, r.do_pg ? r.NKS : 1, 1), dim3(PG_THREADS), r.lds, st, c, r.KS, r.NKS, r.do_pg, 1);
+  if (r.body == 3) hipLaunchKernelGGL((k_pair_gram<true, true>), dim3(d.CTG + 2, r.do_pg ? std::max(r.NKS, c.nch) : c.nch, 1), dim3(PG_THREADS), r.lds, st, c, r.KS, r.NKS, r.do_pg, r.G, 0);
+  else if (r.body == 2) hipLaunchKernelGGL((k_pair_gram<true, false>), dim3(d.CTG + 2, r.do_pg ? std::max(r.NKS, c.nch) : c.nch, 1), dim3(PG_THREADS), r.lds, st, c, r.KS, r.NKS, r.do_pg, 1, 0);
+  else if (r.xcd) hipLaunchKernelGGL((k_pair_gram<false, false>), dim3(PGX_XCDS * r.xcd_items, 1, 1), dim3(PG_THREADS), r.lds, st, c, r.KS, r.NKS, r.do_pg, 1, r.xcd);
+  else hipLaunchKernelGGL((k_pair_gram<false, false>), dim3(d.CTG + 2, r.do_pg ? r.NKS : 1, 1), dim3(PG_THREADS), r.lds, st, c, r.KS, r.NKS, r.do_pg, 1, 0);
 }
 
 void launch_pair_gram_pack(const Ctx& c, const PgRoute& r, hipStream_t st) {
diff --git a/bayesfmmm_amd/csrc/launchers.hpp b/bayesfmmm_amd/csrc/launchers.hpp
--- a/bayesfmmm_amd/csrc/launchers.hpp
+++ b/bayesfmmm_amd/csrc/launchers.hpp
@@ -50,6 +50,8 @@
   int G = 0;
   int tail = 0;
   int do_pg = 0;
+  int xcd = 0;
+  int xcd_items = 0;
   size_t lds = 0;
   PgPack pk;
   double* pack = nullptr;
diff --git a/bayesfmmm_amd/csrc/model.hpp b/bayesfmmm_amd/csrc/model.hpp
--- a/bayesfmmm_amd/csrc/model.hpp
+++ b/bayesfmmm_amd/csrc/model.hpp
@@ -121,6 +121,8 @@
 static_assert(GSTD_REC <= GSTD_SPARE, "the recorded acceptance values live in the spare doubles of gstd");
 __host__ __device__ inline size_t gstd_used(int K, int P, int M) { return (size_t)K * P * M + (size_t)K * M + 13 * (size_t)K + 1; }
 __host__ __device__ inline size_t gstd_doubles(int K, int P, int M) { return gstd_used(K, P, M) + GSTD_SPARE; }
+constexpr int HYPER_AHEAD = 3;
+__host__ __device__ inline size_t hyper_ahead_doubles(int K) { return 2 * (size_t)HYPER_AHEAD * 2 * K; }
 
 struct Ctx {
   Dims d;
@@ -175,6 +177,7 @@
   double* delta_cur;
   int pi_in_factor;
   int defer_loglik;
+  int hyper_inplace;
   int defer_hyper;
   int ll_use_part;
   int covariance_adj;
@@ -190,6 +193,7 @@
   int nblk_curve;
   double* zrec;
 };
+__host__ __device__ inline double* hyper_ahead(const Ctx& c) { return c.gstd + gstd_doubles(c.d.K, c.d.P, c.d.M); }
 
 struct PgPack {
   int KS, NKS;
@@ -233,6 +237,8 @@
 extern int g_exact_instances;
 extern int g_curve_record;
 extern int g_solo_pair_gram;
+extern int g_pair_gram_xcd;
+extern int g_hyper_ahead;
 extern int g_solo_pair_gram_tail;
 
 __host__ __device__ inline int tri_index(int n, int a, int b) {
diff --git a/bayesfmmm_amd/csrc/scalar_jobs.hpp b/bayesfmmm_amd/csrc/scalar_jobs.hpp
--- a/bayesfmmm_amd/csrc/scalar_jobs.hpp
+++ b/bayesfmmm_amd/csrc/scalar_jobs.hpp
@@ -223,6 +223,7 @@
 }
 
 __device__ inline int hyper_gstd_count(const Dims& d) { return d.K * d.P * d.M + d.K * d.M + d.K + 4 * d.K; }
+__device__ inline int hyper_draw_elems(const Dims& d) { return hyper_gstd_count(d) + 1 + 8 * d.K + HYPER_AHEAD * 2 * d.K; }
 
 __device__ inline void job_hyper_draws(const Ctx& c, int first) {
   const Dims& d = c.d;
@@ -231,8 +232,21 @@
   const RngKey key = make_key(c.seed, c.chain, dyn->iter, dyn->tt_step);
   const int nG = K * P * M;
   const int e = first + threadIdx.x;
-  if (e > hyper_gstd_count(d) + 8 * K) return;
+  if (e >= hyper_draw_elems(d)) return;
   double v;
+  if (e > hyper_gstd_count(d) + 8 * K) {
+    const int x = e - hyper_gstd_count(d) - 8 * K - 1, cell = x / HYPER_AHEAD, q = x - HYPER_AHEAD * cell;
+    const int j = cell / 2, i = cell - 2 * j;
+    const double sd = (i == 0) ? (c.h.var_epsilon1 / c.h.beta1l) : (c.h.var_epsilon2 / c.h.beta2l);
+    const double cur = c.Aa[j + (size_t)K * i];
+    if (q == 2) v = log(runif(key, UPD_A_ACC, (uint32_t)cell));
+    else {
+      const double na = rtruncnorm_lo(key, UPD_A_PROP, (uint32_t)(j * 2 + i), cur, sd, 0.0);
+      v = (q == 0) ? dtruncnorm_lo_log(cur, na, sd, 0.0) : dtruncnorm_lo_log(na, cur, sd, 0.0);
+    }
+    hyper_ahead(c)[x] = v;
+    return;
+  }
   if (e > hyper_gstd_count(d)) {
     const int x = e - hyper_gstd_count(d) - 1, cell = x >> 2, q = x & 3;
     const int j = cell / 2, i = cell - 2 * j;
@@ -363,6 +377,8 @@
   const double lgaT = aTerm[cellT * 4 + 2 * (jobT & 1)], laT = aTerm[cellT * 4 + 2 * (jobT & 1) + 1];
   const int cellA = min(tid, 2 * K - 1), idxA = (cellA >> 1) + K * (cellA & 1);
   const double curA = c.Aa[idxA], naA = aProp[cellA], unA = aUnif[cellA];
+  const double* ahead = hyper_ahead(c);
+  const double dtnT = ahead[cellT * HYPER_AHEAD + (jobT & 1)], lunA = ahead[cellA * HYPER_AHEAD + 2];
   const int kt = min(max(tid - 32, 0), K - 1);
   const double tau_old = dyn->tau[kt], gTk = gT[kt];
   constexpr int GU = 3;
@@ -520,7 +536,10 @@
         v = -x * lga + (c.h.alpha2l - 1) * la - (a * c.h.beta2l) + (a - 1) * sl;
       }
     } else {
-      v = (job == 2) ? dtruncnorm_lo_log(cur, na, sd, 0.0) : dtruncnorm_lo_log(na, cur, sd, 0.0);
+      if (c.hyper_inplace) {
+        v = (job == 2) ? dtruncnorm_lo_log(cur, na, sd, 0.0) : dtruncnorm_lo_log(na, cur, sd, 0.0);
+        hyper_ahead(c)[HYPER_AHEAD * 2 * K + cell * HYPER_AHEAD + (job & 1)] = v;
+      } else v = dtnT;
     }
     aw[cell * 6 + 1 + job] = v;
   }
@@ -530,7 +549,9 @@
     if (do_A) {
       const double* w = aw + tid * 6;
       const double acc = (w[2] + w[3]) - w[1] - w[4];
-      if (log(unA) < acc) { av = naA; c.Aa[idxA] = naA; }
+      double lu = lunA;
+      if (c.hyper_inplace) { lu = log(unA); hyper_ahead(c)[HYPER_AHEAD * 2 * K + tid * HYPER_AHEAD + 2] = lu; }
+      if (lu < acc) { av = naA; c.Aa[idxA] = naA; }
     }
     c.c_A[(size_t)slot * K * 2 + idxA] = av;
   }
diff --git a/include/bfmmm.h b/include/bfmmm.h
--- a/include/bfmmm.h
+++ b/include/bfmmm.h
@@ -236,6 +236,10 @@
 
 void bfmmm_set_solo_pair_gram_tail(int enable);
 
+void bfmmm_set_pair_gram_xcd(int enable);
+
+void bfmmm_set_hyper_ahead(int enable);
+
 const char* bfmmm_last_error(void);
 
 #ifdef __cplusplus
```

New measurement: 19060 Gibbs iterations/sec (median of 5 runs). Within noise of the previous version (+0.5%).
